# Quantco/tabmat

Measured on AMD Instinct MI355X. Metric: SplitMatrix.sandwich GFLOP/s + effective HBM GB/s, 10M×1k mixed, higher is better.
Workload: dtype f64; 1 GPU; SplitMatrix.sandwich: dense128 + csr512@5% + cats(256,96,32), 10000000 rows/GPU, p=1024, float64 (BASELINE configs[3]); rows_per_gpu=10000000, p=1024, launch=eager, collective=none

## Files before the change

include/tabmat_hip.h:

```cpp
#ifndef TABMAT_HIP_H
#define TABMAT_HIP_H

#include <stddef.h>
#include <stdint.h>

#ifdef __cplusplus
extern "C" {
#endif

#define TM_OK 0
#define TM_EINVAL (-1)
#define TM_ENOMEM (-2)
#define TM_EUNSUPPORTED (-3)

int tm_version(void);
const char *tm_last_error(void);
int tm_device_count(int *count);
int tm_set_device(int device);
int tm_device_info(char *name, int name_len, int *compute_units, int64_t *hbm_bytes);
int tm_malloc(void **ptr, size_t bytes);
int tm_free(void *ptr);
int tm_memcpy_h2d(void *dst, const void *h_src, size_t bytes, void *stream);
int tm_memcpy_d2h(void *h_dst, const void *src, size_t bytes, void *stream);
int tm_memset(void *dst, int value, size_t bytes, void *stream);
// ... 400 lines not shown
                                          int64_t n_sel, int64_t m, const double *d_sel, double *out,
                                          void *stream);
int tm_multi_cat_sparse_sandwich_rows_u8_f32(const void *const *h_codes, const int64_t *h_ncols,
                                             const int32_t *h_drop_first, int n_cats,
                                             const float *cm_data, const uint8_t *cm_col8,
                                             const int32_t *row_ranges, const int32_t *rows,
                                             int64_t n_sel, int64_t m, const float *d_sel, float *out,
                                             void *stream);
int tm_multi_cat_sparse_sandwich_rows_u8_f64(const void *const *h_codes, const int64_t *h_ncols,
                                             const int32_t *h_drop_first, int n_cats,
                                             const double *cm_data, const uint8_t *cm_col8,
                                             const int32_t *row_ranges, const int32_t *rows,
                                             int64_t n_sel, int64_t m, const double *d_sel, double *out,
                                             void *stream);
int tm_multi_cat_sparse_sandwich_ent_f32(const void *const *h_codes, const int64_t *h_ncols,
                                         const int32_t *h_drop_first, int n_cats, int64_t n, const float *d,
                                         const float *vals, const uint16_t *meta, const uint32_t *bstart,
                                         int64_t n_slots, int64_t mk, float *out, void *stream);
int tm_multi_cat_sparse_sandwich_ent_f64(const void *const *h_codes, const int64_t *h_ncols,
                                         const int32_t *h_drop_first, int n_cats, int64_t n, const double *d,
                                         const double *vals, const uint16_t *meta, const uint32_t *bstart,
                                         int64_t n_slots, int64_t mk, double *out, void *stream);
int tm_multi_cat_pack_codes(const void *const *h_codes, const int64_t *h_ncols, const int32_t *h_drop_first, int n_cats,
                            int64_t n, uint32_t *packed, void *stream);
int tm_multi_cat_sparse_sandwich_entp_f32(const void *const *h_codes, const int64_t *h_ncols,
                                          const int32_t *h_drop_first, int n_cats, int64_t n, const float *d,
                                          const float *vals, const uint16_t *meta, const uint32_t *bstart,
                                          int64_t n_slots, int64_t mk, const uint32_t *packed, float *out, void *stream);
int tm_multi_cat_sparse_sandwich_entp_f64(const void *const *h_codes, const int64_t *h_ncols,
                                          const int32_t *h_drop_first, int n_cats, int64_t n, const double *d,
                                          const double *vals, const uint16_t *meta, const uint32_t *bstart,
                                          int64_t n_slots, int64_t mk, const uint32_t *packed, double *out, void *stream);

int tm_multi_cat_sparse_sandwich_slab_f32(const void *const *h_codes, const int64_t *h_ncols,
                                          const int32_t *h_drop_first, int n_cats, int64_t n,
                                          const float *d, const float *vals, const uint32_t *koff,
                                          const uint8_t *ecol, const int64_t *gptr, int64_t m,
                                          float *out, void *stream);
int tm_multi_cat_sparse_sandwich_slab_f64(const void *const *h_codes, const int64_t *h_ncols,
                                          const int32_t *h_drop_first, int n_cats, int64_t n,
                                          const double *d, const double *vals, const uint32_t *koff,
                                          const uint8_t *ecol, const int64_t *gptr, int64_t m,
                                          double *out, void *stream);

int tm_multi_cat_pairs_max_bins(void);
int tm_multi_cat_pairs_max_slots(void);
int tm_multi_cat_pairs_row_words(void);
int tm_multi_cat_pairs_f32(const int64_t *cat_tab, int64_t n, const float *d, const int32_t *rows,
                           int64_t n_rows, const int32_t *bundles, int n_bundles,
                           const int32_t *wg_map, int n_wg, int slots, int64_t bins,
                           const int64_t *desc, int64_t n_pairs, const int64_t *pos, double *tables,
                           double *out, int64_t p, void *stream);
int tm_multi_cat_pairs_f64(const int64_t *cat_tab, int64_t n, const double *d, const int32_t *rows,
                           int64_t n_rows, const int32_t *bundles, int n_bundles,
                           const int32_t *wg_map, int n_wg, int slots, int64_t bins,
                           const int64_t *desc, int64_t n_pairs, const int64_t *pos, double *tables,
                           double *out, int64_t p, void *stream);

int tm_multi_cat_matvec_f32(const int64_t *cat_tab, int n_cats, const int64_t *pos, const float *v,
                            int64_t n, float *out, void *stream);
int tm_multi_cat_matvec_f64(const int64_t *cat_tab, int n_cats, const int64_t *pos, const double *v,
                            int64_t n, double *out, void *stream);

int tm_csr_densify_cols_f32(const float *data, const int32_t *indices, const int64_t *indptr, int64_t n,
                            const int32_t *colmap, float *T, int64_t ld, void *stream);
int tm_csr_densify_cols_f64(const double *data, const int32_t *indices, const int64_t *indptr, int64_t n,
                            const int32_t *colmap, double *T, int64_t ld, void *stream);
int tm_csc_densify_cols_f32(const int32_t *rows, const float *vals, const int64_t *seg, const int32_t *tcol,
                            int64_t n_sel, int64_t max_len, float *T, int64_t ld, void *stream);
int tm_csc_densify_cols_f64(const int32_t *rows, const double *vals, const int64_t *seg, const int32_t *tcol,
                            int64_t n_sel, int64_t max_len, double *T, int64_t ld, void *stream);
int tm_dense_gather_cols_f32(const float *X, int64_t n, int64_t m, int order_f, const int32_t *cols,
                             int64_t n_sel, float *T, int64_t ld, int64_t t0, void *stream);
int tm_dense_gather_cols_f64(const double *X, int64_t n, int64_t m, int order_f, const int32_t *cols,
                             int64_t n_sel, double *T, int64_t ld, int64_t t0, void *stream);

int tm_scatter_block_f32(const float *src, int64_t nr, int64_t nc, const int64_t *ri,
                         const int64_t *ci, double *out, int64_t p, int mirror, int diag,
                         void *stream);
int tm_scatter_block_f64(const double *src, int64_t nr, int64_t nc, const int64_t *ri,
                         const int64_t *ci, double *out, int64_t p, int mirror, int diag,
                         void *stream);

int tm_sparse_sandwich_chunked_rows_f32(const float *cm_data, const int32_t *cm_indices,
                                        const int32_t *row_ranges, int64_t n_sel, int64_t m,
                                        int64_t nnz, const float *d_sel, float *out, void *stream);
int tm_sparse_sandwich_chunked_rows_f64(const double *cm_data, const int32_t *cm_indices,
                                        const int32_t *row_ranges, int64_t n_sel, int64_t m,
                                        int64_t nnz, const double *d_sel, double *out, void *stream);

int tm_sparse_sandwich_chunked_u8_f32(const float *cm_data, const uint8_t *cm_col8, const int32_t *cptr, int64_t n,
                                      int64_t m, int64_t nnz, const float *d, float *out, void *stream);
int tm_sparse_sandwich_chunked_u8_f64(const double *cm_data, const uint8_t *cm_col8, const int32_t *cptr, int64_t n,
                                      int64_t m, int64_t nnz, const double *d, double *out, void *stream);
int tm_sparse_sandwich_chunked_rows_u8_f32(const float *cm_data, const uint8_t *cm_col8, const int32_t *row_ranges,
                                           int64_t n_sel, int64_t m, int64_t nnz, const float *d_sel, float *out,
                                           void *stream);
int tm_sparse_sandwich_chunked_rows_u8_f64(const double *cm_data, const uint8_t *cm_col8, const int32_t *row_ranges,
                                           int64_t n_sel, int64_t m, int64_t nnz, const double *d_sel, double *out,
                                           void *stream);
int tm_sparse_sandwich_direct_f32(const float *csr_data, const int32_t *csr_indices,
                                  const int64_t *csr_indptr, int64_t n, int64_t m, const float *d,
                                  float *out, void *stream);
int tm_sparse_sandwich_direct_f64(const double *csr_data, const int32_t *csr_indices,
                                  const int64_t *csr_indptr, int64_t n, int64_t m, const double *d,
                                  double *out, void *stream);
int tm_csr_dense_sandwich_rows_f32(const float *cm_data, const int32_t *cm_indices,
                                   const int32_t *row_ranges, int64_t n_sel, const int32_t *rows,
                                   const float *d_sel, int64_t n, int64_t m, const float *B, int64_t r,
                                   int order_f, float *out, void *stream);
int tm_csr_dense_sandwich_rows_f64(const double *cm_data, const int32_t *cm_indices,
                                   const int32_t *row_ranges, int64_t n_sel, const int32_t *rows,
                                   const double *d_sel, int64_t n, int64_t m, const double *B, int64_t r,
                                   int order_f, double *out, void *stream);
int tm_csr_dense_sandwich_rows_u8_f32(const float *cm_data, const uint8_t *cm_col8,
                                      const int32_t *row_ranges, int64_t n_sel, const int32_t *rows,
                                      const float *d_sel, int64_t n, int64_t m, const float *B, int64_t r,
                                      int order_f, float *out, void *stream);
int tm_csr_dense_sandwich_rows_u8_f64(const double *cm_data, const uint8_t *cm_col8,
                                      const int32_t *row_ranges, int64_t n_sel, const int32_t *rows,
                                      const double *d_sel, int64_t n, int64_t m, const double *B, int64_t r,
                                      int order_f, double *out, void *stream);

int tm_cat_det_block_rows(void);
int tm_cat_transpose_matvec_det_f32(const int32_t *perm, const int64_t *bstart, int64_t n_blocks,
                                    const int64_t *cat_bptr, int64_t n_cols, const float *v,
                                    float *out, int accumulate, void *stream);
int tm_cat_transpose_matvec_det_f64(const int32_t *perm, const int64_t *bstart, int64_t n_blocks,
                                    const int64_t *cat_bptr, int64_t n_cols, const double *v,
                                    double *out, int accumulate, void *stream);

int tm_cat_dense_sandwich_sorted_f32(const int32_t *perm, const int64_t *bstart, int64_t n_blocks,
                                     const int64_t *cat_bptr, int64_t n_cols, const float *d,
                                     const float *Y, int64_t m, float *out, void *stream);
int tm_cat_dense_sandwich_sorted_f64(const int32_t *perm, const int64_t *bstart, int64_t n_blocks,
                                     const int64_t *cat_bptr, int64_t n_cols, const double *d,
                                     const double *Y, int64_t m, double *out, void *stream);
int tm_csc_dense_sandwich_sorted_f32(const int32_t *rows, const float *vals, const int64_t *bstart,
                                     int64_t n_blocks, const int64_t *col_bptr, int64_t n_cols,
                                     const float *d, const float *Y, int64_t m, float *out,
                                     void *stream);
int tm_csc_dense_sandwich_sorted_f64(const int32_t *rows, const double *vals, const int64_t *bstart,
                                     int64_t n_blocks, const int64_t *col_bptr, int64_t n_cols,
                                     const double *d, const double *Y, int64_t m, double *out,
                                     void *stream);
int tm_cat_sparse_sandwich_sorted_f32(const int32_t *perm, const int64_t *bstart, int64_t n_blocks,
                                      const int64_t *cat_bptr, int64_t n_cols, const float *d,
                                      const float *csr_data, const int32_t *csr_indices,
                                      const int64_t *csr_indptr, int64_t m, float *out, void *stream);
int tm_cat_sparse_sandwich_sorted_f64(const int32_t *perm, const int64_t *bstart, int64_t n_blocks,
                                      const int64_t *cat_bptr, int64_t n_cols, const double *d,
                                      const double *csr_data, const int32_t *csr_indices,
                                      const int64_t *csr_indptr, int64_t m, double *out, void *stream);

int tm_csr_matvec_multi_f32(const float *csr_data, const int32_t *csr_indices,
                            const int64_t *csr_indptr, int64_t n, int64_t m, const float *V,
                            int64_t K, const int32_t *rows, int64_t n_rows, const int32_t *cols,
                            int64_t n_cols, float *out, void *stream);
int tm_csr_rmatvec_multi_f32(const float *csr_data, const int32_t *csr_indices,
                             const int64_t *csr_indptr, int64_t n, int64_t m, const float *V,
                             int64_t K, const int32_t *rows, int64_t n_rows, const int32_t *cols,
                             int64_t n_cols, float *out, void *stream);
int tm_dense_matvec_multi_f32(const float *X, int64_t n, int64_t m, int order_f, const float *V,
                              int64_t K, const int32_t *rows, int64_t n_rows, const int32_t *cols,
                              int64_t n_cols, float *out, void *stream);
int tm_dense_rmatvec_multi_f32(const float *X, int64_t n, int64_t m, int order_f, const float *V,
// ... 31 lines not shown
```

tabmat_amd/csrc/cat.hip:

```cpp
#include <algorithm>

#include "common.hpp"
#include "reduce.hpp"

namespace tmh {

__global__ void fill_i32_kernel(int32_t *p, int64_t n, int32_t v) {
    int64_t i = (int64_t)blockIdx.x * blockDim.x + threadIdx.x;
    if (i < n) p[i] = v;
}

__global__ void scatter_iota_i32_kernel(int32_t *map, const int32_t *cols, int64_t n_cols) {
    int64_t i = (int64_t)blockIdx.x * blockDim.x + threadIdx.x;
    if (i < n_cols) map[cols[i]] = (int32_t)i;
}

int build_col_map(int32_t *map, int64_t m, const int32_t *cols, int64_t n_cols, hipStream_t st) {
    if (m > 0) {
        hipLaunchKernelGGL(fill_i32_kernel, dim3((unsigned)ceil_div(m, 256)), dim3(256), 0, st, map,
                           m, -1);
        TM_LAUNCH_CHECK();
    }
    if (n_cols > 0) {
        hipLaunchKernelGGL(scatter_iota_i32_kernel, dim3((unsigned)ceil_div(n_cols, 256)),
                           dim3(256), 0, st, map, cols, n_cols);
        TM_LAUNCH_CHECK();
    }
    return TM_OK;
}

template <typename F, bool TWO>
__global__ __launch_bounds__(1024) void hist_lds_kernel(
    const int32_t *__restrict__ ci, const int32_t *__restrict__ cj, const F *__restrict__ w,
    const int32_t *__restrict__ rows, int64_t n_iter, int64_t rows_per_block, int drop_i,
    int drop_j, int i_ncol, int j_ncol, int ti, const int32_t *__restrict__ col_map,
    F *__restrict__ ws, int64_t stride) {
    extern __shared__ __attribute__((aligned(16))) unsigned char smem_raw[];
    lds_acc_t *bins = reinterpret_cast<lds_acc_t *>(smem_raw);
    const int part = blockIdx.y;
    const int i0 = part * ti;
    const int i1 = min(i0 + ti, i_ncol);
    const int nbins = TWO ? (i1 - i0) * j_ncol : (i1 - i0);
    for (int b = threadIdx.x; b < nbins; b += blockDim.x) bins[b] = 0.0;
    __syncthreads();

    const int64_t t0 = (int64_t)blockIdx.x * rows_per_block;
    const int64_t t1 = min(t0 + rows_per_block, n_iter);
    int64_t tbeg = t0;
    if (!TWO && rows == nullptr && (t0 & 3) == 0 &&
        ((reinterpret_cast<uintptr_t>(ci) | reinterpret_cast<uintptr_t>(w)) & 15) == 0) {
        typedef int i4 __attribute__((ext_vector_type(4)));
        const int64_t nvec = (t1 - t0) / 4;
        for (int64_t q = threadIdx.x; q < nvec; q += blockDim.x) {
            const int64_t k = t0 + q * 4;
            const i4 cc = *reinterpret_cast<const i4 *>(ci + k);
            F ww[4];
#pragma unroll
            for (int e = 0; e < 4; ++e) ww[e] = w[k + e];
#pragma unroll
            for (int e = 0; e < 4; ++e) {
                const int c = cc[e] - drop_i;
                if (c >= i0 && c < i1 && !(col_map && col_map[c] < 0)) atomic_add(&bins[c - i0], (lds_acc_t)ww[e]);
            }
        }
        tbeg = t0 + nvec * 4;
    }
    for (int64_t t = tbeg + threadIdx.x; t < t1; t += blockDim.x) {
        const int64_t k = rows ? (int64_t)rows[t] : t;
        const int c = ci[k] - drop_i;
        if (c < i0 || c >= i1) continue;
        if (TWO) {
            const int c2 = cj[k] - drop_j;
            if (c2 < 0) continue;
            atomic_add(&bins[(c - i0) * j_ncol + c2], (lds_acc_t)w[k]);
        } else {
            if (col_map && col_map[c] < 0) continue;
            atomic_add(&bins[c - i0], (lds_acc_t)w[k]);
        }
    }
    __syncthreads();
    F *dst = ws + ((int64_t)part * gridDim.x + blockIdx.x) * stride;
    for (int b = threadIdx.x; b < nbins; b += blockDim.x) dst[b] = (F)bins[b];
}

template <typename F, bool TWO>
// ... 1138 lines not shown
        }
    }
    __syncthreads();
    F *dst = ws + ((int64_t)blockIdx.y * gridDim.x + blockIdx.x) * stride;
    for (int b = threadIdx.x; b < cs.total * GC; b += blockDim.x)
        dst[b] = (F)tile[(b / GC) * TSTR + (b % GC)];
}

template <typename F, typename IX>
__global__ __launch_bounds__(1024) void multi_cat_sparse_rows_kernel(
    CatSet cs, const F *__restrict__ cm_data, const IX *__restrict__ cm_ind,
    const int32_t *__restrict__ ranges, const int32_t *__restrict__ rows, const F *__restrict__ d_sel,
    int64_t n_sel, int64_t rows_per_block, F *__restrict__ ws, int64_t stride) {
    constexpr int GC = 32;
    extern __shared__ __attribute__((aligned(16))) unsigned char smem_raw[];
    lds_acc_t *tile = reinterpret_cast<lds_acc_t *>(smem_raw);
    constexpr int tstr = GC + 1;
    const int nel = cs.total * tstr;
    for (int b = threadIdx.x; b < nel; b += blockDim.x) tile[b] = 0.0;
    __syncthreads();
    static_assert(SPARSE_CHUNK_COLS == 4 * GC, "the chunk of the chunk-major twin must hold four 32-column groups");
    const int g = blockIdx.y;
    const int ch = g >> 2;
    const int lane = threadIdx.x & 63, wave = threadIdx.x >> 6, nwave = blockDim.x >> 6;
    const int lr = lane >> 3, lt = lane & 7;
    const int64_t t0 = (int64_t)blockIdx.x * rows_per_block;
    const int64_t t1 = min(t0 + rows_per_block, n_sel);
    const int32_t *rg = ranges + (int64_t)ch * n_sel * 2;
    for (int64_t k0 = t0 + wave * 8; k0 < t1; k0 += (int64_t)nwave * 8) {
        const int64_t k = k0 + lr;
        if (k >= t1) continue;
        const F dk = d_sel[k];
        if (dk == F(0)) continue;
        const int e0 = rg[2 * k], e1 = rg[2 * k + 1];
        if (e0 >= e1) continue;
        const int64_t row = rows[k];
        int off[MAX_CATS];
#pragma unroll
        for (int c = 0; c < MAX_CATS; ++c) {
            off[c] = -1;
            if (c < cs.n_cats) {
                const int col = cs.codes[c][row] - cs.drop[c];
                off[c] = col >= 0 ? (cs.off[c] + col) * tstr : -1;
            }
        }
        for (int e = e0 + lt; e < e1; e += 8) {
            const int col = (int)cm_ind[e] - (sizeof(IX) == 1 ? (g & 3) : g) * GC;
            if (col < 0 || col >= GC) continue;
            const lds_acc_t x = (lds_acc_t)(dk * cm_data[e]);
#pragma unroll
            for (int c = 0; c < MAX_CATS; ++c)
                if (off[c] >= 0) atomic_add(&tile[off[c] + col], x);
        }
    }
    __syncthreads();
    F *dst = ws + ((int64_t)blockIdx.y * gridDim.x + blockIdx.x) * stride;
    for (int b = threadIdx.x; b < cs.total * GC; b += blockDim.x)
        dst[b] = (F)tile[(b / GC) * tstr + (b % GC)];
}

static int make_catset(const void *const *h_codes, const int64_t *h_ncols, const int32_t *h_drop,
                       int n_cats, CatSet *cs) {
    if (n_cats < 1 || n_cats > MAX_CATS) {
        set_error("multi-cat call supports 1..%d categoricals, got %d", MAX_CATS, n_cats);
        return TM_EINVAL;
    }
    int off = 0;
    for (int c = 0; c < MAX_CATS; ++c) {
        cs->codes[c] = c < n_cats ? reinterpret_cast<const int32_t *>(h_codes[c]) : nullptr;
        cs->ncol[c] = c < n_cats ? (int)h_ncols[c] : 0;
        cs->drop[c] = c < n_cats ? h_drop[c] : 0;
        cs->off[c] = off;
        off += cs->ncol[c];
    }
    cs->n_cats = n_cats;
    cs->total = off;
    return TM_OK;
}

template <typename F>
static int run_multi_cat_dense(const void *const *h_codes, const int64_t *h_ncols,
                               const int32_t *h_drop, int n_cats, int64_t n, const F *d, const F *M,
                               int64_t m, int order_f, F *out, hipStream_t st,
                               const int32_t *rows = nullptr, int64_t n_rows = 0) {
    CatSet cs;
    int rc = make_catset(h_codes, h_ncols, h_drop, n_cats, &cs);
    if (rc) return rc;
    const int64_t total = (int64_t)cs.total * m;
    if (total == 0) return TM_OK;
    if (rows != nullptr) n = n_rows;
    if (n == 0) {
        TM_HIP(hipMemsetAsync(out, 0, sizeof(F) * (size_t)total, st));
        return TM_OK;
    }
    {
        constexpr int VEC = MCW_VEC;
        constexpr int TJW = 16 * VEC;
        const size_t tile_b = ((sizeof(lds_acc_t) * (size_t)cs.total * TJW + 15) / 16) * 16;
        const size_t lds_w = tile_b + (size_t)16 * MCW_RS * (sizeof(F) + (size_t)n_cats * sizeof(int));
        if (!order_f && n_cats <= 8 && m >= VEC && m % VEC == 0 &&
            (reinterpret_cast<uintptr_t>(M) & 15) == 0 && lds_w <= 150 * 1024 &&
            (int64_t)cs.total * TJW * (int64_t)sizeof(lds_acc_t) < (1ll << 30)) {
            const int64_t n_parts = ceil_div(m, TJW);
            const int64_t stride = (int64_t)cs.total * TJW;
            int64_t nblk = std::max<int64_t>(1, tune("catdense_rounds", 1) * NUM_CU / n_parts);
            nblk = std::min<int64_t>(nblk, std::max<int64_t>(1, ceil_div(n, 4096)));
            const int64_t rpb = ceil_div(ceil_div(n, nblk), MCW_RS) * MCW_RS;
            nblk = ceil_div(n, rpb);
            const size_t tmp_bytes = ((sizeof(F) * (size_t)(n_parts * stride) + 255) / 256) * 256;
            void *wsv = nullptr;
            rc = get_workspace(tmp_bytes + sizeof(F) * (size_t)(n_parts * nblk * stride) + 256, &wsv, st);
            if (rc) return rc;
            F *tmp = reinterpret_cast<F *>(wsv);
            F *ws = reinterpret_cast<F *>(reinterpret_cast<char *>(wsv) + tmp_bytes);
            auto gow = [&](auto kern) -> int {
                TM_HIP(hipFuncSetAttribute(reinterpret_cast<const void *>(kern),
                                           hipFuncAttributeMaxDynamicSharedMemorySize, (int)lds_w));
                prof_begin(st);
                const int nw_dflt = (sizeof(F) == 8 && tile_b > 64 * 1024) ? 8 : 16;
                const int nw = (int)std::min<int64_t>(16, std::max<int64_t>(4, tune("catdense_waves", nw_dflt)));
                hipLaunchKernelGGL(kern, dim3((unsigned)nblk, (unsigned)n_parts), dim3(nw * 64), lds_w, st,
                                   cs, d, M, n, m, rpb, ws, stride, rows, wg_log_ptr());
                prof_end(st);
                TM_LAUNCH_CHECK();
                return TM_OK;
            };
            if (n_cats == 1) rc = gow(&multi_cat_dense_wide_kernel<F, 1>);
            else if (n_cats == 2) rc = gow(&multi_cat_dense_wide_kernel<F, 2>);
            else if (n_cats == 3) rc = gow(&multi_cat_dense_wide_kernel<F, 3>);
            else if (n_cats == 4) rc = gow(&multi_cat_dense_wide_kernel<F, 4>);
            else if (n_cats == 5) rc = gow(&multi_cat_dense_wide_kernel<F, 5>);
            else if (n_cats == 6) rc = gow(&multi_cat_dense_wide_kernel<F, 6>);
            else if (n_cats == 7) rc = gow(&multi_cat_dense_wide_kernel<F, 7>);
            else rc = gow(&multi_cat_dense_wide_kernel<F, 8>);
            if (rc) return rc;
            rc = launch_reduce_partials<F>(ws, stride, (int)nblk, (int)n_parts, tmp, n_parts * stride,
                                           false, st);
            if (rc) return rc;
            hipLaunchKernelGGL((multi_cat_untile_kernel<F>), dim3((unsigned)ceil_div(total, 256)),
                               dim3(256), 0, st, tmp, (int64_t)cs.total, m, TJW, out);
            TM_LAUNCH_CHECK();
            return TM_OK;
        }
    }
    if (rows != nullptr) {
        set_error("multi_cat_dense: the row-list form needs the wide-load path");
        return TM_EUNSUPPORTED;
    }
    int TJ = 64;
    while (TJ > 1 && sizeof(lds_acc_t) * (size_t)cs.total * TJ > HIST_LDS_MAX) TJ >>= 1;
    while (TJ > 1 && TJ / 2 >= m) TJ >>= 1;
    if (sizeof(lds_acc_t) * (size_t)cs.total * TJ > HIST_LDS_MAX) {
        set_error("multi_cat_dense: %d stacked categories exceed the LDS tile", cs.total);
        return TM_EUNSUPPORTED;
    }
    const int64_t n_parts = ceil_div(m, TJ);
    const int64_t stride = (int64_t)cs.total * TJ;
    const size_t lds = sizeof(lds_acc_t) * (size_t)stride;
    int64_t nblk = std::max<int64_t>(1, NUM_CU / n_parts);
    nblk = std::min<int64_t>(nblk, std::max<int64_t>(1, ceil_div(n, 4096)));
    const int64_t rpb = ceil_div(n, nblk);
    nblk = ceil_div(n, rpb);
    const size_t tmp_bytes = ((sizeof(F) * (size_t)(n_parts * stride) + 255) / 256) * 256;
    void *wsv = nullptr;
    rc = get_workspace(tmp_bytes + sizeof(F) * (size_t)(n_parts * nblk * stride) + 256, &wsv, st);
    if (rc) return rc;
    F *tmp = reinterpret_cast<F *>(wsv);
    F *ws = reinterpret_cast<F *>(reinterpret_cast<char *>(wsv) + tmp_bytes);
    auto go = [&](auto kern) -> int {
        if (lds > 48 * 1024)
            TM_HIP(hipFuncSetAttribute(reinterpret_cast<const void *>(kern),
                                       hipFuncAttributeMaxDynamicSharedMemorySize, (int)lds));
        prof_begin(st);
        hipLaunchKernelGGL(kern, dim3((unsigned)nblk, (unsigned)n_parts), dim3(1024), lds, st, cs, d,
                           M, n, m, rpb, ws, stride);
        prof_end(st);
        TM_LAUNCH_CHECK();
        return TM_OK;
    };
#define TM_MCD_CASE(V)                                                                       \
    case V:                                                                                  \
        if (order_f) rc = go(&multi_cat_dense_f_kernel<F, V>);                               \
        else if (n_cats == 1) rc = go(&multi_cat_dense_c_kernel<F, V, 1>);                   \
        else if (n_cats == 2) rc = go(&multi_cat_dense_c_kernel<F, V, 2>);                   \
        else if (n_cats == 3) rc = go(&multi_cat_dense_c_kernel<F, V, 3>);                   \
        else if (n_cats == 4) rc = go(&multi_cat_dense_c_kernel<F, V, 4>);                   \
        else rc = go(&multi_cat_dense_c_kernel<F, V, 0>);                                    \
        break;
    switch (TJ) {
        TM_MCD_CASE(64)
        TM_MCD_CASE(32)
        TM_MCD_CASE(16)
        TM_MCD_CASE(8)
        TM_MCD_CASE(4)
        TM_MCD_CASE(2)
        TM_MCD_CASE(1)
        default:
            rc = TM_EINVAL;
    }
#undef TM_MCD_CASE
    if (rc) return rc;
    rc = launch_reduce_partials<F>(ws, stride, (int)nblk, (int)n_parts, tmp, n_parts * stride, false,
                                   st);
    if (rc) return rc;
    hipLaunchKernelGGL((multi_cat_untile_kernel<F>), dim3((unsigned)ceil_div(total, 256)),
                       dim3(256), 0, st, tmp, (int64_t)cs.total, m, TJ, out);
    TM_LAUNCH_CHECK();
    return TM_OK;
}

template <typename F, typename IX>
static int run_multi_cat_sparse_rows(const void *const *h_codes, const int64_t *h_ncols,
                                     const int32_t *h_drop, int n_cats, const F *cm_data,
                                     const IX *cm_ind, const int32_t *ranges, const int32_t *rows,
                                     int64_t n_sel, int64_t m, const F *d_sel, F *out, hipStream_t st);

template <typename F>
static int run_multi_cat_sparse(const void *const *h_codes, const int64_t *h_ncols,
                                const int32_t *h_drop, int n_cats, int64_t n, const F *d,
                                const F *vals, const unsigned *koff, const unsigned char *ecol,
                                const int64_t *gptr, int64_t m, int slab_rows, int group_cols,
                                F *out, hipStream_t st) {
    CatSet cs;
    int rc = make_catset(h_codes, h_ncols, h_drop, n_cats, &cs);
    if (rc) return rc;
    const int64_t total = (int64_t)cs.total * m;
    if (total == 0) return TM_OK;
    if (n == 0) {
        TM_HIP(hipMemsetAsync(out, 0, sizeof(F) * (size_t)total, st));
// ... 1 lines not shown
    }
    const int64_t stride = (int64_t)cs.total * group_cols;
    const size_t tile_bytes = ((sizeof(lds_acc_t) * (size_t)cs.total * (group_cols + 1) + 15) / 16) * 16;
    if (tile_bytes > HIST_LDS_MAX) {
        set_error("multi_cat_sparse: %d stacked categories exceed the LDS tile", cs.total);
        return TM_EUNSUPPORTED;
    }
    const int nw = (int)std::min<int64_t>(16, std::max<int64_t>(4, tune("catsparse_waves", 16)));
    const size_t stage_bytes = (size_t)nw * slab_rows * (sizeof(F) + sizeof(int32_t) * (size_t)n_cats);
    const bool stage = tile_bytes + stage_bytes <= 150 * 1024;
    const size_t lds = tile_bytes + (stage ? stage_bytes : 0);
    const int n_groups = (int)ceil_div(m, group_cols);
    const int64_t n_slabs = ceil_div(n, slab_rows);
    int64_t nblk = std::max<int64_t>(1, tune("catsparse_rounds", 1) * NUM_CU / n_groups);
    nblk = std::min<int64_t>(nblk, n_slabs);
    const int64_t spb = ceil_div(n_slabs, nblk);
    nblk = ceil_div(n_slabs, spb);
    const size_t tmp_bytes = ((sizeof(F) * (size_t)(n_groups * stride) + 255) / 256) * 256;
    void *wsv = nullptr;
    rc = get_workspace(tmp_bytes + sizeof(F) * (size_t)((int64_t)n_groups * nblk * stride) + 256,
                       &wsv, st);
    if (rc) return rc;
    F *tmp = reinterpret_cast<F *>(wsv);
    F *ws = reinterpret_cast<F *>(reinterpret_cast<char *>(wsv) + tmp_bytes);
    if (stage && n_cats <= 8 && slab_rows == 128) {
        auto kpf = n_cats == 1   ? &multi_cat_sparse_pf_kernel<F, 1>
                   : n_cats == 2 ? &multi_cat_sparse_pf_kernel<F, 2>
                   : n_cats == 3 ? &multi_cat_sparse_pf_kernel<F, 3>
                   : n_cats == 4 ? &multi_cat_sparse_pf_kernel<F, 4>
                   : n_cats == 5 ? &multi_cat_sparse_pf_kernel<F, 5>
                   : n_cats == 6 ? &multi_cat_sparse_pf_kernel<F, 6>
                   : n_cats == 7 ? &multi_cat_sparse_pf_kernel<F, 7>
                                 : &multi_cat_sparse_pf_kernel<F, 8>;
        if (lds > 48 * 1024)
            TM_HIP(hipFuncSetAttribute(reinterpret_cast<const void *>(kpf),
                                       hipFuncAttributeMaxDynamicSharedMemorySize, (int)lds));
        prof_begin(st);
        hipLaunchKernelGGL(kpf, dim3((unsigned)nblk, (unsigned)n_groups), dim3(nw * 64), lds, st, cs, d,
                           vals, koff, ecol, gptr, n_groups, n_slabs, spb, group_cols, n, ws, stride,
                           wg_log_ptr());
        prof_end(st);
        TM_LAUNCH_CHECK();
    } else {
        auto kern = stage ? &multi_cat_sparse_kernel<F, true> : &multi_cat_sparse_kernel<F, false>;
        if (lds > 48 * 1024)
            TM_HIP(hipFuncSetAttribute(reinterpret_cast<const void *>(kern),
                                       hipFuncAttributeMaxDynamicSharedMemorySize, (int)lds));
        prof_begin(st);
        hipLaunchKernelGGL(kern, dim3((unsigned)nblk, (unsigned)n_groups), dim3(nw * 64), lds, st, cs,
                           d, vals, koff, ecol, gptr, n_groups, n_slabs, spb, slab_rows, group_cols,
                           n, ws, stride);
        prof_end(st);
        TM_LAUNCH_CHECK();
    }
    rc = launch_reduce_partials<F>(ws, stride, (int)nblk, n_groups, tmp,
                                   (int64_t)n_groups * stride, false, st);
    if (rc) return rc;
    hipLaunchKernelGGL((multi_cat_untile_kernel<F>), dim3((unsigned)ceil_div(total, 256)),
                       dim3(256), 0, st, tmp, (int64_t)cs.total, m, group_cols, out);
    TM_LAUNCH_CHECK();
    return TM_OK;
}

__global__ __launch_bounds__(256) void multi_cat_pack_codes_kernel(CatSet cs, int64_t n, unsigned *__restrict__ out) {
    for (int64_t r = (int64_t)blockIdx.x * blockDim.x + threadIdx.x; r < n; r += (int64_t)gridDim.x * blockDim.x) {
        unsigned pk = 0u;
#pragma unroll
        for (int c = 0; c < 3; ++c) {
            unsigned f = 1023u;
            if (c < cs.n_cats) {
                const int col = cs.codes[c][r] - cs.drop[c];
                if (col >= 0 && col < cs.ncol[c]) f = (unsigned)(cs.off[c] + col);
            }
            pk |= f << (10 * c);
        }
        out[r] = pk;
    }
}

template <typename F>
static int run_multi_cat_sparse_ent(const void *const *h_codes, const int64_t *h_ncols, const int32_t *h_drop,
                                    int n_cats, int64_t n, const F *d, const F *vals, const unsigned short *meta,
                                    const unsigned *bstart, int64_t mk, F *out, hipStream_t st,
                                    const unsigned *packed = nullptr, int64_t n_slots = 0) {
    CatSet cs;
    int rc = make_catset(h_codes, h_ncols, h_drop, n_cats, &cs);
    if (rc) return rc;
    const int64_t total = (int64_t)cs.total * mk;
    if (total == 0) return TM_OK;
    if (n == 0) {
        TM_HIP(hipMemsetAsync(out, 0, sizeof(F) * (size_t)total, st));
        return TM_OK;
    }
    TM_REQUIRE(mk % 16 == 0 && n_cats >= 1 && n_cats <= 8, "kernel columns in groups of 16, 1 .. 8 categoricals");
    TM_REQUIRE(n < (1ll << 28), "at most 2^28 - 1 rows per block");
    constexpr int GC = 32;
    const int64_t stride = (int64_t)cs.total * GC;
    const size_t lds = ((sizeof(lds_acc_t) * (size_t)cs.total * (GC + 1) + 15) / 16) * 16;
    if (lds > HIST_LDS_MAX) {
        set_error("multi_cat_sparse_ent: %d stacked categories exceed the LDS tile", cs.total);
        return TM_EUNSUPPORTED;
    }
    const int nw = (int)std::min<int64_t>(16, std::max<int64_t>(4, tune("catsparse_waves", 16)));
    const int n_groups = (int)(mk / 16);
    const int n_pairs = (n_groups + 1) / 2;
    const int64_t n_slabs = ceil_div(n, 64);
    int64_t nblk = std::max<int64_t>(1, tune("catsparse_rounds", 1) * NUM_CU / n_pairs);
    nblk = std::min<int64_t>(nblk, n_slabs);
    const int64_t spb = ceil_div(n_slabs, nblk);
    nblk = ceil_div(n_slabs, spb);
    const size_t tmp_bytes = ((sizeof(F) * (size_t)(n_pairs * stride) + 255) / 256) * 256;
    void *wsv = nullptr;
    rc = get_workspace(tmp_bytes + sizeof(F) * (size_t)((int64_t)n_pairs * nblk * stride) + 256, &wsv, st);
    if (rc) return rc;
    F *tmp = reinterpret_cast<F *>(wsv);
    F *ws = reinterpret_cast<F *>(reinterpret_cast<char *>(wsv) + tmp_bytes);
    auto kern = n_cats == 1   ? &multi_cat_sparse_ent_kernel<F, 1>
                : n_cats == 2 ? &multi_cat_sparse_ent_kernel<F, 2>
                : n_cats == 3 ? &multi_cat_sparse_ent_kernel<F, 3>
                : n_cats == 4 ? &multi_cat_sparse_ent_kernel<F, 4>
                : n_cats == 5 ? &multi_cat_sparse_ent_kernel<F, 5>
                : n_cats == 6 ? &multi_cat_sparse_ent_kernel<F, 6>
                : n_cats == 7 ? &multi_cat_sparse_ent_kernel<F, 7>
                              : &multi_cat_sparse_ent_kernel<F, 8>;
    TM_REQUIRE(packed == nullptr || (n_cats <= 3 && cs.total < 1023), "packed codes: at most 3 categoricals, 1022 levels");
    const int ncw = packed != nullptr ? 1 : n_cats;
    const size_t lds_staged = lds + (size_t)nw * 64 * (sizeof(F) + 4 * (size_t)ncw);
    const double fill = (double)n_slots / ((double)std::max(n_groups, 1) * (double)n_slabs);
    if (tune("catsparse_staged", 1) != 0 && lds_staged <= 156 * 1024 &&
        fill >= (double)tune("catsparse_staged_fill", 44)) {
        using KS = void (*)(CatSet, const F *, const F *, const unsigned short *, const unsigned *, int, int64_t, int64_t,
                            int64_t, F *, int64_t, const unsigned *, int);
        KS ks = nullptr;
        if (packed != nullptr) {
            ks = n_cats == 1 ? &multi_cat_sparse_ent_staged_kernel<F, 1, true>
                 : n_cats == 2 ? &multi_cat_sparse_ent_staged_kernel<F, 2, true>
                               : &multi_cat_sparse_ent_staged_kernel<F, 3, true>;
        } else {
            ks = n_cats == 1   ? &multi_cat_sparse_ent_staged_kernel<F, 1, false>
                 : n_cats == 2 ? &multi_cat_sparse_ent_staged_kernel<F, 2, false>
                 : n_cats == 3 ? &multi_cat_sparse_ent_staged_kernel<F, 3, false>
                 : n_cats == 4 ? &multi_cat_sparse_ent_staged_kernel<F, 4, false>
                 : n_cats == 5 ? &multi_cat_sparse_ent_staged_kernel<F, 5, false>
                 : n_cats == 6 ? &multi_cat_sparse_ent_staged_kernel<F, 6, false>
                 : n_cats == 7 ? &multi_cat_sparse_ent_staged_kernel<F, 7, false>
                               : &multi_cat_sparse_ent_staged_kernel<F, 8, false>;
        }
        if (lds_staged > 48 * 1024)
            TM_HIP(hipFuncSetAttribute(reinterpret_cast<const void *>(ks),
                                       hipFuncAttributeMaxDynamicSharedMemorySize, (int)lds_staged));
        prof_begin(st);
        hipLaunchKernelGGL(ks, dim3((unsigned)nblk, (unsigned)n_pairs), dim3(nw * 64), lds_staged, st, cs, d, vals,
                           meta, bstart, n_groups, n, n_slabs, spb, ws, stride, packed, (int)lds);
        prof_end(st);
        TM_LAUNCH_CHECK();
    } else {
        if (lds > 48 * 1024)
            TM_HIP(hipFuncSetAttribute(reinterpret_cast<const void *>(kern),
                                       hipFuncAttributeMaxDynamicSharedMemorySize, (int)lds));
        prof_begin(st);
        hipLaunchKernelGGL(kern, dim3((unsigned)nblk, (unsigned)n_pairs), dim3(nw * 64), lds, st, cs, d, vals, meta,
                           bstart, n_groups, n, n_slabs, spb, ws, stride, packed);
        prof_end(st);
        TM_LAUNCH_CHECK();
    }
    rc = launch_reduce_partials<F>(ws, stride, (int)nblk, n_pairs, tmp, (int64_t)n_pairs * stride, false, st);
    if (rc) return rc;
    hipLaunchKernelGGL((multi_cat_untile_kernel<F>), dim3((unsigned)ceil_div(total, 256)), dim3(256), 0, st, tmp,
                       (int64_t)cs.total, mk, GC, out);
    TM_LAUNCH_CHECK();
    return TM_OK;
}

}

using namespace tmh;

#define TM_CHECK_COMMON(nn) \
    TM_REQUIRE((nn) >= 0, "negative size")

extern "C" {

int tm_cat_transpose_matvec_f32(const int32_t *codes, int64_t n, int64_t n_cols, int drop_first,
                                const float *v, const int32_t *rows, int64_t n_rows,
                                const int32_t *cols, int64_t n_cols_sel, float *out, void *stream) {
    TM_CHECK_COMMON(n);
    return run_cat_tmv<float>(codes, n, n_cols, drop_first, v, rows, n_rows, cols, n_cols_sel, out,
                              as_stream(stream));
}
int tm_cat_transpose_matvec_f64(const int32_t *codes, int64_t n, int64_t n_cols, int drop_first,
                                const double *v, const int32_t *rows, int64_t n_rows,
                                const int32_t *cols, int64_t n_cols_sel, double *out,
                                void *stream) {
    TM_CHECK_COMMON(n);
    return run_cat_tmv<double>(codes, n, n_cols, drop_first, v, rows, n_rows, cols, n_cols_sel,
                               out, as_stream(stream));
}

int tm_cat_matvec_f32(const int32_t *codes, int64_t n, int64_t n_cols, int drop_first,
                      const float *v, const int32_t *cols, int64_t n_cols_sel, float *out,
                      void *stream) {
    TM_CHECK_COMMON(n);
    return run_cat_matvec<float>(codes, n, n_cols, drop_first, v, cols, n_cols_sel, out,
                                 as_stream(stream));
}
int tm_cat_matvec_f64(const int32_t *codes, int64_t n, int64_t n_cols, int drop_first,
                      const double *v, const int32_t *cols, int64_t n_cols_sel, double *out,
                      void *stream) {
    TM_CHECK_COMMON(n);
    return run_cat_matvec<double>(codes, n, n_cols, drop_first, v, cols, n_cols_sel, out,
                                  as_stream(stream));
}

int tm_cat_matvec_assign_f32(const int32_t *codes, int64_t n, int64_t n_cols, int drop_first,
                             const float *v, const int32_t *cols, int64_t n_cols_sel, float *out,
                             void *stream) {
    TM_CHECK_COMMON(n);
    return run_cat_matvec<float>(codes, n, n_cols, drop_first, v, cols, n_cols_sel, out,
                                 as_stream(stream), true);
}
int tm_cat_matvec_assign_f64(const int32_t *codes, int64_t n, int64_t n_cols, int drop_first,
                             const double *v, const int32_t *cols, int64_t n_cols_sel, double *out,
                             void *stream) {
    TM_CHECK_COMMON(n);
    return run_cat_matvec<double>(codes, n, n_cols, drop_first, v, cols, n_cols_sel, out,
                                  as_stream(stream), true);
}

int tm_cat_cat_sandwich_f32(const int32_t *i_codes, const int32_t *j_codes, int64_t n,
                            const float *d, const int32_t *rows, int64_t n_rows, int64_t i_ncol,
                            int64_t j_ncol, int i_drop_first, int j_drop_first, float *out,
                            void *stream) {
    TM_CHECK_COMMON(n);
    return run_hist<float, true>(i_codes, j_codes, d, rows, rows ? n_rows : n, i_drop_first,
                                 j_drop_first, i_ncol, j_ncol, nullptr, out, false,
                                 as_stream(stream));
}
int tm_cat_cat_sandwich_f64(const int32_t *i_codes, const int32_t *j_codes, int64_t n,
                            const double *d, const int32_t *rows, int64_t n_rows, int64_t i_ncol,
                            int64_t j_ncol, int i_drop_first, int j_drop_first, double *out,
                            void *stream) {
    TM_CHECK_COMMON(n);
    return run_hist<double, true>(i_codes, j_codes, d, rows, rows ? n_rows : n, i_drop_first,
                                  j_drop_first, i_ncol, j_ncol, nullptr, out, false,
                                  as_stream(stream));
}

int tm_cat_cat_sandwich_atomic_f32(const int32_t *i_codes, const int32_t *j_codes, int64_t n,
// ... 55 lines not shown
    TM_CHECK_COMMON(n);
    return run_cat_sparse<float>(codes, n, i_ncol, drop_first, csr_data, csr_indices, csr_indptr,
                                 s_ncol, d, rows, n_rows, cols, n_cols, out, as_stream(stream));
}
int tm_cat_sparse_sandwich_f64(const int32_t *codes, int64_t n, int64_t i_ncol, int drop_first,
                               const double *csr_data, const int32_t *csr_indices,
                               const int64_t *csr_indptr, int64_t s_ncol, const double *d,
                               const int32_t *rows, int64_t n_rows, const int32_t *cols,
                               int64_t n_cols, double *out, void *stream) {
    TM_CHECK_COMMON(n);
    return run_cat_sparse<double>(codes, n, i_ncol, drop_first, csr_data, csr_indices, csr_indptr,
                                  s_ncol, d, rows, n_rows, cols, n_cols, out, as_stream(stream));
}

int tm_multi_cat_dense_sandwich_f32(const void *const *h_codes, const int64_t *h_ncols,
                                    const int32_t *h_drop_first, int n_cats, int64_t n,
                                    const float *d, const float *M, int64_t M_ncol, int order_f,
                                    float *out, void *stream) {
    return run_multi_cat_dense<float>(h_codes, h_ncols, h_drop_first, n_cats, n, d, M, M_ncol,
                                      order_f, out, as_stream(stream));
}
int tm_multi_cat_dense_sandwich_f64(const void *const *h_codes, const int64_t *h_ncols,
                                    const int32_t *h_drop_first, int n_cats, int64_t n,
                                    const double *d, const double *M, int64_t M_ncol, int order_f,
                                    double *out, void *stream) {
    return run_multi_cat_dense<double>(h_codes, h_ncols, h_drop_first, n_cats, n, d, M, M_ncol,
                                       order_f, out, as_stream(stream));
}
int tm_multi_cat_dense_sandwich_rows_f32(const void *const *h_codes, const int64_t *h_ncols,
                                         const int32_t *h_drop_first, int n_cats, int64_t n,
                                         const float *d, const float *M, int64_t M_ncol,
                                         const int32_t *rows, int64_t n_rows, float *out,
                                         void *stream) {
    return run_multi_cat_dense<float>(h_codes, h_ncols, h_drop_first, n_cats, n, d, M, M_ncol, 0, out,
                                      as_stream(stream), rows, n_rows);
}
int tm_multi_cat_dense_sandwich_rows_f64(const void *const *h_codes, const int64_t *h_ncols,
                                         const int32_t *h_drop_first, int n_cats, int64_t n,
                                         const double *d, const double *M, int64_t M_ncol,
                                         const int32_t *rows, int64_t n_rows, double *out,
                                         void *stream) {
    return run_multi_cat_dense<double>(h_codes, h_ncols, h_drop_first, n_cats, n, d, M, M_ncol, 0, out,
                                       as_stream(stream), rows, n_rows);
}
int tm_multi_cat_sparse_sandwich_ent_f32(const void *const *h_codes, const int64_t *h_ncols,
                                         const int32_t *h_drop_first, int n_cats, int64_t n, const float *d,
                                         const float *vals, const uint16_t *meta, const uint32_t *bstart,
                                         int64_t n_slots, int64_t mk, float *out, void *stream) {
    return run_multi_cat_sparse_ent<float>(h_codes, h_ncols, h_drop_first, n_cats, n, d, vals, meta, bstart, mk,
                                           out, as_stream(stream), nullptr, n_slots);
}
int tm_multi_cat_sparse_sandwich_ent_f64(const void *const *h_codes, const int64_t *h_ncols,
                                         const int32_t *h_drop_first, int n_cats, int64_t n, const double *d,
                                         const double *vals, const uint16_t *meta, const uint32_t *bstart,
                                         int64_t n_slots, int64_t mk, double *out, void *stream) {
    return run_multi_cat_sparse_ent<double>(h_codes, h_ncols, h_drop_first, n_cats, n, d, vals, meta, bstart, mk,
                                            out, as_stream(stream), nullptr, n_slots);
}
int tm_multi_cat_pack_codes(const void *const *h_codes, const int64_t *h_ncols, const int32_t *h_drop_first, int n_cats,
                            int64_t n, uint32_t *packed, void *stream) {
    CatSet cs;
    int rc = make_catset(h_codes, h_ncols, h_drop_first, n_cats, &cs);
    if (rc) return rc;
    TM_REQUIRE(n_cats <= 3 && cs.total < 1023, "packed codes: at most 3 categoricals, 1022 stacked levels");
    if (n == 0) return TM_OK;
    hipLaunchKernelGGL(multi_cat_pack_codes_kernel, dim3((unsigned)std::min<int64_t>(4 * NUM_CU, ceil_div(n, 256))),
                       dim3(256), 0, as_stream(stream), cs, n, packed);
    TM_LAUNCH_CHECK();
    return TM_OK;
}
int tm_multi_cat_sparse_sandwich_entp_f32(const void *const *h_codes, const int64_t *h_ncols,
                                          const int32_t *h_drop_first, int n_cats, int64_t n, const float *d,
                                          const float *vals, const uint16_t *meta, const uint32_t *bstart,
                                          int64_t n_slots, int64_t mk, const uint32_t *packed, float *out, void *stream) {
    return run_multi_cat_sparse_ent<float>(h_codes, h_ncols, h_drop_first, n_cats, n, d, vals, meta, bstart, mk, out,
                                           as_stream(stream), packed, n_slots);
}
int tm_multi_cat_sparse_sandwich_entp_f64(const void *const *h_codes, const int64_t *h_ncols,
                                          const int32_t *h_drop_first, int n_cats, int64_t n, const double *d,
                                          const double *vals, const uint16_t *meta, const uint32_t *bstart,
                                          int64_t n_slots, int64_t mk, const uint32_t *packed, double *out, void *stream) {
    return run_multi_cat_sparse_ent<double>(h_codes, h_ncols, h_drop_first, n_cats, n, d, vals, meta, bstart, mk,
                                            out, as_stream(stream), packed, n_slots);
}
int tm_multi_cat_sparse_sandwich_slab_f32(const void *const *h_codes, const int64_t *h_ncols,
                                          const int32_t *h_drop_first, int n_cats, int64_t n,
                                          const float *d, const float *vals, const uint32_t *koff,
                                          const uint8_t *ecol, const int64_t *gptr, int64_t m,
                                          float *out, void *stream) {
    return run_multi_cat_sparse<float>(h_codes, h_ncols, h_drop_first, n_cats, n, d, vals, koff,
                                       ecol, gptr, m, tm_slab_rows(), tm_slab_group_cols(), out,
                                       as_stream(stream));
}
int tm_multi_cat_sparse_sandwich_slab_f64(const void *const *h_codes, const int64_t *h_ncols,
                                          const int32_t *h_drop_first, int n_cats, int64_t n,
                                          const double *d, const double *vals, const uint32_t *koff,
                                          const uint8_t *ecol, const int64_t *gptr, int64_t m,
                                          double *out, void *stream) {
    return run_multi_cat_sparse<double>(h_codes, h_ncols, h_drop_first, n_cats, n, d, vals, koff,
                                        ecol, gptr, m, tm_slab_rows(), tm_slab_group_cols(), out,
                                        as_stream(stream));
}

}

namespace tmh {
template <typename F, typename IX>
static int run_multi_cat_sparse_rows(const void *const *h_codes, const int64_t *h_ncols,
                                     const int32_t *h_drop, int n_cats, const F *cm_data,
                                     const IX *cm_ind, const int32_t *ranges, const int32_t *rows,
                                     int64_t n_sel, int64_t m, const F *d_sel, F *out, hipStream_t st) {
    CatSet cs;
    int rc = make_catset(h_codes, h_ncols, h_drop, n_cats, &cs);
    if (rc) return rc;
    const int64_t total = (int64_t)cs.total * m;
    if (total == 0) return TM_OK;
    if (n_sel == 0) {
        TM_HIP(hipMemsetAsync(out, 0, sizeof(F) * (size_t)total, st));
        return TM_OK;
    }
    constexpr int GC = 32;
    const size_t lds = ((sizeof(lds_acc_t) * (size_t)cs.total * (GC + 1) + 15) / 16) * 16;
    if (lds > HIST_LDS_MAX) {
        set_error("multi_cat_sparse_rows: %d stacked categories exceed the LDS tile", cs.total);
        return TM_EUNSUPPORTED;
    }
    const int n_groups = (int)ceil_div(m, GC);
    const int64_t stride = (int64_t)cs.total * GC;
    int64_t nblk = std::max<int64_t>(1, tune("catsparse_rounds", 1) * NUM_CU / n_groups);
    nblk = std::min<int64_t>(nblk, std::max<int64_t>(1, ceil_div(n_sel, 2048)));
    const int64_t rpb = ceil_div(n_sel, nblk);
    nblk = ceil_div(n_sel, rpb);
    const size_t tmp_bytes = ((sizeof(F) * (size_t)(n_groups * stride) + 255) / 256) * 256;
    void *wsv = nullptr;
    rc = get_workspace(tmp_bytes + sizeof(F) * (size_t)((int64_t)n_groups * nblk * stride) + 256, &wsv, st);
    if (rc) return rc;
    F *tmp = reinterpret_cast<F *>(wsv);
    F *ws = reinterpret_cast<F *>(reinterpret_cast<char *>(wsv) + tmp_bytes);
    auto kern = &multi_cat_sparse_rows_kernel<F, IX>;
    if (lds > 48 * 1024)
        TM_HIP(hipFuncSetAttribute(reinterpret_cast<const void *>(kern),
                                   hipFuncAttributeMaxDynamicSharedMemorySize, (int)lds));
    prof_begin(st);
    hipLaunchKernelGGL(kern, dim3((unsigned)nblk, (unsigned)n_groups), dim3(1024), lds, st, cs, cm_data,
                       cm_ind, ranges, rows, d_sel, n_sel, rpb, ws, stride);
    prof_end(st);
    TM_LAUNCH_CHECK();
    rc = launch_reduce_partials<F>(ws, stride, (int)nblk, n_groups, tmp, (int64_t)n_groups * stride, false, st);
    if (rc) return rc;
    hipLaunchKernelGGL((multi_cat_untile_kernel<F>), dim3((unsigned)ceil_div(total, 256)), dim3(256), 0,
                       st, tmp, (int64_t)cs.total, m, GC, out);
    TM_LAUNCH_CHECK();
    return TM_OK;
}
}

extern "C" {
int tm_multi_cat_sparse_sandwich_rows_f32(const void *const *h_codes, const int64_t *h_ncols,
                                          const int32_t *h_drop_first, int n_cats,
                                          const float *cm_data, const int32_t *cm_indices,
                                          const int32_t *row_ranges, const int32_t *rows,
                                          int64_t n_sel, int64_t m, const float *d_sel, float *out,
                                          void *stream) {
    return tmh::run_multi_cat_sparse_rows<float, int32_t>(h_codes, h_ncols, h_drop_first, n_cats, cm_data,
                                                 cm_indices, row_ranges, rows, n_sel, m, d_sel, out,
                                                 tmh::as_stream(stream));
// ... 33 lines not shown
```

tabmat_amd/csrc/common.hpp:

```cpp
#pragma once

#include <hip/hip_runtime.h>
#include <type_traits>
#include <stdint.h>
#include <stdio.h>

#include "../../include/tabmat_hip.h"

namespace tmh {

constexpr int WAVE = 64;
constexpr int NUM_CU = 256;
constexpr int NUM_XCD = 8;
constexpr int SPARSE_CHUNK_COLS = 128;
constexpr size_t LDS_BYTES = 160 * 1024;

void set_error(const char *fmt, ...);
int hip_fail(hipError_t e, const char *what, const char *file, int line);

#define TM_HIP(expr)                                                  \
    do {                                                              \
        hipError_t _e = (expr);                                       \
        if (_e != hipSuccess) return tmh::hip_fail(_e, #expr, __FILE__, __LINE__); \
    } while (0)

#define TM_LAUNCH_CHECK() TM_HIP(hipGetLastError())

#define TM_REQUIRE(cond, msg)                 \
    do {                                      \
        if (!(cond)) {                        \
            tmh::set_error("%s: %s", __func__, msg); \
            return TM_EINVAL;                 \
        }                                     \
    } while (0)

int get_workspace(size_t bytes, void **ptr, hipStream_t st);

void prof_begin(hipStream_t st);
void prof_end(hipStream_t st);
void prof_hold(bool on);

int64_t tune(const char *key, int64_t dflt);

int run_syrk_co(const double *X, int64_t n, int64_t m, const double *d, double *out,
                double *colsum, hipStream_t st, const double *center = nullptr, const double *v = nullptr,
                double *xtv = nullptr);
inline bool syrk_co_ok(const void *X, int64_t m) {
    return m > 0 && m <= 128 && (reinterpret_cast<uintptr_t>(X) & 15) == 0;
}
inline bool syrk_co_pays(int64_t m) { return m > 64; }

int run_syrk_i8_panel(const double *X, int64_t ldx, int64_t n, int64_t m, const double *d, const double *colmax,
                      double *out, int64_t ldo, double *colsum, int *history, hipStream_t st,
                      const double *center = nullptr, const double *v = nullptr, double *xtv = nullptr);

int run_syrk_bf16x3(const float *X, int64_t n, int64_t m, const float *d, float *out, hipStream_t st);
inline bool syrk_bf16x3_ok(const void *X, int64_t m) {
    return m > 0 && m <= 256 && m % 4 == 0 && (reinterpret_cast<uintptr_t>(X) & 15) == 0;
}

bool syrk_narrow_ok(int64_t m);
template <typename F>
int run_syrk_narrow(const F *X, int64_t n, int64_t m, int order_f, const F *d, F *out, hipStream_t st);

inline hipStream_t as_stream(void *s) { return reinterpret_cast<hipStream_t>(s); }

inline int64_t ceil_div(int64_t a, int64_t b) { return (a + b - 1) / b; }

typedef double lds_acc_t;

template <typename F>
__device__ __forceinline__ void atomic_add(F *p, F v) {
    atomicAdd(p, v);
}

template <typename F>
__device__ __forceinline__ F wave_sum(F v) {
#pragma unroll
    for (int off = 32; off > 0; off >>= 1) v += __shfl_down(v, off, 64);
    return v;
}

template <int S>
__device__ __forceinline__ int dpp_xor_i32(int v) {
    if constexpr (S == 1) return __builtin_amdgcn_mov_dpp(v, 0xB1, 0xF, 0xF, true);
    else if constexpr (S == 2) return __builtin_amdgcn_mov_dpp(v, 0x4E, 0xF, 0xF, true);
    else if constexpr (S == 3) return __builtin_amdgcn_mov_dpp(v, 0x1B, 0xF, 0xF, true);
    else if constexpr (S == 4) {
        const int m = __builtin_amdgcn_mov_dpp(v, 0x141, 0xF, 0xF, true);
        return __builtin_amdgcn_mov_dpp(m, 0x1B, 0xF, 0xF, true);
    } else return __builtin_amdgcn_mov_dpp(v, 0x128, 0xF, 0xF, true);
}
template <int S>
__device__ __forceinline__ double dpp_xor(double v) {
    return __hiloint2double(dpp_xor_i32<S>(__double2hiint(v)), dpp_xor_i32<S>(__double2loint(v)));
}
template <int S>
__device__ __forceinline__ float dpp_xor(float v) {
    return __int_as_float(dpp_xor_i32<S>(__float_as_int(v)));
}


__device__ __forceinline__ int64_t readfirstlane_i64(int64_t v) {
    const unsigned lo = (unsigned)__builtin_amdgcn_readfirstlane((int)(v & 0xffffffffll));
    const unsigned hi = (unsigned)__builtin_amdgcn_readfirstlane((int)(v >> 32));
    return (int64_t)(((unsigned long long)hi << 32) | lo);
}

template <int N, int K0 = 0, typename Fn>
__device__ __forceinline__ void static_for(Fn &&f) {
    if constexpr (K0 < N) {
        f(std::integral_constant<int, K0>{});
        static_for<N, K0 + 1>(f);
    }
}

template <int K>
__device__ __forceinline__ int dpp_bcast8_i32(int v, int x4) {
    constexpr int QP = (K & 3) * 0x55;
    const int t = __builtin_amdgcn_mov_dpp(x4, QP, 0xF, 0xF, true);
    return __builtin_amdgcn_update_dpp(t, v, QP, 0xF, K < 4 ? 0x5 : 0xA, false);
}
template <int K>
__device__ __forceinline__ double dpp_bcast8(double v, double x4) {
    return __hiloint2double(dpp_bcast8_i32<K>(__double2hiint(v), __double2hiint(x4)),
                            dpp_bcast8_i32<K>(__double2loint(v), __double2loint(x4)));
}
template <int K>
__device__ __forceinline__ float dpp_bcast8(float v, float x4) {
    return __int_as_float(dpp_bcast8_i32<K>(__float_as_int(v), __float_as_int(x4)));
}

struct WgLog {
    unsigned long long hw, t0, t1, tag;
};
struct WgLogBuf {
    unsigned long long count, cap, pad0, pad1;
    WgLog e[1];
};
enum WgTag { WG_SYRK_CO = 1, WG_K2 = 2, WG_CAT_DENSE = 3, WG_CAT_SPARSE = 4, WG_K3 = 5 };
inline WgLogBuf *wg_log_ptr() { return reinterpret_cast<WgLogBuf *>((uintptr_t)tune("wg_log", 0)); }
__device__ __forceinline__ unsigned long long wg_log_begin(const WgLogBuf *b) {
    return b ? wall_clock64() : 0ull;
}
__device__ __forceinline__ void wg_log_end(WgLogBuf *b, unsigned long long t_begin, int tag) {
    if (!b) return;
    const unsigned long long i = atomicAdd(&b->count, 1ull);
    if (i >= b->cap) return;
    const unsigned hw = __builtin_amdgcn_s_getreg((31 << 11) | 4);
    const unsigned xcc = __builtin_amdgcn_s_getreg((31 << 11) | 20);
// ... 12 lines not shown
```

tabmat_amd/csrc/reduce.hpp:

```cpp
#pragma once
#include "common.hpp"

namespace tmh {

template <typename F, bool ACCUMULATE, int NW>
__global__ __launch_bounds__(NW * 64) void reduce_partials_kernel(const F *__restrict__ ws,
                                                                  int64_t stride, int nb,
                                                                  F *__restrict__ out,
                                                                  int64_t out_elems) {
    __shared__ double red[NW][64];
    const int lane = threadIdx.x & 63;
    const int wave = threadIdx.x >> 6;
    const int64_t e = (int64_t)blockIdx.x * 64 + lane;
    const int part = blockIdx.y;
    double acc = 0.0;
    if (e < stride) {
        const F *p = ws + ((int64_t)part * nb) * stride + e;
        for (int b = wave; b < nb; b += NW) acc += (double)p[(int64_t)b * stride];
    }
    red[wave][lane] = acc;
    __syncthreads();
    if (wave == 0 && e < stride) {
        const int64_t o = (int64_t)part * stride + e;
        if (o < out_elems) {
            double s = 0.0;
#pragma unroll
            for (int w = 0; w < NW; w += 4)
                s += (red[w][lane] + red[w + 1][lane]) + (red[w + 2][lane] + red[w + 3][lane]);
            if (ACCUMULATE)
                out[o] += (F)s;
            else
                out[o] = (F)s;
        }
    }
}

template <typename F>
inline int launch_reduce_partials(const F *ws, int64_t stride, int nb, int n_parts, F *out,
                                  int64_t out_elems, bool accumulate, hipStream_t st) {
    dim3 grid((unsigned)ceil_div(stride, 64), (unsigned)n_parts);
    const bool small = (int64_t)grid.x * grid.y < 1024 && nb > 16;
    if (small) {
        if (accumulate)
            hipLaunchKernelGGL((reduce_partials_kernel<F, true, 16>), grid, dim3(1024), 0, st, ws,
                               stride, nb, out, out_elems);
        else
            hipLaunchKernelGGL((reduce_partials_kernel<F, false, 16>), grid, dim3(1024), 0, st, ws,
                               stride, nb, out, out_elems);
    } else if (accumulate) {
        hipLaunchKernelGGL((reduce_partials_kernel<F, true, 4>), grid, dim3(256), 0, st, ws, stride,
                           nb, out, out_elems);
    } else {
        hipLaunchKernelGGL((reduce_partials_kernel<F, false, 4>), grid, dim3(256), 0, st, ws, stride,
                           nb, out, out_elems);
    }
    TM_LAUNCH_CHECK();
    return TM_OK;
}

__global__ void fill_i32_kernel(int32_t *p, int64_t n, int32_t v);
__global__ void scatter_iota_i32_kernel(int32_t *map, const int32_t *cols, int64_t n_cols);

int build_col_map(int32_t *map, int64_t m, const int32_t *cols, int64_t n_cols, hipStream_t st);

}
```

tabmat_amd/csrc/sparse_blocks.hip:

```cpp
#include <algorithm>

#include "common.hpp"
#include "reduce.hpp"

namespace tmh {

constexpr int KB_WAVES = 16;
constexpr int KB_TS = 128;

template <typename F>
__global__ void blocks_assemble_kernel(const F *__restrict__ tiles, int n_out, F *__restrict__ out) {
    const int j = blockIdx.x * blockDim.x + threadIdx.x;
    const int i = blockIdx.y;
    if (i >= n_out || j >= n_out) return;
    const int hi = max(i, j), lo = min(i, j);
    const int I = hi / KB_TS, J = lo / KB_TS;
    const int part = I * (I + 1) / 2 + J;
    out[(int64_t)i * n_out + j] = tiles[(int64_t)part * KB_TS * KB_TS + (hi % KB_TS) * KB_TS + (lo % KB_TS)];
}

constexpr int KB_FLAG_REP_A = 1 << 16;
constexpr int KB_FLAG_REP_B = 1 << 17;

template <typename F, bool U8, bool D12 = false>
__global__ __launch_bounds__(KB_WAVES * 64) void sparse_sandwich_blocks_kernel(
    const F *__restrict__ data, const int32_t *__restrict__ ind, const int32_t *__restrict__ cptr,
    int64_t n, int64_t nnz1, const int32_t *__restrict__ blocks, const int4 *__restrict__ wg_tab,
    const F *__restrict__ d, int max_nb, F *__restrict__ ws, WgLogBuf *__restrict__ wglog) {
    constexpr int TS = KB_TS;
    const unsigned long long t_begin = wg_log_begin(wglog);
    extern __shared__ __attribute__((aligned(16))) unsigned char smem_raw[];
    lds_acc_t *tile = reinterpret_cast<lds_acc_t *>(smem_raw);
    const int4 w = wg_tab[2 * blockIdx.x], x = wg_tab[2 * blockIdx.x + 1];
    const int part = __builtin_amdgcn_readfirstlane(w.x), slot = __builtin_amdgcn_readfirstlane(w.y);
    const int b0 = __builtin_amdgcn_readfirstlane(w.z), b1 = __builtin_amdgcn_readfirstlane(w.w);
    const int bfull = __builtin_amdgcn_readfirstlane(x.x);
    int wfull = __builtin_amdgcn_readfirstlane(x.y);
    {
        const int nwv = (int)(blockDim.x >> 6);
        if (nwv != KB_WAVES) {
            wfull = (wfull * nwv + KB_WAVES / 2) / KB_WAVES;
            if (bfull > b0) wfull = max(wfull, 1);
            if (b1 > bfull) wfull = min(wfull, nwv - 1);
            if (bfull == b0) wfull = 0;
            if (b1 == bfull) wfull = nwv;
        }
    }
    int I = (int)((sqrtf(8.0f * (float)part + 1.0f) - 1.0f) * 0.5f);
    while ((I + 1) * (I + 2) / 2 <= part) ++I;
    while (I * (I + 1) / 2 > part) --I;
    const int J = part - I * (I + 1) / 2;
    const int i0 = I * TS, j0 = J * TS;
    for (int b = threadIdx.x; b < TS * TS; b += blockDim.x) tile[b] = 0.0;
    __syncthreads();

    const int lane = threadIdx.x & 63;
    const int wave = __builtin_amdgcn_readfirstlane(threadIdx.x >> 6);
    const int lr = lane >> 3, lt = lane & 7;
    if (b1 > b0) {
        const int row_first = __builtin_amdgcn_readfirstlane(x.z), row_last = __builtin_amdgcn_readfirstlane(x.w);
        const int32_t *cpA = cptr + (int64_t)I * (n + 1), *cpB = cptr + (int64_t)J * (n + 1);
        const int baseA = __builtin_amdgcn_readfirstlane(cpA[row_first]);
        const int baseB = __builtin_amdgcn_readfirstlane(cpB[row_first]);
        const unsigned spanA1 = (unsigned)max(__builtin_amdgcn_readfirstlane(cpA[row_last + 1]) - baseA - 1, 0);
        const unsigned spanB1 = (unsigned)max(__builtin_amdgcn_readfirstlane(cpB[row_last + 1]) - baseB - 1, 0);
        const F *dataA = data + min((int64_t)baseA, nnz1), *dataB = data + min((int64_t)baseB, nnz1);
        const int32_t *indA = ind + min((int64_t)baseA, nnz1), *indB = ind + min((int64_t)baseB, nnz1);
        const unsigned char *ind8 = reinterpret_cast<const unsigned char *>(ind);
        const unsigned char *ind8A = ind8 + min((int64_t)baseA, nnz1), *ind8B = ind8 + min((int64_t)baseB, nnz1);
        const int i0c = U8 ? 0 : i0, j0c = U8 ? 0 : j0;
        const unsigned nrow1 = (unsigned)max(n - 1, (int64_t)0);
        auto ldi = [](const int32_t *base, unsigned i) {
            return *reinterpret_cast<const int32_t *>(reinterpret_cast<const char *>(base) + (i << 2));
        };
        auto ldf = [](const F *base, unsigned i) {
            return *reinterpret_cast<const F *>(reinterpret_cast<const char *>(base) + (i * (unsigned)sizeof(F)));
        };
        constexpr int SH = 3;
        constexpr int BIGKEY = 0x7ffffff0;
        char *const tile_bytes = reinterpret_cast<char *>(tile);
        auto add_pair = [&](int kb, int la, int ba, F prod) {
            if (kb <= la)
                atomic_add(reinterpret_cast<lds_acc_t *>(tile_bytes + (unsigned)(kb ^ ba)), (lds_acc_t)prod);
        };

// ... 35 lines not shown
                const unsigned iA = min((unsigned)(sd.q.x - baseA) + min((unsigned)e.ta, (unsigned)max(e.nA - 1, 0)), spanA1);
                const unsigned iB = min((unsigned)(sd.q.y - baseB) + min((unsigned)e.tb, (unsigned)max(e.nB - 1, 0)), spanB1);
#ifdef KB_ABL_WRAP
                const unsigned iAw = iA & (unsigned)(KB_ABL_WRAP), iBw = iB & (unsigned)(KB_ABL_WRAP);
                e.ca = ldi(indA, min(iAw, spanA1));
                e.va = ldf(dataA, min(iAw, spanA1));
                e.cb = ldi(indB, min(iBw, spanB1));
                e.vb = ldf(dataB, min(iBw, spanB1));
                return e;
#endif
                e.ca = U8 ? (int)ind8A[iA] : ldi(indA, iA);
                e.va = ldf(dataA, iA);
                e.cb = U8 ? (int)ind8B[iB] : ldi(indB, iB);
                e.vb = ldf(dataB, iB);
                return e;
            };
            auto process = [&](const Grp &cur) {
                __builtin_amdgcn_s_setprio(1);
                const int colA = cur.ta < cur.nA ? cur.ca - i0c : -1;
                const int colB = cur.tb < cur.nB ? cur.cb - j0c : -1;
                const int la = (colA < 0 ? -8 : colA << SH) | offmask;
                const int ba = (int)(((unsigned)colA << (7 + SH)) | ((colA & 15) << (3 + SH)));
                const int kb = colB < 0 ? BIGKEY : colB << SH;
                const F av = cur.va * cur.d, vb = cur.vb;
                add_pair(kb, la, ba, av * vb);
                add_pair(dpp_xor_i32<1>(kb), la, ba, av * dpp_xor<1>(vb));
                add_pair(dpp_xor_i32<2>(kb), la, ba, av * dpp_xor<2>(vb));
                add_pair(dpp_xor_i32<3>(kb), la, ba, av * dpp_xor<3>(vb));
#ifndef KB_ABL_HALFSTEPS
                if constexpr (FULL) {
                    const int kb4 = dpp_xor_i32<4>(kb);
                    const F vb4 = dpp_xor<4>(vb);
                    add_pair(kb4, la, ba, av * vb4);
                    add_pair(dpp_xor_i32<1>(kb4), la, ba, av * dpp_xor<1>(vb4));
                    add_pair(dpp_xor_i32<2>(kb4), la, ba, av * dpp_xor<2>(vb4));
                    add_pair(dpp_xor_i32<3>(kb4), la, ba, av * dpp_xor<3>(vb4));
                }
#endif
                __builtin_amdgcn_s_setprio(0);
            };
            const int gstep = nw * 8;
            const int gw = (wave - w0) * 8;
            Grp ea[2], eb[2];
            Dsc ps[2];
            ea[0] = load_entries(load_desc(gw));
            ea[1] = load_entries(load_desc(gw + gstep));
            ps[0] = load_desc(gw + 2 * gstep);
            ps[1] = load_desc(gw + 3 * gstep);
            for (int g = gw; g < nseg; g += 4 * gstep) {
                eb[0] = load_entries(ps[0]);
                eb[1] = load_entries(ps[1]);
                ps[0] = load_desc(g + 4 * gstep);
                ps[1] = load_desc(g + 5 * gstep);
                process(ea[0]);
                if (g + gstep < nseg) process(ea[1]);
                if (g + 2 * gstep >= nseg) break;
                ea[0] = load_entries(ps[0]);
                ea[1] = load_entries(ps[1]);
                ps[0] = load_desc(g + 6 * gstep);
                ps[1] = load_desc(g + 7 * gstep);
                process(eb[0]);
                if (g + 3 * gstep < nseg) process(eb[1]);
            }
        };
        auto run_tile = [&](auto diag_c) {
            if (wave < wfull) run_list(diag_c, std::true_type{}, b0, bfull, 0, wfull);
            else run_list(diag_c, std::false_type{}, bfull, b1, wfull, (int)(blockDim.x >> 6) - wfull);
        };
        if (I == J) run_tile(std::true_type{});
        else run_tile(std::false_type{});
    }
    __syncthreads();
    if (threadIdx.x == 0) wg_log_end(wglog, t_begin, WG_K2);
    F *dst = ws + ((int64_t)part * max_nb + slot) * (TS * TS);
    for (int b = threadIdx.x; b < TS * TS; b += blockDim.x) {
        const int r = b / TS, c = b % TS;
        dst[b] = (F)tile[r * TS + (c ^ ((r & 15) << 3))];
    }
}

template <typename F, bool U8 = false, bool D12 = false>
static int run_sparse_sandwich_blocks(const F *data, const int32_t *ind, const int32_t *cptr, int64_t n,
                                      int64_t m, int64_t nnz, const int32_t *blocks, const int32_t *wg_tab,
                                      int n_wg, int max_nb, const F *d, F *out, hipStream_t st) {
    if (m == 0) return TM_OK;
    if (n == 0 || nnz == 0 || n_wg == 0) {
        TM_HIP(hipMemsetAsync(out, 0, sizeof(F) * (size_t)(m * m), st));
        return TM_OK;
    }
    constexpr int TS = KB_TS;
    const int nchunk = (int)ceil_div(m, TS);
    const int n_parts = nchunk * (nchunk + 1) / 2;
    TM_REQUIRE(nnz < (1ll << 31) && n < (1ll << 29), "sparse block too large for the block-list sandwich");
    TM_REQUIRE(!D12 || n < (1ll << 24), "12-byte block descriptors hold 24 bits of row");
    TM_REQUIRE(max_nb >= 1 && n_wg >= 1, "empty workgroup table");
    const size_t lds = sizeof(lds_acc_t) * (size_t)(TS * TS);
    const size_t tmp_bytes = (sizeof(F) * (size_t)n_parts * TS * TS + 255) / 256 * 256;
    const size_t ws_bytes = sizeof(F) * (size_t)n_parts * (size_t)max_nb * TS * TS;
    void *wsv = nullptr;
    int rc = get_workspace(tmp_bytes + ws_bytes + 256, &wsv, st);
    if (rc) return rc;
    F *tmp = reinterpret_cast<F *>(wsv);
    F *ws = reinterpret_cast<F *>(reinterpret_cast<char *>(wsv) + tmp_bytes);
    TM_HIP(hipMemsetAsync(ws, 0, ws_bytes, st));
    auto kern = &sparse_sandwich_blocks_kernel<F, U8, D12>;
    TM_HIP(hipFuncSetAttribute(reinterpret_cast<const void *>(kern),
                               hipFuncAttributeMaxDynamicSharedMemorySize, (int)lds));
    prof_begin(st);
    const int kb_waves = (int)std::min<int64_t>(KB_WAVES, std::max<int64_t>(2, tune("k2b_waves", KB_WAVES)));
    hipLaunchKernelGGL(kern, dim3((unsigned)n_wg), dim3(kb_waves * 64), lds, st, data, ind, cptr, n, nnz - 1,
                       blocks, reinterpret_cast<const int4 *>(wg_tab), d,
                       max_nb, ws, wg_log_ptr());
    prof_end(st);
    TM_LAUNCH_CHECK();
    rc = launch_reduce_partials<F>(ws, (int64_t)TS * TS, max_nb, n_parts, tmp, (int64_t)n_parts * TS * TS,
                                   false, st);
    if (rc) return rc;
    hipLaunchKernelGGL((blocks_assemble_kernel<F>), dim3((unsigned)ceil_div(m, 64), (unsigned)m), dim3(64),
                       0, st, tmp, (int)m, out);
    TM_LAUNCH_CHECK();
    return TM_OK;
}

}

extern "C" {

int tm_sparse_sandwich_blocks_f32(const float *cm_data, const int32_t *cm_indices, const int32_t *cptr,
                                  int64_t n, int64_t m, int64_t nnz, const int32_t *blocks,
                                  const int32_t *wg_tab, int n_wg, int max_nb, const float *d, float *out,
                                  void *stream) {
    return tmh::run_sparse_sandwich_blocks<float>(cm_data, cm_indices, cptr, n, m, nnz, blocks, wg_tab, n_wg,
                                                  max_nb, d, out, tmh::as_stream(stream));
}
int tm_sparse_sandwich_blocks_f64(const double *cm_data, const int32_t *cm_indices, const int32_t *cptr,
                                  int64_t n, int64_t m, int64_t nnz, const int32_t *blocks,
                                  const int32_t *wg_tab, int n_wg, int max_nb, const double *d, double *out,
                                  void *stream) {
    return tmh::run_sparse_sandwich_blocks<double>(cm_data, cm_indices, cptr, n, m, nnz, blocks, wg_tab, n_wg,
                                                   max_nb, d, out, tmh::as_stream(stream));
}

int tm_sparse_sandwich_blocks_u8_f32(const float *cm_data, const uint8_t *cm_col8, const int32_t *cptr,
                                     int64_t n, int64_t m, int64_t nnz, const int32_t *blocks,
                                     const int32_t *wg_tab, int n_wg, int max_nb, const float *d, float *out,
                                     void *stream) {
    return tmh::run_sparse_sandwich_blocks<float, true>(cm_data, reinterpret_cast<const int32_t *>(cm_col8), cptr, n, m,
                                                        nnz, blocks, wg_tab, n_wg, max_nb, d, out,
                                                        tmh::as_stream(stream));
}
int tm_sparse_sandwich_blocks_u8_f64(const double *cm_data, const uint8_t *cm_col8, const int32_t *cptr,
                                     int64_t n, int64_t m, int64_t nnz, const int32_t *blocks,
                                     const int32_t *wg_tab, int n_wg, int max_nb, const double *d, double *out,
                                     void *stream) {
    return tmh::run_sparse_sandwich_blocks<double, true>(cm_data, reinterpret_cast<const int32_t *>(cm_col8), cptr, n, m,
                                                         nnz, blocks, wg_tab, n_wg, max_nb, d, out,
                                                         tmh::as_stream(stream));
}

int tm_sparse_sandwich_blocks_p12_f32(const float *cm_data, const uint8_t *cm_col8, const int32_t *cptr,
                                      int64_t n, int64_t m, int64_t nnz, const int32_t *blocks12,
                                      const int32_t *wg_tab, int n_wg, int max_nb, const float *d, float *out,
                                      void *stream) {
    return tmh::run_sparse_sandwich_blocks<float, true, true>(cm_data, reinterpret_cast<const int32_t *>(cm_col8), cptr,
                                                              n, m, nnz, blocks12, wg_tab, n_wg, max_nb, d, out,
                                                              tmh::as_stream(stream));
}
int tm_sparse_sandwich_blocks_p12_f64(const double *cm_data, const uint8_t *cm_col8, const int32_t *cptr,
                                      int64_t n, int64_t m, int64_t nnz, const int32_t *blocks12,
                                      const int32_t *wg_tab, int n_wg, int max_nb, const double *d, double *out,
                                      void *stream) {
    return tmh::run_sparse_sandwich_blocks<double, true, true>(cm_data, reinterpret_cast<const int32_t *>(cm_col8), cptr,
                                                               n, m, nnz, blocks12, wg_tab, n_wg, max_nb, d, out,
                                                               tmh::as_stream(stream));
}

}
```

tabmat_amd/csrc/sparse_ent.hip:

```cpp
#include "common.hpp"
#include "reduce.hpp"

namespace tmh {

constexpr int EN_R = 64;
constexpr int EN_C = 16;
constexpr int EN_NW = 16;
constexpr int EN_THREADS = EN_NW * 64;
constexpr int EN_W = 128;
constexpr int EN_B = 16;
constexpr int EN_SB = 64;

template <typename F>
struct EnLds {
    static constexpr int ROWB = EN_W * (int)sizeof(F);
    static constexpr int SLABB = EN_R * ROWB;
    static constexpr int SCR_OFF = ROWB + 2 * SLABB;
    static constexpr int CS_OFF = SCR_OFF + EN_NW * EN_SB * 16;
    static constexpr int TOTAL = CS_OFF + EN_NW * EN_C * (int)sizeof(double);
};

constexpr int EN_CVGPR = 24;
#define EN_LD "40"

#if defined(__HIP_DEVICE_COMPILE__)
typedef __amdgpu_buffer_rsrc_t en_rsrc_t;
__device__ __forceinline__ en_rsrc_t en_rsrc(const void *base, int64_t bytes) {
    const unsigned nb = bytes <= 0 ? 0u : (bytes > 0xFFFFFFFFll ? 0xFFFFFFFFu : (unsigned)bytes);
    return __builtin_amdgcn_make_buffer_rsrc(const_cast<void *>(base), 0, (int)nb, 0x00020000);
}
__device__ __forceinline__ void en_buf_to_lds16(en_rsrc_t rs, void *lds, int voff, int soff) {
    __builtin_amdgcn_raw_ptr_buffer_load_lds(rs, (__attribute__((address_space(3))) void *)lds, 16, voff,
                                             soff, 0, 0);
}
template <typename F>
__device__ __forceinline__ void en_zero_acc() {
    if constexpr (sizeof(F) == 8) {
        static_for<16>([&](auto jc) {
            asm volatile("v_mov_b32 v[64+4*%0], 0\n\tv_mov_b32 v[64+4*%0+1], 0\n\t"
                         "v_mov_b32 v[64+4*%0+2], 0\n\tv_mov_b32 v[64+4*%0+3], 0"
                         :: "n"(decltype(jc)::value) : "v127");
        });
    } else {
        static_for<16>([&](auto jc) {
            asm volatile("v_mov_b32 v[64+2*%0], 0\n\tv_mov_b32 v[64+2*%0+1], 0" :: "n"(decltype(jc)::value) : "v95");
        });
    }
}
template <int K>
__device__ __forceinline__ unsigned en_read_acc() {
    unsigned x;
    asm volatile("v_mov_b32 %0, v[64+%1]" : "=v"(x) : "n"(K));
    return x;
}
template <typename F>
__device__ __forceinline__ void en_load_stream(unsigned voff_v, const F *vp, unsigned voff_m, const unsigned short *mp) {
    if constexpr (sizeof(F) == 8)
        asm volatile("global_load_dwordx2 v[" EN_LD ":" EN_LD "+1], %0, %1\n\t"
                     "global_load_ushort v[" EN_LD "+2], %2, %3" :: "v"(voff_v), "s"(vp), "v"(voff_m), "s"(mp) : "memory");
    else
        asm volatile("global_load_dword v[" EN_LD "], %0, %1\n\t"
                     "global_load_ushort v[" EN_LD "+2], %2, %3" :: "v"(voff_v), "s"(vp), "v"(voff_m), "s"(mp) : "memory");
}
template <typename F>
__device__ __forceinline__ void en_load_d(unsigned voff, const F *dp) {
    if constexpr (sizeof(F) == 8)
        asm volatile("global_load_dwordx2 v[" EN_LD "+4:" EN_LD "+5], %0, %1" :: "v"(voff), "s"(dp) : "memory");
    else
        asm volatile("global_load_dword v[" EN_LD "+4], %0, %1" :: "v"(voff), "s"(dp) : "memory");
}
template <int N>
__device__ __forceinline__ void en_take(double &v, unsigned &m, double &dd) {
    unsigned vl, vh, dl, dh;
    asm volatile("s_waitcnt vmcnt(%5)\n\t"
                 "v_mov_b32 %0, v[" EN_LD "]\n\tv_mov_b32 %1, v[" EN_LD "+1]\n\tv_mov_b32 %2, v[" EN_LD "+2]\n\t"
                 "v_mov_b32 %3, v[" EN_LD "+4]\n\tv_mov_b32 %4, v[" EN_LD "+5]"
                 : "=v"(vl), "=v"(vh), "=v"(m), "=v"(dl), "=v"(dh) : "n"(N) : "memory");
    v = __hiloint2double((int)vh, (int)vl);
    dd = __hiloint2double((int)dh, (int)dl);
}
template <int N>
__device__ __forceinline__ void en_take(float &v, unsigned &m, float &dd) {
    unsigned vl, dl;
// ... 195 lines not shown
        if (q != 3) enext = scratch[(q + 1) * EN_B + l16];
        EN_TICK(pt_a)
        const int slab = __builtin_amdgcn_readlane((int)e[3], 1);
        while (w < slab) end_slab();
        if (ncopied == 0 && w + 1 < ns) {
            issue_pieces((w & 1) ^ 1, 0, NV);

            ncopied = NV;
            psince += NV;
            lsince = 0;
        }
        EN_TICK(pt_p)
        F a;
        if constexpr (sizeof(F) == 8) a = __hiloint2double((int)e[1], (int)e[0]);
        else a = __uint_as_float(e[0]);
#if defined(EN_ABL_NOBATCH)
        asm volatile("" ::"v"(a), "v"(e[2]), "v"(e[3]));
#else
        const unsigned live = (unsigned)__builtin_amdgcn_ballot_w64(a != F(0)) & 0xffffu;
        const int nq = live ? ((31 - __builtin_clz(live)) >> 2) + 1 : 0;
        unsigned p0 = (unsigned)__builtin_amdgcn_readlane((int)e[3], 0);
        unsigned p1 = (unsigned)__builtin_amdgcn_readlane((int)e[3], 4);
        unsigned p2 = (unsigned)__builtin_amdgcn_readlane((int)e[3], 8);
        unsigned p3 = (unsigned)__builtin_amdgcn_readlane((int)e[3], 12);
        if (nq == 4) en_batch_asm<16, F>(p0, p1, p2, p3, a, e[2], lane_off);
        else if (nq == 3) en_batch_asm<12, F>(p0, p1, p2, p3, a, e[2], lane_off);
        else if (nq == 2) en_batch_asm<8, F>(p0, p1, p2, p3, a, e[2], lane_off);
        else if (nq == 1) en_batch_asm<4, F>(p0, p1, p2, p3, a, e[2], lane_off);
#endif
        EN_TICK(pt_x)
#if defined(EN_PROF)
        ++pt_n;
#endif
    }
    while (w < ns) end_slab();
    wait_loads(std::integral_constant<int, 0>{});
#if defined(EN_PROF)
    if (prof != nullptr && lane == 0) {
        long long *o = prof + (((int64_t)blockIdx.z * gridDim.y + blockIdx.y) * gridDim.x + blockIdx.x) * (EN_NW * 8) + wave * 8;
        o[0] = pt_a; o[1] = pt_p; o[2] = pt_x; o[3] = pt_b; o[4] = pt_bar; o[5] = pt_n; o[6] = clock64() - pt_start; o[7] = ns;
    }
#endif

    if (active) {
        F *dst = ws + (((int64_t)blockIdx.y * gridDim.x + blockIdx.x) * n_groups + group) * (EN_C * EN_W);
        static_for<EN_C>([&](auto jc) {
            constexpr int j = decltype(jc)::value;
            if constexpr (sizeof(F) == 8) {
                const u4 o = u4{en_read_acc<4 * j>(), en_read_acc<4 * j + 1>(), en_read_acc<4 * j + 2>(),
                                en_read_acc<4 * j + 3>()};
                *reinterpret_cast<u4 *>(dst + j * EN_W + 2 * lane) = o;
            } else {
                typedef unsigned u2 __attribute__((ext_vector_type(2)));
                const u2 o = u2{en_read_acc<2 * j>(), en_read_acc<2 * j + 1>()};
                *reinterpret_cast<u2 *>(dst + j * EN_W + 2 * lane) = o;
            }
        });
        if constexpr (CSUM) {
            if (blockIdx.y == 0 && lane < EN_C)
                ws_csum[(int64_t)blockIdx.x * (n_groups * EN_C) + group * EN_C + lane] = (F)cs_lds[lane];
        }
    }
}

template <typename F>
__global__ void en_untile_kernel(const F *__restrict__ tmp, int64_t m, int64_t nB, F *__restrict__ out) {
    const int64_t e = (int64_t)blockIdx.x * blockDim.x + threadIdx.x;
    if (e >= m * nB) return;
    const int64_t i = e / nB, j = e % nB;
    out[e] = tmp[((j / EN_W) * m + i) * EN_W + (j % EN_W)];
}

template <typename F>
__global__ void en_csum_kernel(const F *__restrict__ part, int nblk, int64_t m, F *__restrict__ csum) {
    const int64_t c = (int64_t)blockIdx.x * blockDim.x + threadIdx.x;
    if (c >= m) return;
    double a = 0.0;
    for (int b = 0; b < nblk; ++b) a += (double)part[(int64_t)b * m + c];
    csum[c] = (F)a;
}

template <typename F>
static int run_csr_dense_ent(const F *vals, const uint16_t *meta, const uint32_t *bstart, int64_t n, int64_t m,
                             const F *B, int64_t r, const F *d, F *out, F *colsum, hipStream_t st) {
    const int64_t nB = r;
    const int64_t total = m * nB;
    if (total == 0) return TM_OK;
    constexpr int VEC = 16 / (int)sizeof(F);
    if ((reinterpret_cast<uintptr_t>(B) & 15) != 0 || r % VEC != 0 || nB < VEC) {
        set_error("tm_csr_dense_sandwich_ent: B must be C-ordered with 16-byte aligned rows");
        return TM_EUNSUPPORTED;
    }
    if (m % EN_C != 0) {
        set_error("tm_csr_dense_sandwich_ent: m must be a multiple of tm_ent_group_cols()");
        return TM_EINVAL;
    }
    if (n >= (1ll << 28)) {
        set_error("tm_csr_dense_sandwich_ent: at most 2^28 - 1 rows per block (work in row parts)");
        return TM_EUNSUPPORTED;
    }
    const int64_t n_slabs = ceil_div(n, EN_R);
    const int n_groups = (int)(m / EN_C);
    const int n_parts = (int)ceil_div(nB, EN_W);
    const int nz = (int)ceil_div(n_groups, EN_NW);
    const bool want_csum = colsum != nullptr;
    if (n_slabs == 0) {
        TM_HIP(hipMemsetAsync(out, 0, sizeof(F) * (size_t)total, st));
        if (want_csum) TM_HIP(hipMemsetAsync(colsum, 0, sizeof(F) * (size_t)m, st));
        return TM_OK;
    }
    int64_t nblk = std::max<int64_t>(1, tune("ent_rounds", 1) * NUM_CU / ((int64_t)n_parts * nz));
    nblk = std::min<int64_t>(nblk, n_slabs);
    const int64_t spb = ceil_div(n_slabs, nblk);
    nblk = ceil_div(n_slabs, spb);
    const int64_t stride = m * EN_W;
    const size_t tmp_bytes = (sizeof(F) * (size_t)(n_parts * stride) + 255) / 256 * 256;
    const size_t part_bytes = (sizeof(F) * (size_t)((int64_t)n_parts * nblk * stride) + 255) / 256 * 256;
    const size_t csum_bytes = ((want_csum ? sizeof(F) * (size_t)(nblk * m) : 0) + 255) / 256 * 256 + 256;
    void *wsv = nullptr;
    int rc = get_workspace(tmp_bytes + part_bytes + csum_bytes + 256, &wsv, st);
    if (rc) return rc;
    F *tmp = reinterpret_cast<F *>(wsv);
    F *ws = reinterpret_cast<F *>(reinterpret_cast<char *>(wsv) + tmp_bytes);
    F *ws_csum = reinterpret_cast<F *>(reinterpret_cast<char *>(wsv) + tmp_bytes + part_bytes);
    const size_t lds = (size_t)EnLds<F>::TOTAL;
    auto kern = want_csum ? &csr_dense_ent_kernel<F, true> : &csr_dense_ent_kernel<F, false>;
    TM_HIP(hipFuncSetAttribute(reinterpret_cast<const void *>(kern),
                               hipFuncAttributeMaxDynamicSharedMemorySize, (int)lds));
    prof_begin(st);
    hipLaunchKernelGGL(kern, dim3((unsigned)nblk, (unsigned)n_parts, (unsigned)nz), dim3(EN_THREADS), lds, st,
                       vals, meta, bstart, n_groups, n_slabs, spb, B, n, r, (int)nB, d, ws, ws_csum,
                       reinterpret_cast<long long *>((uintptr_t)tune("ent_prof", 0)));
    prof_end(st);
    TM_LAUNCH_CHECK();
    rc = launch_reduce_partials<F>(ws, stride, (int)nblk, n_parts, tmp, n_parts * stride, false, st);
    if (rc) return rc;
    hipLaunchKernelGGL((en_untile_kernel<F>), dim3((unsigned)ceil_div(total, 256)), dim3(256), 0, st, tmp, m,
                       nB, out);
    TM_LAUNCH_CHECK();
    if (want_csum) {
        hipLaunchKernelGGL((en_csum_kernel<F>), dim3((unsigned)ceil_div(m, 256)), dim3(256), 0, st, ws_csum,
                           (int)nblk, m, colsum);
        TM_LAUNCH_CHECK();
    }
    return TM_OK;
}

}

extern "C" {
int tm_ent_rows(void) { return tmh::EN_R; }
int tm_ent_group_cols(void) { return tmh::EN_C; }
int tm_ent_batch_slots(void) { return tmh::EN_B; }

int tm_csr_dense_sandwich_ent_f32(const float *vals, const uint16_t *meta, const uint32_t *bstart, int64_t n,
                                  int64_t m, const float *B, int64_t r, const float *d, float *out,
                                  float *colsum, void *stream) {
    return tmh::run_csr_dense_ent<float>(vals, meta, bstart, n, m, B, r, d, out, colsum, tmh::as_stream(stream));
}
int tm_csr_dense_sandwich_ent_f64(const double *vals, const uint16_t *meta, const uint32_t *bstart, int64_t n,
                                  int64_t m, const double *B, int64_t r, const double *d, double *out,
                                  double *colsum, void *stream) {
    return tmh::run_csr_dense_ent<double>(vals, meta, bstart, n, m, B, r, d, out, colsum, tmh::as_stream(stream));
}
}
```

tabmat_amd/sparse_matrix.py:

```python
from __future__ import annotations

import os

import numpy as np
import torch
from scipy import sparse as sps

from . import _device as D
from .ext import sparse as xs
from .ext._types import CsrDev, SlabCsc, SlabEll, SlabEnt, SlabLg
from .matrix_base import MatrixBase
from .util import (
    check_indexer,
    check_matvec_dimensions,
    check_matvec_out_shape,
    check_sandwich_compatible,
    check_transpose_matvec_out_shape,
    normalize_index,
    device_row_index,
    selects_all_columns,
)


ELL_MAX_PAD = 8.0
# ... 141 lines not shown
    @property
    def indices(self):
        return self._host().indices

    @property
    def indptr(self):
        return self._host().indptr

    @property
    def data(self):
        return self._host().data

    __array_ufunc__ = None

    def tocsc(self, copy=False):
        return self._host().tocsc(copy=copy)

    def unpack(self):
        return self._host()

    def toarray(self):
        return self._host().toarray()

    def dot(self, other):
        return self._host().dot(other)

    def transpose(self):
        return type(self)(self._host().T)

    T = property(transpose)

    def getcol(self, i):
        return type(self)(self._host()[:, [i]], column_names=[self._colnames[i]],
                          term_names=[self._terms[i]])

    def astype(self, dtype, order="K", casting="unsafe", copy=True):
        return type(self)(self._host().astype(dtype, casting, copy))

    def __getitem__(self, key):
        row, col = check_indexer(key)
        if self._devblk is not None and selects_all_columns(col, self.shape[1]):
            sub = type(self).from_device(self._devblk.take_rows(*device_row_index(row, self.shape[0])))
            sub._colnames, sub._terms = list(self._colnames), list(self._terms)
            return sub
        names = np.array(self._colnames, dtype=object)[col].ravel().tolist()
        terms = np.array(self._terms, dtype=object)[col].ravel().tolist()
        return type(self)(self._host()[row, col], column_names=names, term_names=terms)

    def __matmul__(self, other):
        return self.matvec(other)

    def multiply(self, other):
        if other.ndim == 1:
            return type(self)(self._host().multiply(other[:, np.newaxis]))
        return type(self)(self._host().multiply(other))

    def _row_parts(self):
        parts = self.__dict__.get("_parts_cache", False)
        if parts is False:
            parts = None
            ptr = self._dev().indptr
            nnz = int(self._dev().data.numel())
            if nnz >= PART_NNZ:
                n = self.shape[0]
                k = -(-nnz // max(1, int(0.8 * PART_NNZ)))
                targets = torch.arange(1, k, device=ptr.device, dtype=torch.int64) * nnz // k
                cuts = sorted(set([0] + torch.searchsorted(ptr, targets).clamp_(0, n).tolist() + [n]))
                parts = [(a, b, self[a:b]) for a, b in zip(cuts[:-1], cuts[1:]) if b > a]
            self.__dict__["_parts_cache"] = parts
        return parts

    def _narrow_pays(self, w: int) -> bool:
        n, mcols = self.shape
        nnz = float(self._dev().data.numel())
        per_row = nnz / max(n, 1)
        pairs = n * per_row * (per_row + 1) / 2
        nch = -(-mcols // 128)
        t_full = max(31e-12 * (nch * (nch + 1) / 2) * n, 1.6e-12 * pairs)
        if getattr(self, "_direct_pays", None):
            t_full = pairs / 22e9
        t_narrow = 0.2e-3 + n * w * 4.5e-12 + nnz * w / max(mcols, 1) * 40e-12
        return t_narrow < 0.8 * t_full

    def _sandwich_dev(self, d, rows, cols):
        parts = self._row_parts()
        if parts is not None:
            out = None
            for a, b, part in parts:
                r = None
                if rows is not None:
                    r64 = rows.to(torch.int64)
                    sel = r64[(r64 >= a) & (r64 < b)]
                    if sel.numel() == 0:
                        continue
                    r = (sel - a).to(torch.int32)
                res = part._sandwich_dev(d[a:b], r, cols)
                out = res if out is None else out + res
            if out is None:
                k = self.shape[1] if cols is None else D.nlen(cols)
                out = D.zeros((k, k), d.dtype)
            return out
        A = self._dev()
        from . import categorical_matrix as _cm

        if _cm.DETERMINISTIC and A.data.numel() > 0 and self.shape[0] > 0:
            res = self._sandwich_deterministic(d, rows, cols)
            if res is not None:
                return res
            import warnings

            warnings.warn("TABMAT_AMD_DETERMINISTIC=1: this sparse block has no entry twin, its self sandwich "
                          "falls back to the LDS-atomic kernels and is NOT bit-reproducible from run to run",
                          RuntimeWarning, stacklevel=3)
        if getattr(self, "_direct_pays", None) is None:
            self._direct_pays = xs.direct_sandwich_pays(A)
        w = D.nlen(cols) if cols is not None else 0
        if (0 < w <= NARROW_COLS and 2 * w < self.shape[1] and self.shape[0] > 0 and A.data.numel() > 0
                and self._narrow_pays(w)
                and self.shape[0] * w * A.data.element_size() * 4 < torch.cuda.mem_get_info()[0]):
            from .ext import dense as xd
            from .ext._types import DenseDev

            rws, vls, bstart, _, col_bptr = A.csc_blocks()
            mx = getattr(self, "_max_col_len", None)
            if mx is None:
                ends = bstart[col_bptr]
                mx = self._max_col_len = int((ends[1:] - ends[:-1]).max().item())
            cd = cols.to(torch.int64)
            seg = torch.stack([bstart[col_bptr[cd]], bstart[col_bptr[cd + 1]]], dim=1).contiguous()
            T = torch.zeros((self.shape[0], w), dtype=A.data.dtype, device=A.data.device)
            xs.csc_densify_cols(rws, vls, seg, torch.arange(w, dtype=torch.int32, device=A.data.device),
                                mx, T)
            return xd.dense_sandwich(DenseDev(T, self.shape[0], w, 0), d, rows, None)
        pp = getattr(self, "_pairs_pay", None)
        if pp is None:
            pp = self._pairs_pay = xs.pairs_sandwich_pays(A)
        if pp and (rows is None or D.nlen(rows) > 0.3 * self.shape[0]):
            d = D.masked_d(d, rows, as_set=True)
            res = xs.sparse_sandwich_pairs(A, d)
            if cols is not None:
                c64 = cols.to(torch.int64)
                res = res[c64][:, c64].contiguous()
            return res
        pays = getattr(self, "_direct_pays", None)
        if pays is None:
            pays = self._direct_pays = xs.direct_sandwich_pays(A)
        if pays:
            d = D.masked_d(d, rows, as_set=True)
            res = xs.sparse_sandwich_direct(A, d)
            if cols is not None:
                c64 = cols.to(torch.int64)
                res = res[c64][:, c64].contiguous()
            return res
        if A.data.numel() > 0 and A.data.numel() < 2**31 and self.shape[1] <= 128 * 32:
            if rows is not None and 0 < D.nlen(rows) <= ROW_LIST_FRACTION * self.shape[0]:
                res = xs.sparse_sandwich_rows(A, d, rows)
                if cols is not None:
                    c64 = cols.to(torch.int64)
                    res = res[c64][:, c64].contiguous()
                return res
            d = D.masked_d(d, rows, as_set=True)
            bl = getattr(self, "_blocks_pay", None)
            if bl is None:
                bl = self._blocks_pay = xs.blocks_sandwich_pays(A)
            res = xs.sparse_sandwich_blocks(A, d) if bl else xs.sparse_sandwich_chunked(A, d)
            if cols is not None:
                c64 = cols.to(torch.int64)
                res = res[c64][:, c64].contiguous()
            return res
        return xs.sparse_sandwich(A, d, rows, cols)

    def _ent_det(self):
        ent = self._ent()
        if ent is None:
            hit = getattr(self, "_entblk_det", None)
            if hit is None:
                twin = SlabEnt.from_csr(self._dev(), max_pad=None)
                hit = self._entblk_det = twin if twin is not None else False
            ent = hit or None
        return ent

    def _sandwich_deterministic(self, d, rows, cols=None):
        from .ext._types import DenseDev

        ent = self._ent_det()
        if ent is None:
            return None
        n, m = self.shape
        A = self._dev()
        d = D.masked_d(d, rows, as_set=True)
        inv = None
        if cols is None:
            sel = torch.arange(m, dtype=torch.int64, device=d.device)
        else:
            sel, inv = torch.unique(cols.to(torch.int64), return_inverse=True)
            if int(sel.numel()) == int(inv.numel()) and bool((sel == cols.to(torch.int64)).all()):
                inv = None
        k = int(sel.numel())
        out = torch.empty((m, k), dtype=d.dtype, device=d.device)
        W = 128
        for c0 in range(0, k, W):
            w = min(W, k - c0)
            w_pad = (w + 3) // 4 * 4
            colmap = torch.full((m,), -1, dtype=torch.int32, device=d.device)
            colmap[sel[c0:c0 + w]] = torch.arange(w, dtype=torch.int32, device=d.device)
            T = torch.zeros((n, w_pad), dtype=A.data.dtype, device=d.device)
            xs.csr_densify_cols(A, colmap, T)
            res = xs.csr_dense_sandwich_ent(ent, DenseDev(T, n, w_pad, 0), d)
            out[:, c0:c0 + w] = res[:, :w]
            del T
        out = out if cols is None else out[sel]
        low = torch.tril(out)
        full = low + torch.tril(out, -1).T
        if inv is not None:
            full = full.index_select(0, inv).index_select(1, inv)
        return full

    def _sdiag_dev(self, d, rows, want_s1=False):
        parts = self._row_parts()
        if parts is not None:
            s1 = D.zeros((self.shape[1],), d.dtype) if want_s1 else None
            s2 = D.zeros((self.shape[1],), d.dtype)
            for a, b, part in parts:
                r = None
                if rows is not None:
                    r64 = rows.to(torch.int64)
                    sel = r64[(r64 >= a) & (r64 < b)]
                    if sel.numel() == 0:
                        continue
                    r = (sel - a).to(torch.int32)
                p1, p2 = part._sdiag_dev(d[a:b], r, want_s1)
                s2 += p2
                if want_s1:
                    s1 += p1
            return s1, s2
        A = self._dev()
        if rows is not None and A.data.numel() > 0 and not self._values_finite():
            r64 = rows.to(torch.int64)
            return xs.csr_sandwich_diag(A.take_rows("index", r64), d[r64].contiguous(), want_s1)
        return xs.csr_sandwich_diag(A, D.masked_d(d, rows).contiguous(), want_s1)

    def sandwich_diag(self, d, rows=None, cols=None):
        from .matrix_base import _sd_args

        a = _sd_args(self, d, rows, cols)
        if a.trivial is not None:
            return a.finish(a.trivial)
        tdt = D.torch_dtype(self.dtype)
        _, g = self._sdiag_dev(D.to_dev(a.d, tdt), D.idx_dev(a.rows))
        if a.cols is not None:
            g = g[D.idx_dev(a.cols, torch.int64)]
        return a.finish(g)

    def sandwich(self, d, rows=None, cols=None):
        on_dev = D.is_dev(d)
        if not on_dev:
            d = np.asarray(d)
        check_sandwich_compatible(self, d)
        res = self._sandwich_dev(D.to_dev(d), D.idx_dev(normalize_index(rows, self.shape[0])),
                                 D.idx_dev(normalize_index(cols, self.shape[1])))
        return res if on_dev else D.to_host(res)

    def _cross_sandwich_dev(self, other, d, rows, L_cols, R_cols, colsum_box=None):
        from .categorical_matrix import CategoricalMatrix
        from .dense_matrix import DenseMatrix

        if isinstance(other, DenseMatrix):
            if other.dtype != self.dtype:
                raise TypeError(
                    "self, B and d all need to be of same dtype, either np.float64 or "
                    f"np.float32. This matrix is of type {self.dtype}, B is of type "
                    f"{other.dtype}.")
            Bd = other._dev_c()
            A = self._dev()
            if (rows is not None and 0 < D.nlen(rows) <= ROW_LIST_FRACTION_K3 * self.shape[0]
                    and 0 < A.data.numel() < 2**31 and self.shape[1] <= 128 * 32):
                res = xs.csr_dense_sandwich_rows(A, Bd, d, rows)
                if L_cols is not None:
                    res = res[L_cols.to(torch.int64)]
                if R_cols is not None:
                    res = res[:, R_cols.to(torch.int64)]
                return res
            if self.shape[0] > 0 and self._dev().data.numel() > 0 and (
                    rows is None or self._values_finite()):
                d = D.masked_d(d, rows)
                if (A.data.numel() <= SORTED_K3_NNZ_PER_ROW * self.shape[0] and self.shape[1] >= 1024
                        and xs.ell_supported(Bd)):
                    res = xs.csc_dense_sandwich_sorted(A, Bd, d)
                    if L_cols is not None:
                        res = res[L_cols.to(torch.int64)]
                    if R_cols is not None:
                        res = res[:, R_cols.to(torch.int64)]
                    return res
                wide = Bd.m > 64 and xs.ell_supported(Bd)
                ent = self._ent() if wide else None
                lg = self._lg() if (wide and ent is None) else None
                ell = None
                if ent is None and lg is None and xs.ell_supported(Bd):
                    ell = self._ell(wide=Bd.m > 64)
                if ent is not None and colsum_box is not None:
                    res, cs = xs.csr_dense_sandwich_ent(ent, Bd, d, want_colsum=True)
                    colsum_box.append(cs if L_cols is None else cs[L_cols.to(torch.int64)])
                elif ent is not None:
                    res = xs.csr_dense_sandwich_ent(ent, Bd, d)
                elif lg is not None and colsum_box is not None:
                    res, cs = xs.csr_dense_sandwich_lg(lg, Bd, d, want_colsum=True)
                    colsum_box.append(cs if L_cols is None else cs[L_cols.to(torch.int64)])
                elif lg is not None:
                    res = xs.csr_dense_sandwich_lg(lg, Bd, d)
                elif ell is not None:
                    res = xs.csr_dense_sandwich_ell(ell, Bd, d)
                else:
                    res = xs.csr_dense_sandwich_slab(self._slab(), Bd, d)
                if L_cols is not None:
                    res = res[L_cols.to(torch.int64)]
                if R_cols is not None:
                    res = res[:, R_cols.to(torch.int64)]
                return res
            return xs.csr_dense_sandwich(self._dev(), Bd, d, rows, L_cols, R_cols)
        if isinstance(other, CategoricalMatrix):
            return other._cross_sandwich_dev(self, d, rows, R_cols, L_cols).T
        raise TypeError

    def _cross_sandwich(self, other, d, rows, L_cols=None, R_cols=None):
        on_dev = D.is_dev(d)
        if not on_dev:
            d = np.asarray(d)
        check_sandwich_compatible(self, d)
        res = self._cross_sandwich_dev(
            other, D.to_dev(d), D.idx_dev(normalize_index(rows, self.shape[0])),
            D.idx_dev(normalize_index(L_cols, self.shape[1])),
            D.idx_dev(normalize_index(R_cols, other.shape[1])))
        return res if on_dev else D.to_host(res)

    def sandwich_dense(self, B, d, rows, L_cols, R_cols):
        from .dense_matrix import DenseMatrix

        Bm = B if isinstance(B, DenseMatrix) else DenseMatrix(B)
        return self._cross_sandwich(Bm, d, rows, L_cols, R_cols)

    def _matvec_dev(self, vec, rows, cols, out, transpose):
        fn = xs.csc_rmatvec if transpose else xs.csr_matvec
        return fn(self._dev(), vec, rows, cols, out)

    def _matvec_helper(self, vec, rows, cols, out, transpose):
        on_dev = D.is_dev(vec)
        if not on_dev:
            vec = np.asarray(vec)
        check_matvec_dimensions(self, vec, transpose)
        n, m = self.shape
        rows_n = normalize_index(rows, n)
        cols_n = normalize_index(cols, m)
        if rows_n is not None and len(rows_n) == n:
            rows_n = None
        if cols_n is not None and len(cols_n) == m:
            cols_n = None
        tdt = D.torch_dtype(self.dtype)
        v_dev = D.to_dev(vec, tdt)
        rd, cd = D.idx_dev(rows_n), D.idx_dev(cols_n)
        if v_dev.ndim == 1:
            res = self._matvec_dev(v_dev, rd, cd, None, transpose)
        else:
            res = xs.csr_matvec_multi(self._dev(), v_dev, rd, cd, transpose)
        if not on_dev:
            res = D.to_host(res)
        if out is None:
            return res
        if transpose and cols_n is not None:
            out[cols_n if not D.is_dev(out) else D.idx_dev(cols_n, torch.int64)] += res
        else:
            out += res
        return out

    def matvec(self, vec, cols=None, out=None):
        check_matvec_out_shape(self, out)
        return self._matvec_helper(vec, None, cols, out, False)

    def transpose_matvec(self, vec, rows=None, cols=None, out=None):
        check_transpose_matvec_out_shape(self, out)
        return self._matvec_helper(vec, rows, cols, out, True)

    def _get_col_stds(self, weights, col_means):
        tdt = D.torch_dtype(self.dtype)
        ex2 = D.to_host(xs.transpose_square_dot_weights(self._dev(),
                                                        D.to_dev(np.asarray(weights), tdt)))
# ... 4 lines not shown
```

tabmat_amd/split_matrix.py:

```python
from __future__ import annotations

import os
import warnings
from collections.abc import Sequence
from typing import Optional, Union

import numpy as np
import torch
from scipy import sparse as sps

from . import _device as D
from .categorical_matrix import CategoricalMatrix
from .dense_matrix import DenseMatrix
from .ext import split as xsplit
from .ext.dense import dense_sandwich_matvec as xd_smv
from .matrix_base import MatrixBase
from .sparse_matrix import SparseMatrix
from .standardized_mat import StandardizedMatrix
from .util import (
    check_matvec_dimensions,
    check_matvec_out_shape,
    check_sandwich_compatible,
    check_transpose_matvec_out_shape,
    collapse_identity,
    normalize_index,
    set_up_rows_or_cols,
)


ROW_LIST_FRACTION_CATSPARSE = 0.04
DIAG_FROM_PAIRS = True
CAT_PAIRS_FUSED = os.environ.get("TABMAT_AMD_CAT_PAIRS", "1") != "0"
FULL_THEN_SELECT = float(os.environ.get("TABMAT_AMD_FULL_THEN_SELECT", "0.5"))
FULL_RESULT_MAX_BYTES = 256 << 20
FULL_UNSELECTED_SHARE = 0.2
FULL_THEN_SELECT_MV = 0.0
NARROW_COLS = int(os.environ.get("TABMAT_AMD_NARROW_COLS", "128"))
from . import categorical_matrix as _cm
from . import sparse_matrix as _spm


class _Centering:
    NARROW_GROUP = 1 << 20

    def __init__(self, vec):
        self.vec = dict(vec)
        self.cs_centered = set()
        self.groups = None

    def get(self, b):
        return self.vec.get(b)


class _Xtv:

    def __init__(self, v):
        self.v = v
        self.out = {}


def as_tabmat(a):
    if isinstance(a, (MatrixBase, StandardizedMatrix)):
        return a
    if sps.issparse(a):
        return SparseMatrix(a.tocsc(copy=False))
    if isinstance(a, np.ndarray):
        return DenseMatrix(a)
    raise ValueError(f"Cannot convert type {type(a)} to Matrix.")


def hstack(tup: Sequence) -> MatrixBase:
    mats = [as_tabmat(a) for a in tup]
    if not mats:
        raise ValueError("Need at least one array to concatenate.")
    if all(isinstance(m, SparseMatrix) for m in mats):
        return SparseMatrix(sps.hstack([m.array_csc for m in mats]))
    if all(isinstance(m, DenseMatrix) for m in mats):
        return DenseMatrix(np.hstack([m.toarray() for m in mats]))
    return SplitMatrix(mats)


def _merge_same_kind(matrices, indices):
    for kind in (DenseMatrix, SparseMatrix):
        which = [i for i, m in enumerate(matrices) if isinstance(m, kind)]
        if len(which) <= 1:
            continue
        gidx = np.concatenate([indices[i] for i in which])
        order = np.argsort(gidx)
        names = np.concatenate([np.array(matrices[i]._colnames, dtype=object) for i in which])
        terms = np.concatenate([np.array(matrices[i]._terms, dtype=object) for i in which])
        if kind is DenseMatrix:
            merged = DenseMatrix(np.hstack([matrices[i].toarray() for i in which])[:, order])
        else:
            merged = SparseMatrix(sps.hstack([matrices[i].array_csc for i in which]).tocsc()[:, order])
        merged._colnames = names[order].tolist()
        merged._terms = terms[order].tolist()
# ... 222 lines not shown

    def _pairs_pos_sel(self, plan, cols_host, split=None):
        key = np.asarray(cols_host).tobytes()
        hit = self.__dict__.get("_pos_sel")
        if hit is not None and hit[0] == key:
            return hit[1]
        pos_h, sub_h = split if split is not None else self._split_col_subsets(cols_host)[:2]
        pf = np.full(int(plan.pstart[-1]), -1, dtype=np.int64)
        for a, i in enumerate(plan.cat_ids):
            if len(sub_h[i]):
                pf[int(plan.pstart[a]) + np.asarray(sub_h[i], dtype=np.int64)] = pos_h[i]
        t = D.to_dev(pf)
        self.__dict__["_pos_sel"] = (key, t)
        return t

    def _sandwich_xtd_dev(self, d, rows, cols_host, center=None):
        colsum = [None] * len(self.matrices)
        out = self._sandwich_dev(d, rows, cols_host, colsum=colsum, center=center)
        pos_d, sub_d, n_cols = self._sandwich_plan(cols_host)
        xtd = D.zeros((n_cols,), torch.float64)
        cmask = None if center is None else torch.zeros((n_cols,), dtype=torch.bool, device=xtd.device)
        for i, (mi, pd, sd) in enumerate(zip(self.matrices, pos_d, sub_d)):
            if sd is not None and D.nlen(sd) == 0:
                continue
            cs = colsum[i]
            if cs is None:
                if isinstance(mi, CategoricalMatrix):
                    full = D.zeros((mi.shape[1],), d.dtype)
                    mi._transpose_matvec_dev(d, rows, sd, full)
                    cs = full if sd is None else full[sd.to(torch.int64)]
                else:
                    cs = mi._matvec_dev(d, rows, sd, None, True)
            elif center is not None and i in center.cs_centered:
                cmask[pd] = True
            xtd[pd] = cs.to(torch.float64)
        if center is not None:
            return out, xtd, cmask, center.groups
        return out, xtd

    FUSED_LEVELS = 496
    FUSED_CATS = 8

    def _cat_groups(self, cat_ids):
        groups, cur, tot = [], [], 0
        for i in cat_ids:
            k = self.matrices[i].shape[1]
            if k > self.FUSED_LEVELS:
                continue
            if cur and (len(cur) == self.FUSED_CATS or tot + k > self.FUSED_LEVELS):
                groups.append(cur)
                cur, tot = [], 0
            cur.append(i)
            tot += k
        if cur:
            groups.append(cur)
        return groups

    def _cat_pairs_plan(self):
        plan = self.__dict__.get("_cp_plan", False)
        if plan is False:
            plan = None
            ids = [i for i, m in enumerate(self.matrices)
                   if isinstance(m, CategoricalMatrix) and m.shape[1] > 0]
            if len(ids) >= 1:
                pos = self._full_dev_indices()
                plan = xsplit.CatPairsPlan([(i, self.matrices[i].shape[1]) for i in ids],
                                           [pos[i] for i in ids])
            self.__dict__["_cp_plan"] = plan
        return plan

    def _cat_hist_plan(self):
        plan = self.__dict__.get("_ch_plan", False)
        if plan is False:
            plan = None
            ids = [i for i, m in enumerate(self.matrices)
                   if isinstance(m, CategoricalMatrix) and m.shape[1] > 0 and m.shape[0] > 0]
            if len(ids) >= 2:
                pos = self._full_dev_indices()
                plan = xsplit.CatPairsPlan([(i, self.matrices[i].shape[1]) for i in ids],
                                           [pos[i] for i in ids], diag_only=True)
            self.__dict__["_ch_plan"] = plan
        return plan

    def _fused_cats(self, mw, cats, cat_ids, d_eff, rows, total, budget, d_rows=None):
        if isinstance(mw, DenseMatrix) and xsplit.multi_cat_dense_wide_ok(cats, mw._dev_c()):
            if rows is not None and D.nlen(rows) <= 0.5 * self.shape[0]:
                return xsplit.multi_cat_dense_sandwich(cats, d_rows, mw._dev_c(), rows)
            return xsplit.multi_cat_dense_sandwich(cats, d_eff, mw._dev_c())
        if isinstance(mw, DenseMatrix) and xsplit.multi_cat_dense_tile_ok(cats, mw._dev_c()):
            return xsplit.multi_cat_dense_sandwich(cats, d_eff, mw._dev_c())
        if isinstance(mw, DenseMatrix):
            if xsplit.cat_dense_sorted_ok(mw._dev_c()):
                return None
            from .ext import sparse as xs

            oh, inv = self._onehot_slab(cat_ids)
            return xs.csr_dense_sandwich_slab(oh, mw._dev_c(), d_eff)[inv]
        if (isinstance(mw, SparseMatrix) and total * 33 <= budget and rows is not None
                and 0 < D.nlen(rows) <= ROW_LIST_FRACTION_CATSPARSE * self.shape[0]
                and 0 < mw._dev().data.numel() < 2**31):
            return xsplit.multi_cat_sparse_sandwich_rows(cats, d_rows, mw._dev(), rows)
        if (isinstance(mw, SparseMatrix) and total * 33 <= budget
                and mw._dev().data.numel() > 0 and (rows is None or mw._values_finite())):
            ent = None
            if len(cats) <= 8 and (getattr(mw, "_entblk", None) or any(
                    isinstance(mo, DenseMatrix) and mo.shape[1] > 64 and mo.dtype == mw.dtype
                    for mo in self.matrices)):
                ent = mw._ent()
            if ent is not None:
                pk_cache = self.__dict__.setdefault("_packed_codes", {})
                key = tuple(cat_ids)
                if key not in pk_cache:
                    pk_cache[key] = xsplit.pack_codes(cats)
                return xsplit.multi_cat_sparse_sandwich_ent(cats, d_eff, ent, pk_cache[key])
            return xsplit.multi_cat_sparse_sandwich(cats, d_eff, mw._slab())
        return None

    def _parts(self):
        parts = self.__dict__.get("_row_parts", False)
        if parts is False:
            parts = None
            big = [m for m in self.matrices
                   if isinstance(m, SparseMatrix) and m._dev().data.numel() >= _spm.PART_NNZ]
            if big:
                n = self.shape[0]
                lead = max(big, key=lambda m: m._dev().data.numel())
                ptr = lead._dev().indptr
                nnz = int(ptr[-1].item())
                k = -(-nnz // max(1, int(0.8 * _spm.PART_NNZ)))
                while True:
                    targets = torch.arange(1, k, device=ptr.device, dtype=torch.int64) * nnz // k
                    cuts = [0] + torch.searchsorted(ptr, targets).clamp_(0, n).tolist() + [n]
                    cuts = sorted(set(int(c) for c in cuts))
                    ok = all(int((m._dev().indptr[cuts[1:]] - m._dev().indptr[cuts[:-1]]).max().item())
                             < _spm.PART_NNZ for m in big)
                    if ok or k >= n:
                        break
                    k += 1
                parts = [(a, b, self[a:b]) for a, b in zip(cuts[:-1], cuts[1:]) if b > a]
            self.__dict__["_row_parts"] = parts
        return parts

    def _sandwich_parts(self, parts, d, rows, cols_host, colsum, center=None):
        out = None
        for a, b, part in parts:
            r = None
            if rows is not None:
                r64 = rows.to(torch.int64)
                sel = r64[(r64 >= a) & (r64 < b)]
                if sel.numel() == 0:
                    continue
                r = (sel - a).to(torch.int32)
            cs = [None] * len(self.matrices) if colsum is not None else None
            sub_cen = None if center is None else _Centering(center.vec)
            res = part._sandwich_dev(d[a:b], r, cols_host, None, cs, center=sub_cen)
            if sub_cen is not None:
                center.groups = sub_cen.groups
            if sub_cen is not None and colsum is not None:
                dsum = (d[a:b] if r is None else d[a:b][r.to(torch.int64)]).sum(dtype=torch.float64)
                _, sub_p, _ = self._sandwich_plan(cols_host)
                for i in sub_cen.cs_centered:
                    if cs[i] is not None and sub_cen.get(i) is not None:
                        cv = sub_cen.get(i).to(torch.float64)
                        if sub_p[i] is not None:
                            cv = cv[sub_p[i].to(torch.int64)]
                        cs[i] = cs[i].to(torch.float64) + cv * dsum
            out = res if out is None else out + res
            if colsum is not None:
                for i, c in enumerate(cs):
                    if c is None:
                        colsum[i] = False
                    elif colsum[i] is not False:
                        colsum[i] = c if colsum[i] is None else colsum[i] + c
        if colsum is not None:
            for i, c in enumerate(colsum):
                if c is False:
                    colsum[i] = None
        if out is None:
            _, _, n_cols = self._sandwich_plan(cols_host)
            out = D.zeros((n_cols, n_cols), torch.float64)
        return out

    def _full_product_pays(self, sub_h) -> bool:
        p = self.shape[1]
        if p * p * 8 > FULL_RESULT_MAX_BYTES:
            return False
        n = max(self.shape[0], 1)
        tot = unsel = 0.0
        for b, mb in enumerate(self.matrices):
            if isinstance(mb, DenseMatrix):
                wb = float(mb.shape[1])
            elif isinstance(mb, SparseMatrix):
                nnz = mb._devblk.data.numel() if mb._devblk is not None else mb._host().nnz
                wb = max(1.0, float(nnz) / n)
            else:
                wb = 1.0 + mb.shape[1] / 256.0
            tot += wb
            if len(sub_h[b]) == 0:
                unsel += wb
        return unsel <= FULL_UNSELECTED_SHARE * tot

    def _full_product_pays_cols(self, cols_host) -> bool:
        key = np.asarray(cols_host).tobytes()
        hit = self.__dict__.get("_fpp_cache")
        if hit is None or hit[0] != key:
            hit = self.__dict__["_fpp_cache"] = (key, self._full_product_pays(self._split_col_subsets(cols_host)[1]))
        return hit[1]

    def _narrow_plan(self, cols_host):
        key = np.asarray(cols_host).tobytes()
        hit = self.__dict__.get("_narrow_cache")
        if hit is not None and hit[0] == key:
            return hit[1]
        nar = None
        pos_h, sub_h, n_cols = self._split_col_subsets(cols_host)
        mats = self.matrices
        noncat = [b for b, mb in enumerate(mats) if not isinstance(mb, CategoricalMatrix)]
        cat = [b for b, mb in enumerate(mats) if isinstance(mb, CategoricalMatrix) and len(sub_h[b]) > 0]
        w = sum(len(sub_h[b]) for b in noncat)
        itemsize = np.dtype(self.dtype).itemsize
        if (noncat and 0 < w <= NARROW_COLS and self.shape[0] > 0
                and all(isinstance(mats[b], (DenseMatrix, SparseMatrix)) and mats[b].dtype == self.dtype
                        for b in noncat)
                and any(len(sub_h[b]) < mats[b].shape[1] for b in noncat)
                and self.shape[0] * (w + 1) * itemsize * 4 < torch.cuda.mem_get_info()[0]):
            w_pad = w + (w & 1)
            t0, parts = 0, []
            sel = np.zeros(n_cols, dtype=np.int64)
            for b in noncat:
                s = len(sub_h[b])
                if s == 0:
                    continue
                sc = np.asarray(sub_h[b], dtype=np.int32)
                if isinstance(mats[b], SparseMatrix):
                    rws, vls, bstart, _, col_bptr = mats[b]._dev().csc_blocks()
                    cd = D.idx_dev(sc, torch.int64)
                    seg = torch.stack([bstart[col_bptr[cd]], bstart[col_bptr[cd + 1]]], dim=1).contiguous()
                    mx = int((seg[:, 1] - seg[:, 0]).max().item()) if s else 0
                    tcol = D.to_dev(t0 + np.arange(s, dtype=np.int32))
                    parts.append((b, t0, s, (rws, vls, seg, tcol, mx)))
                else:
                    parts.append((b, t0, s, D.to_dev(sc)))
                sel[np.asarray(pos_h[b], dtype=np.int64)] = t0 + np.arange(s)
                t0 += s
            off, cat_off, cat_sub = w_pad, {}, {}
            for i in cat:
                cat_off[i] = off
                if len(sub_h[i]):
                    sel[np.asarray(pos_h[i], dtype=np.int64)] = off + np.asarray(sub_h[i], dtype=np.int64)
                    cat_sub[i] = D.idx_dev(sub_h[i], torch.int64)
                off += mats[i].shape[1]
            indices = [np.arange(w_pad)] + [cat_off[i] + np.arange(mats[i].shape[1]) for i in cat]
            nar = dict(w=w, w_pad=w_pad, parts=parts, cat=cat, cat_sub=cat_sub, indices=indices,
                       sel=D.to_dev(sel), tmp=None, n_cols=n_cols)
        elif noncat and w > NARROW_COLS and FULL_THEN_SELECT <= 1.0 and self._full_product_pays(sub_h):
            nar = "wide"
        self.__dict__["_narrow_cache"] = (key, nar)
        return nar

    def _sandwich_narrow(self, nar, d, rows, colsum, center=None):
        from .ext import dense as xd
        from .ext import sparse as xs
        from .ext._types import DenseDev

        n = self.shape[0]
        T = torch.zeros((n, nar["w_pad"]), dtype=d.dtype, device=d.device)
        for b, t0, s, idx in nar["parts"]:
            mb = self.matrices[b]
            if isinstance(mb, SparseMatrix):
                xs.csc_densify_cols(*idx, T)
            else:
                xd.dense_gather_cols(mb._dev(), idx, T, t0)
        tmp = nar["tmp"]
        if tmp is None:
            tmp = nar["tmp"] = SplitMatrix([DenseMatrix(T)] + [self.matrices[i] for i in nar["cat"]],
                                           nar["indices"])
        dm = tmp.matrices[0]
        dm._devblk = DenseDev(T, n, nar["w_pad"], 0)
        sub_cen = None
        if center is not None:
            tc = torch.zeros((nar["w_pad"],), dtype=d.dtype, device=d.device)
            for b, t0, s, idx in nar["parts"]:
                if center.get(b) is not None:
                    tc[t0:t0 + s] = center.get(b)[idx.to(torch.int64)]
            sub_cen = _Centering({0: tc})
        try:
            cs_tmp = [None] * len(tmp.matrices) if colsum is not None else None
            full = tmp._sandwich_dev(d, rows, None, None, cs_tmp, center=sub_cen)
        finally:
            dm._devblk = None
        if colsum is not None:
            if cs_tmp[0] is not None:
                for b, t0, s, _ in nar["parts"]:
                    colsum[b] = cs_tmp[0][t0:t0 + s]
                    if sub_cen is not None and 0 in sub_cen.cs_centered:
                        center.cs_centered.add(b)
            for k, i in enumerate(nar["cat"]):
                if cs_tmp[1 + k] is not None and i in nar["cat_sub"]:
                    colsum[i] = cs_tmp[1 + k][nar["cat_sub"][i]]
        if center is not None:
            g = torch.full_like(nar["sel"], -1, dtype=torch.int32)
            g[nar["sel"] < nar["w_pad"]] = _Centering.NARROW_GROUP
            center.groups = g
        sel = nar["sel"]
        return full.index_select(0, sel).index_select(1, sel)

    def _sandwich_dev(self, d, rows, cols_host, plan=None, colsum=None, center=None, xtv=None):
        if cols_host is not None and len(cols_host) >= FULL_THEN_SELECT * self.shape[1] \
                and len(cols_host) > 0 and self._full_product_pays_cols(cols_host):
            pos_d, sub_d, n_cols = plan if plan is not None else self._sandwich_plan(cols_host)
            cs_full = [None] * len(self.matrices) if colsum is not None else None
            full = self._sandwich_dev(d, rows, None, None, cs_full, center=center, xtv=xtv)
            if colsum is not None:
                for i, c in enumerate(cs_full):
                    if c is not None:
                        colsum[i] = c if sub_d[i] is None else c[sub_d[i].to(torch.int64)]
            cd = self._cols_dev64(cols_host)
            return full.index_select(0, cd).index_select(1, cd)
        parts = self._parts()
        if parts is not None:
            return self._sandwich_parts(parts, d, rows, cols_host, colsum, center)
        if cols_host is not None and plan is None and NARROW_COLS > 0:
            nar = self._narrow_plan(cols_host)
            if nar == "wide":
                cs_full = [None] * len(self.matrices) if colsum is not None else None
                full = self._sandwich_dev(d, rows, None, None, cs_full, center=center, xtv=xtv)
                if colsum is not None:
                    _, sub_sel, _ = self._sandwich_plan(cols_host)
                    for i, c in enumerate(cs_full):
                        if c is not None:
                            colsum[i] = c if sub_sel[i] is None else c[sub_sel[i].to(torch.int64)]
                cd = self._cols_dev64(cols_host)
                return full.index_select(0, cd).index_select(1, cd)
            if nar is not None and d.dtype == D.torch_dtype(self.dtype):
                return self._sandwich_narrow(nar, d, rows, colsum, center)
        pos_d, sub_d, n_cols = plan if plan is not None else self._sandwich_plan(cols_host)
        out = D.zeros((n_cols, n_cols), torch.float64)
        mats = self.matrices
        empty = [sd is not None and D.nlen(sd) == 0 for sd in sub_d]
        done = set()
        return self._sandwich_terms(d, rows, cols_host, colsum, out, pos_d, sub_d, empty, done, center,
                                    xtv if cols_host is None else None)

    def _sandwich_terms(self, d, rows, cols_host, colsum, out, pos_d, sub_d, empty, done, center=None, xtv=None):
        from .ext import dense as xd

        mats = self.matrices
        cat_ids = [i for i, m in enumerate(mats) if isinstance(m, CategoricalMatrix) and not empty[i]
                   and m.shape[1] > 0]
        budget = (128 * 1024) // 8
        groups = self._cat_groups(cat_ids)
        if groups:
            d_eff = D.masked_d(d, rows)
        for grp in groups:
            cats = [(mats[i]._dev(), mats[i].shape[1], mats[i].drop_first) for i in grp]
            total = sum(c[1] for c in cats)
            offs = np.concatenate([[0], np.cumsum([c[1] for c in cats])])
            for w, mw in enumerate(mats):
                if empty[w] or mw.dtype != self.dtype or d.dtype != D.torch_dtype(self.dtype):
                    continue
                stacked = self._fused_cats(mw, cats, grp, d_eff, rows, total, budget, d)
                if stacked is None:
                    continue
                whole = cols_host is None and len(grp) > 1
                if whole:
                    cache = self.__dict__.setdefault("_group_pos", {})
                    gpos = cache.get(tuple(grp))
                    if gpos is None:
                        gpos = cache[tuple(grp)] = torch.cat([pos_d[i] for i in grp])
                    xsplit.scatter_block(stacked.contiguous(), gpos, pos_d[w], out, mirror=True)
                for ci, i in enumerate(grp):
                    res = stacked[int(offs[ci]):int(offs[ci + 1])]
                    if (colsum is not None and colsum[w] is None and not mats[i].drop_first
                            and not mats[i]._has_missings):
                        cs = res.sum(dim=0)
                        colsum[w] = cs if sub_d[w] is None else cs[sub_d[w].to(torch.int64)]
                    if not whole:
                        res = CategoricalMatrix._restrict(res, sub_d[i], sub_d[w])
                        xsplit.scatter_block(res.contiguous(), pos_d[i], pos_d[w], out, mirror=True)
                    done.add((min(i, w), max(i, w)))
        big = [i for i in cat_ids if mats[i].shape[1] > self.FUSED_LEVELS]
        if len(big) >= 2 and len(big) <= 16 and d.dtype == D.torch_dtype(self.dtype):
            cats = [(mats[i]._dev(), mats[i].shape[1], mats[i].drop_first) for i in big]
            offs = np.concatenate([[0], np.cumsum([c[1] for c in cats])])
            d_big = None
            for w, mw in enumerate(mats):
                if (empty[w] or not isinstance(mw, DenseMatrix) or mw.dtype != self.dtype
                        or not xsplit.multi_cat_dense_tile_ok(cats, mw._dev_c())):
                    continue
                if d_big is None:
                    d_big = D.masked_d(d, rows)
                stacked = xsplit.multi_cat_dense_sandwich(cats, d_big, mw._dev_c())
                for ci, i in enumerate(big):
                    res = stacked[int(offs[ci]):int(offs[ci + 1])]
                    if (colsum is not None and colsum[w] is None and not mats[i].drop_first
                            and not mats[i]._has_missings):
                        cs = res.sum(dim=0)
                        colsum[w] = cs if sub_d[w] is None else cs[sub_d[w].to(torch.int64)]
                    res = CategoricalMatrix._restrict(res, sub_d[i], sub_d[w])
                    xsplit.scatter_block(res.contiguous(), pos_d[i], pos_d[w], out, mirror=True)
                    done.add((min(i, w), max(i, w)))
        cat_diag = {}
        diag_scattered = set()
        det = _cm.DETERMINISTIC
        plan = self._cat_pairs_plan() if CAT_PAIRS_FUSED and not det else None
        if (plan is not None and plan.n_pairs > 0
                and d.dtype in (torch.float32, torch.float64)
                and d.dtype == D.torch_dtype(self.dtype)):
            cl = [(mats[i]._dev(), mats[i].shape[1], mats[i].drop_first) for i in plan.cat_ids]
            pos_sel = None if cols_host is None else self._pairs_pos_sel(plan, cols_host)
            tables = xsplit.multi_cat_pairs(plan, cl, d, rows, out, pos=pos_sel)
            for i, j, toff, li, lj, stride in plan.pairs:
                if i == j:
                    if not empty[i]:
                        full = tables[toff:toff + (li - 1) * stride + 1:stride]
                        if sub_d[i] is not None and colsum is not None:
                            full = full[sub_d[i].to(torch.int64)]
                        cat_diag[i] = full.to(d.dtype)
                        diag_scattered.add(i)
                else:
                    done.add((i, j))
        complete = [isinstance(m, CategoricalMatrix) and not m.drop_first and not m._has_missings
                    and sub_d[k] is None and not empty[k] for k, m in enumerate(mats)]
        for i, mi in enumerate(mats):
            if empty[i] or not isinstance(mi, CategoricalMatrix):
                continue
            for j in range(i + 1, len(mats)):
                if empty[j] or not isinstance(mats[j], CategoricalMatrix) or (i, j) in done:
                    continue
                res = mi._cross_sandwich_dev(mats[j], d, rows, sub_d[i], sub_d[j])
                xsplit.scatter_block(res.contiguous(), pos_d[i], pos_d[j], out, mirror=True)
                done.add((i, j))
                if DIAG_FROM_PAIRS and not det and complete[j] and i not in cat_diag:
                    cat_diag[i] = res.sum(dim=1)
                if DIAG_FROM_PAIRS and not det and complete[i] and j not in cat_diag:
                    cat_diag[j] = res.sum(dim=0)
        for i, mi in enumerate(mats):
            if empty[i]:
                continue
            if isinstance(mi, CategoricalMatrix):
                diag = cat_diag[i] if i in cat_diag else mi._sandwich_diag_dev(d, rows, sub_d[i])
                if colsum is not None:
                    colsum[i] = diag
                if i not in diag_scattered:
                    xsplit.scatter_block(diag, pos_d[i], pos_d[i], out, diag=True)
            elif (xtv is not None and colsum is None and center is None and isinstance(mi, DenseMatrix)
                  and sub_d[i] is None and (both := mi._sandwich_xtv_dev(d, xtv.v, rows)) is not None):
                res, xtv.out[i] = both
                xsplit.scatter_block(res, pos_d[i], pos_d[i], out)
            elif (colsum is not None and colsum[i] is None and isinstance(mi, DenseMatrix)
                  and rows is None and sub_d[i] is None
                  and (both := mi._sandwich_xtd_dev(d, cen_i := (center.get(i) if center else None))) is not None):
                res, colsum[i] = both
                if cen_i is not None:
                    center.cs_centered.add(i)
                xsplit.scatter_block(res, pos_d[i], pos_d[i], out)
            elif isinstance(mi, DenseMatrix) and center is not None and center.get(i) is not None:
                res = mi._sandwich_dev(d, rows, sub_d[i], center=center.get(i))
                xsplit.scatter_block(res, pos_d[i], pos_d[i], out)
            else:
                res = mi._sandwich_dev(d, rows, sub_d[i])
                xsplit.scatter_block(res, pos_d[i], pos_d[i], out)
        for i, mi in enumerate(mats):
            if empty[i]:
                continue
            for j in range(i + 1, len(mats)):
                if empty[j] or (i, j) in done:
                    continue
                si, di = (i, j) if isinstance(mi, SparseMatrix) else (j, i)
                if (colsum is not None and colsum[si] is None and isinstance(mats[si], SparseMatrix)
                        and isinstance(mats[di], DenseMatrix)):
                    box = []
                    res = mats[si]._cross_sandwich_dev(mats[di], d, rows, sub_d[si], sub_d[di],
                                                       colsum_box=box)
                    if box:
                        colsum[si] = box[0]
                    if si != i:
                        res = res.T
                else:
                    res = mi._cross_sandwich_dev(mats[j], d, rows, sub_d[i], sub_d[j])
                xsplit.scatter_block(res.contiguous(), pos_d[i], pos_d[j], out, mirror=True)
        return out

    def sandwich_graph(self, d, rows=None, cols=None):
        from .graph import CapturedProduct

        check_sandwich_compatible(self, d)
        rows_d = D.idx_dev(normalize_index(rows, self.shape[0]))
        cols_n = collapse_identity(normalize_index(cols, self.shape[1]), self.shape[1])
        plan = self._sandwich_plan(cols_n)
        return CapturedProduct(lambda dd: self._sandwich_dev(dd, rows_d, cols_n, plan), d)

    def sandwich(self, d, rows=None, cols=None):
        on_dev = D.is_dev(d)
        if not on_dev:
            d = np.asarray(d)
        check_sandwich_compatible(self, d)
        rows_n = normalize_index(rows, self.shape[0])
        cols_n = collapse_identity(normalize_index(cols, self.shape[1]), self.shape[1])
        out = self._sandwich_dev(D.to_dev(d), D.idx_dev(rows_n), cols_n)
        return out if on_dev else D.to_host(out)

    def sandwich_and_transpose_matvec(self, d, v, rows=None, cols=None):
        from .matrix_base import _check_1d

        _check_1d(v)
        d_dev_side, v_dev_side = D.is_dev(d), D.is_dev(v)
        if not d_dev_side:
            d = np.asarray(d)
        if not v_dev_side:
            v = np.asarray(v)
        check_sandwich_compatible(self, d)
        check_matvec_dimensions(self, v, transpose=True)
        rows_n = normalize_index(rows, self.shape[0])
        cols_n = collapse_identity(normalize_index(cols, self.shape[1]), self.shape[1])
        tdt = D.torch_dtype(self.dtype)
        v_dev = D.to_dev(v, tdt)
        acc = None
        if (tdt == torch.float64 and not _cm.DETERMINISTIC
                and (rows_n is None or len(rows_n) < self.shape[0])):
            acc = _Xtv(v_dev)
        H = self._sandwich_dev(D.to_dev(d), D.idx_dev(rows_n), cols_n, xtv=acc)
        g, _ = self._transpose_matvec_dev(v_dev, rows_n, cols_n, done=None if acc is None else acc.out)
        if not v_dev_side:
            g = D.to_host(g)
            if np.issubdtype(v.dtype, np.floating):
                g = g.astype(np.result_type(self.dtype, v.dtype), copy=False)
        return (H if d_dev_side else D.to_host(H)), g

    def sandwich_matvec(self, d, u, rows=None, cols=None):
        from .matrix_base import _smv_args, _smv_compose

        a = _smv_args(self, d, u, rows, cols, h_dtype=np.float64)
        if a.trivial is not None:
            return a.finish(a.trivial)
        tdt = D.torch_dtype(self.dtype)
        res = None
        if (rows is None and cols is None) or self._blocks_finite():
            res = self._smv_dev(a.d_masked(tdt), a.u_full(tdt))
        if res is None:
            return a.finish(_smv_compose(self, a))
        g = res[0]
        if a.cols is not None:
            g = g[self._cols_dev64(a.cols)]
        return a.finish(g)

    def _sdiag_dev(self, d, rows, cols_host=None, centers=None, want_s1=False):
        p = self.shape[1]
        parts = self._parts()
        if parts is not None:
            s2 = D.zeros((p,), torch.float64)
            s1 = D.zeros((p,), torch.float64) if want_s1 else None
            for a, b, part in parts:
                r = None
                if rows is not None:
                    r64 = rows.to(torch.int64)
                    sel = r64[(r64 >= a) & (r64 < b)]
                    if sel.numel() == 0:
                        continue
                    r = (sel - a).to(torch.int32)
                p2, p1 = part._sdiag_dev(d[a:b], r, cols_host, centers, want_s1)
                s2 += p2
                if want_s1:
                    s1 += p1
# ... 214 lines not shown
```

Measured before the change: 1059 GB/s.

## Defer per-block partial reductions into a single fused sandwich finish kernel

Adds partial-only variants of the multi-cat dense, multi-cat sparse, CSR-dense cross and sparse blocked sandwich kernels. These write per-block partials into a shared arena and register a job descriptor instead of reducing, untiling and scattering each term separately. A new finish kernel then processes all jobs in one launch, reducing the partials and scattering them straight into the output matrix. The aim is to remove many small reduce, untile and scatter launches and intermediate buffers per sandwich. The cost is a new arena, extra job bookkeeping on the host, and more complex code paths.

```diff
diff --git a/include/tabmat_hip.h b/include/tabmat_hip.h
--- a/include/tabmat_hip.h
+++ b/include/tabmat_hip.h
@@ -506,6 +506,54 @@
                          const int64_t *ci, double *out, int64_t p, int mirror, int diag,
                          void *stream);
 
+int tm_sandwich_finish_job_words(void);
+int tm_sandwich_finish_f32(const int64_t *jobs, int n_jobs, int64_t n_blocks, double *out, int64_t p, void *stream);
+int tm_sandwich_finish_f64(const int64_t *jobs, int n_jobs, int64_t n_blocks, double *out, int64_t p, void *stream);
+int tm_csr_dense_sandwich_ent_partial_f32(const float *vals, const uint16_t *meta, const uint32_t *bstart, int64_t n,
+                                          int64_t m, const float *B, int64_t r, const float *d, float *partials,
+                                          int64_t cap, int64_t *job, void *stream);
+int tm_csr_dense_sandwich_ent_partial_f64(const double *vals, const uint16_t *meta, const uint32_t *bstart, int64_t n,
+                                          int64_t m, const double *B, int64_t r, const double *d, double *partials,
+                                          int64_t cap, int64_t *job, void *stream);
+int tm_sparse_sandwich_blocks_u8_partial_f32(const float *cm_data, const uint8_t *cm_col8, const int32_t *cptr,
+                                             int64_t n, int64_t m, int64_t nnz, const int32_t *blocks,
+                                             const int32_t *wg_tab, int n_wg, int max_nb,
+                                             const int32_t *slot_used, const float *d, float *partials,
+                                             int64_t cap, int64_t *job, void *stream);
+int tm_sparse_sandwich_blocks_u8_partial_f64(const double *cm_data, const uint8_t *cm_col8, const int32_t *cptr,
+                                             int64_t n, int64_t m, int64_t nnz, const int32_t *blocks,
+                                             const int32_t *wg_tab, int n_wg, int max_nb,
+                                             const int32_t *slot_used, const double *d, double *partials,
+                                             int64_t cap, int64_t *job, void *stream);
+int tm_sparse_sandwich_blocks_p12_partial_f32(const float *cm_data, const uint8_t *cm_col8, const int32_t *cptr,
+                                              int64_t n, int64_t m, int64_t nnz, const int32_t *blocks12,
+                                              const int32_t *wg_tab, int n_wg, int max_nb,
+                                              const int32_t *slot_used, const float *d, float *partials,
+                                              int64_t cap, int64_t *job, void *stream);
+int tm_sparse_sandwich_blocks_p12_partial_f64(const double *cm_data, const uint8_t *cm_col8, const int32_t *cptr,
+                                              int64_t n, int64_t m, int64_t nnz, const int32_t *blocks12,
+                                              const int32_t *wg_tab, int n_wg, int max_nb,
+                                              const int32_t *slot_used, const double *d, double *partials,
+                                              int64_t cap, int64_t *job, void *stream);
+int tm_multi_cat_dense_sandwich_partial_f32(const void *const *h_codes, const int64_t *h_ncols,
+                                            const int32_t *h_drop_first, int n_cats, int64_t n, const float *d,
+                                            const float *M, int64_t M_ncol, float *partials, int64_t cap,
+                                            int64_t *job, void *stream);
+int tm_multi_cat_dense_sandwich_partial_f64(const void *const *h_codes, const int64_t *h_ncols,
+                                            const int32_t *h_drop_first, int n_cats, int64_t n, const double *d,
+                                            const double *M, int64_t M_ncol, double *partials, int64_t cap,
+                                            int64_t *job, void *stream);
+int tm_multi_cat_sparse_sandwich_entp_partial_f32(const void *const *h_codes, const int64_t *h_ncols,
+                                                  const int32_t *h_drop_first, int n_cats, int64_t n, const float *d,
+                                                  const float *vals, const uint16_t *meta, const uint32_t *bstart,
+                                                  int64_t n_slots, int64_t mk, const uint32_t *packed,
+                                                  float *partials, int64_t cap, int64_t *job, void *stream);
+int tm_multi_cat_sparse_sandwich_entp_partial_f64(const void *const *h_codes, const int64_t *h_ncols,
+                                                  const int32_t *h_drop_first, int n_cats, int64_t n, const double *d,
+                                                  const double *vals, const uint16_t *meta, const uint32_t *bstart,
+                                                  int64_t n_slots, int64_t mk, const uint32_t *packed,
+                                                  double *partials, int64_t cap, int64_t *job, void *stream);
+
 int tm_sparse_sandwich_chunked_rows_f32(const float *cm_data, const int32_t *cm_indices,
                                         const int32_t *row_ranges, int64_t n_sel, int64_t m,
                                         int64_t nnz, const float *d_sel, float *out, void *stream);
diff --git a/tabmat_amd/csrc/cat.hip b/tabmat_amd/csrc/cat.hip
--- a/tabmat_amd/csrc/cat.hip
+++ b/tabmat_amd/csrc/cat.hip
@@ -1,6 +1,7 @@
 #include <algorithm>
 
 #include "common.hpp"
+#include "finish.hpp"
 #include "reduce.hpp"
 
 namespace tmh {
@@ -1305,14 +1306,16 @@
 static int run_multi_cat_dense(const void *const *h_codes, const int64_t *h_ncols,
                                const int32_t *h_drop, int n_cats, int64_t n, const F *d, const F *M,
                                int64_t m, int order_f, F *out, hipStream_t st,
-                               const int32_t *rows = nullptr, int64_t n_rows = 0) {
+                               const int32_t *rows = nullptr, int64_t n_rows = 0, const PartialReq *pr = nullptr) {
     CatSet cs;
     int rc = make_catset(h_codes, h_ncols, h_drop, n_cats, &cs);
     if (rc) return rc;
     const int64_t total = (int64_t)cs.total * m;
+    if (pr) finish_empty_job(*pr);
     if (total == 0) return TM_OK;
     if (rows != nullptr) n = n_rows;
     if (n == 0) {
+        if (pr) return TM_OK;
         TM_HIP(hipMemsetAsync(out, 0, sizeof(F) * (size_t)total, st));
         return TM_OK;
     }
@@ -1332,10 +1335,16 @@
             nblk = ceil_div(n, rpb);
             const size_t tmp_bytes = ((sizeof(F) * (size_t)(n_parts * stride) + 255) / 256) * 256;
             void *wsv = nullptr;
-            rc = get_workspace(tmp_bytes + sizeof(F) * (size_t)(n_parts * nblk * stride) + 256, &wsv, st);
-            if (rc) return rc;
-            F *tmp = reinterpret_cast<F *>(wsv);
-            F *ws = reinterpret_cast<F *>(reinterpret_cast<char *>(wsv) + tmp_bytes);
+            F *tmp = nullptr, *ws = nullptr;
+            if (pr) {
+                if (!finish_fill_job(*pr, n_parts, nblk, stride, FL_PANEL, TJW, cs.total, m, nullptr)) return TM_OK;
+                ws = reinterpret_cast<F *>(pr->buf);
+            } else {
+                rc = get_workspace(tmp_bytes + sizeof(F) * (size_t)(n_parts * nblk * stride) + 256, &wsv, st);
+                if (rc) return rc;
+                tmp = reinterpret_cast<F *>(wsv);
+                ws = reinterpret_cast<F *>(reinterpret_cast<char *>(wsv) + tmp_bytes);
+            }
             auto gow = [&](auto kern) -> int {
                 TM_HIP(hipFuncSetAttribute(reinterpret_cast<const void *>(kern),
                                            hipFuncAttributeMaxDynamicSharedMemorySize, (int)lds_w));
@@ -1356,7 +1365,7 @@
             else if (n_cats == 6) rc = gow(&multi_cat_dense_wide_kernel<F, 6>);
             else if (n_cats == 7) rc = gow(&multi_cat_dense_wide_kernel<F, 7>);
             else rc = gow(&multi_cat_dense_wide_kernel<F, 8>);
-            if (rc) return rc;
+            if (rc || pr) return rc;
             rc = launch_reduce_partials<F>(ws, stride, (int)nblk, (int)n_parts, tmp, n_parts * stride,
                                            false, st);
             if (rc) return rc;
@@ -1366,8 +1375,8 @@
             return TM_OK;
         }
     }
-    if (rows != nullptr) {
-        set_error("multi_cat_dense: the row-list form needs the wide-load path");
+    if (rows != nullptr || pr != nullptr) {
+        set_error("multi_cat_dense: the row-list and partial-only forms need the wide-load path");
         return TM_EUNSUPPORTED;
     }
     int TJ = 64;
@@ -1535,13 +1544,16 @@
 static int run_multi_cat_sparse_ent(const void *const *h_codes, const int64_t *h_ncols, const int32_t *h_drop,
                                     int n_cats, int64_t n, const F *d, const F *vals, const unsigned short *meta,
                                     const unsigned *bstart, int64_t mk, F *out, hipStream_t st,
-                                    const unsigned *packed = nullptr, int64_t n_slots = 0) {
+                                    const unsigned *packed = nullptr, int64_t n_slots = 0,
+                                    const PartialReq *pr = nullptr) {
     CatSet cs;
     int rc = make_catset(h_codes, h_ncols, h_drop, n_cats, &cs);
     if (rc) return rc;
     const int64_t total = (int64_t)cs.total * mk;
+    if (pr) finish_empty_job(*pr);
     if (total == 0) return TM_OK;
     if (n == 0) {
+        if (pr) return TM_OK;
         TM_HIP(hipMemsetAsync(out, 0, sizeof(F) * (size_t)total, st));
         return TM_OK;
     }
@@ -1564,10 +1576,16 @@
     nblk = ceil_div(n_slabs, spb);
     const size_t tmp_bytes = ((sizeof(F) * (size_t)(n_pairs * stride) + 255) / 256) * 256;
     void *wsv = nullptr;
-    rc = get_workspace(tmp_bytes + sizeof(F) * (size_t)((int64_t)n_pairs * nblk * stride) + 256, &wsv, st);
-    if (rc) return rc;
-    F *tmp = reinterpret_cast<F *>(wsv);
-    F *ws = reinterpret_cast<F *>(reinterpret_cast<char *>(wsv) + tmp_bytes);
+    F *tmp = nullptr, *ws = nullptr;
+    if (pr) {
+        if (!finish_fill_job(*pr, n_pairs, nblk, stride, FL_PANEL, GC, cs.total, mk, nullptr)) return TM_OK;
+        ws = reinterpret_cast<F *>(pr->buf);
+    } else {
+        rc = get_workspace(tmp_bytes + sizeof(F) * (size_t)((int64_t)n_pairs * nblk * stride) + 256, &wsv, st);
+        if (rc) return rc;
+        tmp = reinterpret_cast<F *>(wsv);
+        ws = reinterpret_cast<F *>(reinterpret_cast<char *>(wsv) + tmp_bytes);
+    }
     auto kern = n_cats == 1   ? &multi_cat_sparse_ent_kernel<F, 1>
                 : n_cats == 2 ? &multi_cat_sparse_ent_kernel<F, 2>
                 : n_cats == 3 ? &multi_cat_sparse_ent_kernel<F, 3>
@@ -1617,6 +1635,7 @@
         prof_end(st);
         TM_LAUNCH_CHECK();
     }
+    if (pr) return TM_OK;
     rc = launch_reduce_partials<F>(ws, stride, (int)nblk, n_pairs, tmp, (int64_t)n_pairs * stride, false, st);
     if (rc) return rc;
     hipLaunchKernelGGL((multi_cat_untile_kernel<F>), dim3((unsigned)ceil_div(total, 256)), dim3(256), 0, st, tmp,
@@ -1838,6 +1857,44 @@
                                           int64_t n_slots, int64_t mk, const uint32_t *packed, double *out, void *stream) {
     return run_multi_cat_sparse_ent<double>(h_codes, h_ncols, h_drop_first, n_cats, n, d, vals, meta, bstart, mk,
                                             out, as_stream(stream), packed, n_slots);
+}
+int tm_multi_cat_dense_sandwich_partial_f32(const void *const *h_codes, const int64_t *h_ncols,
+                                            const int32_t *h_drop_first, int n_cats, int64_t n, const float *d,
+                                            const float *M, int64_t M_ncol, float *partials, int64_t cap,
+                                            int64_t *job, void *stream) {
+    TM_REQUIRE(job != nullptr, "job is required");
+    const PartialReq pr{partials, cap, job};
+    return run_multi_cat_dense<float>(h_codes, h_ncols, h_drop_first, n_cats, n, d, M, M_ncol, 0, nullptr,
+                                      as_stream(stream), nullptr, 0, &pr);
+}
+int tm_multi_cat_dense_sandwich_partial_f64(const void *const *h_codes, const int64_t *h_ncols,
+                                            const int32_t *h_drop_first, int n_cats, int64_t n, const double *d,
+                                            const double *M, int64_t M_ncol, double *partials, int64_t cap,
+                                            int64_t *job, void *stream) {
+    TM_REQUIRE(job != nullptr, "job is required");
+    const PartialReq pr{partials, cap, job};
+    return run_multi_cat_dense<double>(h_codes, h_ncols, h_drop_first, n_cats, n, d, M, M_ncol, 0, nullptr,
+                                       as_stream(stream), nullptr, 0, &pr);
+}
+int tm_multi_cat_sparse_sandwich_entp_partial_f32(const void *const *h_codes, const int64_t *h_ncols,
+                                                  const int32_t *h_drop_first, int n_cats, int64_t n, const float *d,
+                                                  const float *vals, const uint16_t *meta, const uint32_t *bstart,
+                                                  int64_t n_slots, int64_t mk, const uint32_t *packed,
+                                                  float *partials, int64_t cap, int64_t *job, void *stream) {
+    TM_REQUIRE(job != nullptr, "job is required");
+    const PartialReq pr{partials, cap, job};
+    return run_multi_cat_sparse_ent<float>(h_codes, h_ncols, h_drop_first, n_cats, n, d, vals, meta, bstart, mk,
+                                           nullptr, as_stream(stream), packed, n_slots, &pr);
+}
+int tm_multi_cat_sparse_sandwich_entp_partial_f64(const void *const *h_codes, const int64_t *h_ncols,
+                                                  const int32_t *h_drop_first, int n_cats, int64_t n, const double *d,
+                                                  const double *vals, const uint16_t *meta, const uint32_t *bstart,
+                                                  int64_t n_slots, int64_t mk, const uint32_t *packed,
+                                                  double *partials, int64_t cap, int64_t *job, void *stream) {
+    TM_REQUIRE(job != nullptr, "job is required");
+    const PartialReq pr{partials, cap, job};
+    return run_multi_cat_sparse_ent<double>(h_codes, h_ncols, h_drop_first, n_cats, n, d, vals, meta, bstart, mk,
+                                            nullptr, as_stream(stream), packed, n_slots, &pr);
 }
 int tm_multi_cat_sparse_sandwich_slab_f32(const void *const *h_codes, const int64_t *h_ncols,
                                           const int32_t *h_drop_first, int n_cats, int64_t n,
diff --git a/tabmat_amd/csrc/common.hpp b/tabmat_amd/csrc/common.hpp
--- a/tabmat_amd/csrc/common.hpp
+++ b/tabmat_amd/csrc/common.hpp
@@ -66,6 +66,10 @@
 inline hipStream_t as_stream(void *s) { return reinterpret_cast<hipStream_t>(s); }
 
 inline int64_t ceil_div(int64_t a, int64_t b) { return (a + b - 1) / b; }
+
+inline int reduce_waves(int64_t stride, int64_t n_parts, int64_t nb) {
+    return (ceil_div(stride, 64) * n_parts < 1024 && nb > 16) ? 16 : 4;
+}
 
 typedef double lds_acc_t;
 
diff --git a/tabmat_amd/csrc/finish.hip b/tabmat_amd/csrc/finish.hip
--- /dev/null
+++ b/tabmat_amd/csrc/finish.hip
@@ -0,0 +1,103 @@
+#include "finish.hpp"
+
+namespace tmh {
+
+template <typename F>
+__global__ __launch_bounds__(FINISH_THREADS) void sandwich_finish_kernel(const int64_t *__restrict__ jobs,
+                                                                         int n_jobs, double *__restrict__ out,
+                                                                         int64_t p) {
+    constexpr int WAVES = FINISH_THREADS / 64;
+    __shared__ double red[WAVES][64];
+    const int lane = threadIdx.x & 63;
+    const int wave = threadIdx.x >> 6;
+    int jn = 0;
+    for (int k = 1; k < n_jobs; ++k)
+        if ((int64_t)blockIdx.x >= jobs[(int64_t)k * FJ_WORDS + FJ_FIRST]) jn = k;
+    const int64_t *job = jobs + (int64_t)jn * FJ_WORDS;
+    const int64_t lb = (int64_t)blockIdx.x - job[FJ_FIRST];
+    const int64_t stride = job[FJ_STRIDE];
+    const int nb = (int)job[FJ_NB];
+    const int nw = (int)job[FJ_NW];
+    const int n_parts = (int)job[FJ_NPARTS];
+    const int groups = WAVES / nw;
+    const int64_t gpp = (stride + 64 * groups - 1) / (64 * groups);
+    const int part = (int)(lb / gpp);
+    const int g = wave / nw, w = wave % nw;
+    const int64_t e = ((lb % gpp) * groups + g) * 64 + lane;
+    const bool live = lb < job[FJ_NBLOCKS] && part < n_parts && e < stride;
+    double acc = 0.0;
+    if (live) {
+        const int32_t *used = reinterpret_cast<const int32_t *>((uintptr_t)job[FJ_USED]);
+        if (used) used += (int64_t)part * nb;
+        const F *src = reinterpret_cast<const F *>((uintptr_t)job[FJ_PTR]) + ((int64_t)part * nb) * stride + e;
+        const int64_t step = (int64_t)nw * stride;
+        const F *q = src + (int64_t)w * stride;
+        int b = w;
+        for (; b + 7 * nw < nb; b += 8 * nw, q += 8 * step) {
+            F x[8];
+#pragma unroll
+            for (int u = 0; u < 8; ++u)
+                x[u] = (!used || used[b + u * nw]) ? __builtin_nontemporal_load(q + u * step) : F(0);
+#pragma unroll
+            for (int u = 0; u < 8; ++u) acc += (double)x[u];
+        }
+        for (; b < nb; b += nw, q += step)
+            if (!used || used[b]) acc += (double)__builtin_nontemporal_load(q);
+    }
+    red[wave][lane] = acc;
+    __syncthreads();
+    if (!live || w != 0) return;
+    double s = 0.0;
+    for (int k = 0; k < nw; k += 4) {
+        const int r = g * nw + k;
+        s += (red[r][lane] + red[r + 1][lane]) + (red[r + 2][lane] + red[r + 3][lane]);
+    }
+    const double v = (double)(F)s;
+    const int64_t nr = job[FJ_NR], nc = job[FJ_NC];
+    int64_t i, j;
+    bool mirror = (job[FJ_FLAGS] & 1) != 0;
+    if (job[FJ_LAYOUT] == FL_TRI128) {
+        int I = 0;
+        while ((I + 1) * (I + 2) / 2 <= part) ++I;
+        const int J = part - I * (I + 1) / 2;
+        i = (int64_t)I * 128 + e / 128;
+        j = (int64_t)J * 128 + e % 128;
+        if (j > i) return;
+        mirror = i != j;
+    } else {
+        const int64_t tj = job[FJ_TJ];
+        i = e / tj;
+        j = (int64_t)part * tj + e % tj;
+    }
+    if (i >= nr || j >= nc) return;
+    const int64_t r = reinterpret_cast<const int64_t *>((uintptr_t)job[FJ_POS_R])[i];
+    const int64_t c = reinterpret_cast<const int64_t *>((uintptr_t)job[FJ_POS_C])[j];
+    if ((uint64_t)r >= (uint64_t)p || (uint64_t)c >= (uint64_t)p) return;
+    out[r * p + c] = v;
+    if (mirror) out[c * p + r] = v;
+}
+
+template <typename F>
+static int run_sandwich_finish(const int64_t *jobs, int n_jobs, int64_t n_blocks, double *out, int64_t p,
+                               hipStream_t st) {
+    TM_REQUIRE(n_jobs >= 0 && n_blocks >= 0 && p >= 0, "negative size");
+    if (n_jobs == 0 || n_blocks == 0) return TM_OK;
+    TM_REQUIRE(jobs != nullptr && out != nullptr, "jobs and out are required");
+    TM_REQUIRE(n_blocks < (1ll << 31), "epilogue grid too large");
+    hipLaunchKernelGGL((sandwich_finish_kernel<F>), dim3((unsigned)n_blocks), dim3(FINISH_THREADS), 0, st, jobs,
+                       n_jobs, out, p);
+    TM_LAUNCH_CHECK();
+    return TM_OK;
+}
+
+}
+
+extern "C" {
+int tm_sandwich_finish_job_words(void) { return tmh::FJ_WORDS; }
+int tm_sandwich_finish_f32(const int64_t *jobs, int n_jobs, int64_t n_blocks, double *out, int64_t p, void *stream) {
+    return tmh::run_sandwich_finish<float>(jobs, n_jobs, n_blocks, out, p, tmh::as_stream(stream));
+}
+int tm_sandwich_finish_f64(const int64_t *jobs, int n_jobs, int64_t n_blocks, double *out, int64_t p, void *stream) {
+    return tmh::run_sandwich_finish<double>(jobs, n_jobs, n_blocks, out, p, tmh::as_stream(stream));
+}
+}
diff --git a/tabmat_amd/csrc/finish.hpp b/tabmat_amd/csrc/finish.hpp
--- /dev/null
+++ b/tabmat_amd/csrc/finish.hpp
@@ -0,0 +1,64 @@
+#pragma once
+#include "common.hpp"
+
+namespace tmh {
+
+enum FinishWord {
+    FJ_PTR = 0,
+    FJ_NPARTS,
+    FJ_NB,
+    FJ_STRIDE,
+    FJ_LAYOUT,
+    FJ_TJ,
+    FJ_NR,
+    FJ_NC,
+    FJ_USED,
+    FJ_NW,
+    FJ_POS_R,
+    FJ_POS_C,
+    FJ_FLAGS,
+    FJ_NBLOCKS,
+    FJ_FIRST,
+    FJ_NEED,
+    FJ_WORDS
+};
+
+enum FinishLayout {
+    FL_PANEL = 0,
+    FL_TRI128 = 1
+};
+
+constexpr int FINISH_THREADS = 1024;
+
+struct PartialReq {
+    void *buf;
+    int64_t cap;
+    int64_t *job;
+};
+
+inline bool finish_fill_job(const PartialReq &pr, int64_t n_parts, int64_t nb, int64_t stride, int layout,
+                            int64_t tj, int64_t nr, int64_t nc, const int32_t *used) {
+    int64_t *j = pr.job;
+    for (int w = 0; w < FJ_WORDS; ++w) j[w] = 0;
+    j[FJ_NPARTS] = n_parts;
+    j[FJ_NB] = nb;
+    j[FJ_STRIDE] = stride;
+    j[FJ_LAYOUT] = layout;
+    j[FJ_TJ] = tj;
+    j[FJ_NR] = nr;
+    j[FJ_NC] = nc;
+    j[FJ_USED] = (int64_t)reinterpret_cast<uintptr_t>(used);
+    const int nw = reduce_waves(stride, n_parts, nb);
+    j[FJ_NW] = nw;
+    j[FJ_NBLOCKS] = n_parts * ceil_div(stride, 64 * (FINISH_THREADS / 64 / nw));
+    j[FJ_NEED] = n_parts * nb * stride;
+    if (pr.buf == nullptr || pr.cap < j[FJ_NEED]) return false;
+    j[FJ_PTR] = (int64_t)reinterpret_cast<uintptr_t>(pr.buf);
+    return true;
+}
+
+inline void finish_empty_job(const PartialReq &pr) {
+    for (int w = 0; w < FJ_WORDS; ++w) pr.job[w] = 0;
+}
+
+}
diff --git a/tabmat_amd/csrc/reduce.hpp b/tabmat_amd/csrc/reduce.hpp
--- a/tabmat_amd/csrc/reduce.hpp
+++ b/tabmat_amd/csrc/reduce.hpp
@@ -39,7 +39,7 @@
 inline int launch_reduce_partials(const F *ws, int64_t stride, int nb, int n_parts, F *out,
                                   int64_t out_elems, bool accumulate, hipStream_t st) {
     dim3 grid((unsigned)ceil_div(stride, 64), (unsigned)n_parts);
-    const bool small = (int64_t)grid.x * grid.y < 1024 && nb > 16;
+    const bool small = reduce_waves(stride, n_parts, nb) == 16;
     if (small) {
         if (accumulate)
             hipLaunchKernelGGL((reduce_partials_kernel<F, true, 16>), grid, dim3(1024), 0, st, ws,
diff --git a/tabmat_amd/csrc/sparse_blocks.hip b/tabmat_amd/csrc/sparse_blocks.hip
--- a/tabmat_amd/csrc/sparse_blocks.hip
+++ b/tabmat_amd/csrc/sparse_blocks.hip
@@ -1,6 +1,7 @@
 #include <algorithm>
 
 #include "common.hpp"
+#include "finish.hpp"
 #include "reduce.hpp"
 
 namespace tmh {
@@ -202,9 +203,12 @@
 template <typename F, bool U8 = false, bool D12 = false>
 static int run_sparse_sandwich_blocks(const F *data, const int32_t *ind, const int32_t *cptr, int64_t n,
                                       int64_t m, int64_t nnz, const int32_t *blocks, const int32_t *wg_tab,
-                                      int n_wg, int max_nb, const F *d, F *out, hipStream_t st) {
+                                      int n_wg, int max_nb, const F *d, F *out, hipStream_t st,
+                                      const PartialReq *pr = nullptr, const int32_t *slot_used = nullptr) {
+    if (pr) finish_empty_job(*pr);
     if (m == 0) return TM_OK;
     if (n == 0 || nnz == 0 || n_wg == 0) {
+        if (pr) return TM_OK;
         TM_HIP(hipMemsetAsync(out, 0, sizeof(F) * (size_t)(m * m), st));
         return TM_OK;
     }
@@ -218,11 +222,19 @@
     const size_t tmp_bytes = (sizeof(F) * (size_t)n_parts * TS * TS + 255) / 256 * 256;
     const size_t ws_bytes = sizeof(F) * (size_t)n_parts * (size_t)max_nb * TS * TS;
     void *wsv = nullptr;
-    int rc = get_workspace(tmp_bytes + ws_bytes + 256, &wsv, st);
-    if (rc) return rc;
-    F *tmp = reinterpret_cast<F *>(wsv);
-    F *ws = reinterpret_cast<F *>(reinterpret_cast<char *>(wsv) + tmp_bytes);
-    TM_HIP(hipMemsetAsync(ws, 0, ws_bytes, st));
+    int rc = TM_OK;
+    F *tmp = nullptr, *ws = nullptr;
+    if (pr) {
+        TM_REQUIRE(slot_used != nullptr, "the partial-only form needs the mask of the written slots");
+        if (!finish_fill_job(*pr, n_parts, max_nb, (int64_t)TS * TS, FL_TRI128, TS, m, m, slot_used)) return TM_OK;
+        ws = reinterpret_cast<F *>(pr->buf);
+    } else {
+        rc = get_workspace(tmp_bytes + ws_bytes + 256, &wsv, st);
+        if (rc) return rc;
+        tmp = reinterpret_cast<F *>(wsv);
+        ws = reinterpret_cast<F *>(reinterpret_cast<char *>(wsv) + tmp_bytes);
+        TM_HIP(hipMemsetAsync(ws, 0, ws_bytes, st));
+    }
     auto kern = &sparse_sandwich_blocks_kernel<F, U8, D12>;
     TM_HIP(hipFuncSetAttribute(reinterpret_cast<const void *>(kern),
                                hipFuncAttributeMaxDynamicSharedMemorySize, (int)lds));
@@ -233,6 +245,7 @@
                        max_nb, ws, wg_log_ptr());
     prof_end(st);
     TM_LAUNCH_CHECK();
+    if (pr) return TM_OK;
     rc = launch_reduce_partials<F>(ws, (int64_t)TS * TS, max_nb, n_parts, tmp, (int64_t)n_parts * TS * TS,
                                    false, st);
     if (rc) return rc;
@@ -295,4 +308,20 @@
                                                                tmh::as_stream(stream));
 }
 
-}
+#define TM_K2B_PARTIAL(NAME, F, ...)                                                                              \
+    int NAME(const F *cm_data, const uint8_t *cm_col8, const int32_t *cptr, int64_t n, int64_t m, int64_t nnz,   \
+             const int32_t *blocks, const int32_t *wg_tab, int n_wg, int max_nb, const int32_t *slot_used,        \
+             const F *d, F *partials, int64_t cap, int64_t *job, void *stream) {                                  \
+        TM_REQUIRE(job != nullptr, "job is required");                                                            \
+        const tmh::PartialReq pr{partials, cap, job};                                                             \
+        return tmh::run_sparse_sandwich_blocks<F, __VA_ARGS__>(cm_data, reinterpret_cast<const int32_t *>(cm_col8), \
+                                                               cptr, n, m, nnz, blocks, wg_tab, n_wg, max_nb, d,  \
+                                                               nullptr, tmh::as_stream(stream), &pr, slot_used);   \
+    }
+TM_K2B_PARTIAL(tm_sparse_sandwich_blocks_u8_partial_f32, float, true)
+TM_K2B_PARTIAL(tm_sparse_sandwich_blocks_u8_partial_f64, double, true)
+TM_K2B_PARTIAL(tm_sparse_sandwich_blocks_p12_partial_f32, float, true, true)
+TM_K2B_PARTIAL(tm_sparse_sandwich_blocks_p12_partial_f64, double, true, true)
+#undef TM_K2B_PARTIAL
+
+}
diff --git a/tabmat_amd/csrc/sparse_ent.hip b/tabmat_amd/csrc/sparse_ent.hip
--- a/tabmat_amd/csrc/sparse_ent.hip
+++ b/tabmat_amd/csrc/sparse_ent.hip
@@ -1,4 +1,5 @@
 #include "common.hpp"
+#include "finish.hpp"
 #include "reduce.hpp"
 
 namespace tmh {
@@ -360,9 +361,11 @@
 
 template <typename F>
 static int run_csr_dense_ent(const F *vals, const uint16_t *meta, const uint32_t *bstart, int64_t n, int64_t m,
-                             const F *B, int64_t r, const F *d, F *out, F *colsum, hipStream_t st) {
+                             const F *B, int64_t r, const F *d, F *out, F *colsum, hipStream_t st,
+                             const PartialReq *pr = nullptr) {
     const int64_t nB = r;
     const int64_t total = m * nB;
+    if (pr) finish_empty_job(*pr);
     if (total == 0) return TM_OK;
     constexpr int VEC = 16 / (int)sizeof(F);
     if ((reinterpret_cast<uintptr_t>(B) & 15) != 0 || r % VEC != 0 || nB < VEC) {
@@ -383,6 +386,7 @@
     const int nz = (int)ceil_div(n_groups, EN_NW);
     const bool want_csum = colsum != nullptr;
     if (n_slabs == 0) {
+        if (pr) return TM_OK;
         TM_HIP(hipMemsetAsync(out, 0, sizeof(F) * (size_t)total, st));
         if (want_csum) TM_HIP(hipMemsetAsync(colsum, 0, sizeof(F) * (size_t)m, st));
         return TM_OK;
@@ -396,11 +400,18 @@
     const size_t part_bytes = (sizeof(F) * (size_t)((int64_t)n_parts * nblk * stride) + 255) / 256 * 256;
     const size_t csum_bytes = ((want_csum ? sizeof(F) * (size_t)(nblk * m) : 0) + 255) / 256 * 256 + 256;
     void *wsv = nullptr;
-    int rc = get_workspace(tmp_bytes + part_bytes + csum_bytes + 256, &wsv, st);
-    if (rc) return rc;
-    F *tmp = reinterpret_cast<F *>(wsv);
-    F *ws = reinterpret_cast<F *>(reinterpret_cast<char *>(wsv) + tmp_bytes);
-    F *ws_csum = reinterpret_cast<F *>(reinterpret_cast<char *>(wsv) + tmp_bytes + part_bytes);
+    int rc = TM_OK;
+    F *tmp = nullptr, *ws = nullptr, *ws_csum = nullptr;
+    if (pr) {
+        if (!finish_fill_job(*pr, n_parts, nblk, stride, FL_PANEL, EN_W, m, nB, nullptr)) return TM_OK;
+        ws = reinterpret_cast<F *>(pr->buf);
+    } else {
+        rc = get_workspace(tmp_bytes + part_bytes + csum_bytes + 256, &wsv, st);
+        if (rc) return rc;
+        tmp = reinterpret_cast<F *>(wsv);
+        ws = reinterpret_cast<F *>(reinterpret_cast<char *>(wsv) + tmp_bytes);
+        ws_csum = reinterpret_cast<F *>(reinterpret_cast<char *>(wsv) + tmp_bytes + part_bytes);
+    }
     const size_t lds = (size_t)EnLds<F>::TOTAL;
     auto kern = want_csum ? &csr_dense_ent_kernel<F, true> : &csr_dense_ent_kernel<F, false>;
     TM_HIP(hipFuncSetAttribute(reinterpret_cast<const void *>(kern),
@@ -411,6 +422,7 @@
                        reinterpret_cast<long long *>((uintptr_t)tune("ent_prof", 0)));
     prof_end(st);
     TM_LAUNCH_CHECK();
+    if (pr) return TM_OK;
     rc = launch_reduce_partials<F>(ws, stride, (int)nblk, n_parts, tmp, n_parts * stride, false, st);
     if (rc) return rc;
     hipLaunchKernelGGL((en_untile_kernel<F>), dim3((unsigned)ceil_div(total, 256)), dim3(256), 0, st, tmp, m,
@@ -441,4 +453,20 @@
                                   double *colsum, void *stream) {
     return tmh::run_csr_dense_ent<double>(vals, meta, bstart, n, m, B, r, d, out, colsum, tmh::as_stream(stream));
 }
-}
+int tm_csr_dense_sandwich_ent_partial_f32(const float *vals, const uint16_t *meta, const uint32_t *bstart, int64_t n,
+                                          int64_t m, const float *B, int64_t r, const float *d, float *partials,
+                                          int64_t cap, int64_t *job, void *stream) {
+    TM_REQUIRE(job != nullptr, "job is required");
+    const tmh::PartialReq pr{partials, cap, job};
+    return tmh::run_csr_dense_ent<float>(vals, meta, bstart, n, m, B, r, d, nullptr, nullptr, tmh::as_stream(stream),
+                                         &pr);
+}
+int tm_csr_dense_sandwich_ent_partial_f64(const double *vals, const uint16_t *meta, const uint32_t *bstart, int64_t n,
+                                          int64_t m, const double *B, int64_t r, const double *d, double *partials,
+                                          int64_t cap, int64_t *job, void *stream) {
+    TM_REQUIRE(job != nullptr, "job is required");
+    const tmh::PartialReq pr{partials, cap, job};
+    return tmh::run_csr_dense_ent<double>(vals, meta, bstart, n, m, B, r, d, nullptr, nullptr,
+                                          tmh::as_stream(stream), &pr);
+}
+}
diff --git a/tabmat_amd/ext/finish.py b/tabmat_amd/ext/finish.py
--- /dev/null
+++ b/tabmat_amd/ext/finish.py
@@ -0,0 +1,202 @@
+from __future__ import annotations
+
+import os
+
+import numpy as np
+import torch
+
+from .. import _device as D
+from .._lib import call, lib
+
+STEP_EPILOGUE = os.environ.get("TABMAT_AMD_STEP_EPILOGUE", "0") == "1"
+MAX_IDLE_ARENAS = 2
+
+J_PTR, J_NPARTS, J_POS_R, J_POS_C, J_FLAGS, J_NBLOCKS, J_FIRST, J_NEED = 0, 1, 10, 11, 12, 13, 14, 15
+_ALIGN = 64
+
+
+class PartialArena:
+
+    def __init__(self, dtype):
+        self.dtype = dtype
+        self.chunks = []
+        self._ci = self._off = 0
+        self._k = 0
+        self._plan = []
+        self.captured = False
+        self._jobs_key = None
+        self._jobs_dev = None
+
+    def nbytes(self) -> int:
+        return sum(c.numel() * c.element_size() for c in self.chunks)
+
+    def begin(self):
+        self._ci = self._off = self._k = 0
+        if torch.cuda.is_current_stream_capturing():
+            self.captured = True
+        if D.POISON:
+            for c in self.chunks:
+                c.fill_(float("nan"))
+
+    def run(self, launch):
+        job = np.zeros(_job_words(), dtype=np.int64)
+        k = self._k
+        self._k += 1
+        if k < len(self._plan):
+            self._ci, self._off = self._plan[k]
+        for attempt in range(2):
+            if self._ci < len(self.chunks):
+                c = self.chunks[self._ci]
+                launch(c.data_ptr() + self._off * c.element_size(), c.numel() - self._off, job.ctypes.data)
+            else:
+                launch(None, 0, job.ctypes.data)
+            if job[J_NPARTS] == 0:
+                return None
+            if job[J_PTR] != 0:
+                del self._plan[k:]
+                self._plan.append((self._ci, self._off))
+                self._off += -(-int(job[J_NEED]) // _ALIGN) * _ALIGN
+                return job
+            assert attempt == 0, "a partial-only entry point refused a buffer of the size it asked for"
+            need = -(-int(job[J_NEED]) // _ALIGN) * _ALIGN
+            self._ci += 1 if self._ci < len(self.chunks) else 0
+            while self._ci < len(self.chunks) and self.chunks[self._ci].numel() < need:
+                self._ci += 1
+            self._off = 0
+            if self._ci == len(self.chunks):
+                if torch.cuda.is_current_stream_capturing():
+                    raise RuntimeError("the partial arena of a sandwich step must be sized by a warm-up call "
+                                       "before the step is captured into a graph")
+                c = torch.empty((need,), dtype=self.dtype, device=D.require_gpu())
+                if D.POISON:
+                    c.fill_(float("nan"))
+                self.chunks.append(c)
+        raise AssertionError
+
+    def jobs_dev(self, jobs: np.ndarray) -> torch.Tensor:
+        key = jobs.tobytes()
+        if key != self._jobs_key:
+            self._jobs_dev = D.to_dev(jobs.reshape(-1))
+            self._jobs_key = key
+        return self._jobs_dev
+
+
+_WORDS = None
+
+
+def _job_words() -> int:
+    global _WORDS
+    if _WORDS is None:
+        _WORDS = int(lib().tm_sandwich_finish_job_words())
+    return _WORDS
+
+
+def arena_for(owner: dict, dtype) -> PartialArena:
+    arenas = owner.setdefault("_epi_arenas", {})
+    key = (D.stream_ptr(), dtype)
+    arena = arenas.pop(key, None)
+    if arena is None:
+        arena = PartialArena(dtype)
+    arenas[key] = arena
+    idle = [k for k, a in arenas.items() if not a.captured and k != key]
+    for k in idle[:max(0, len(idle) - (MAX_IDLE_ARENAS - 1))]:
+        del arenas[k]
+    return arena
+
+
+class StepEpilogue:
+
+    def __init__(self, arena: PartialArena, dtype):
+        self.arena = arena
+        self.dtype = dtype
+        self.jobs = []
+        self._keep = []
+        arena.begin()
+
+    def add(self, launch, pos_r, pos_c, mirror: bool) -> None:
+        job = self.arena.run(launch)
+        if job is None:
+            return
+        assert pos_r.dtype == torch.int64 and pos_c.dtype == torch.int64
+        assert pos_r.numel() >= job[6] and pos_c.numel() >= job[7], "one position per logical row / column"
+        job[J_POS_R], job[J_POS_C], job[J_FLAGS] = pos_r.data_ptr(), pos_c.data_ptr(), int(bool(mirror))
+        self._keep += [pos_r, pos_c]
+        self.jobs.append(job)
+
+    def launch(self, out) -> None:
+        if not self.jobs:
+            return
+        jobs = np.stack(self.jobs)
+        jobs[:, J_FIRST] = np.concatenate([[0], np.cumsum(jobs[:-1, J_NBLOCKS])])
+        n_blocks = int(jobs[:, J_NBLOCKS].sum())
+        assert out.dtype == torch.float64 and out.is_contiguous()
+        call(f"tm_sandwich_finish_{'f32' if self.dtype == torch.float32 else 'f64'}",
+             D.p(self.arena.jobs_dev(jobs)), len(self.jobs), n_blocks, D.p(out), out.shape[0], D.stream_ptr())
+        self.jobs = []
+
+
+def csr_dense_ent(epi: StepEpilogue, A, B, d, kpos, pos_b) -> None:
+    from . import sparse as xs
+
+    D.same_float("csr_dense_sandwich_ent", A.vals, B.buf, d)
+    epi.add(lambda ptr, cap, job: xs.call("tm_csr_dense_sandwich_ent_partial_" + D.fsuf(A.vals), D.p(A.vals),
+                                          D.p(A.meta), D.p(A.bstart), A.n, A.mk, D.p(B.buf), B.m, D.p(d), ptr, cap,
+                                          job, D.stream_ptr()),
+            kpos, pos_b, True)
+
+
+def k2b_slot_mask(wg_tab, n_parts: int, max_nb: int):
+    wt = wg_tab.detach().cpu().numpy().reshape(-1, 8)
+    mask = np.zeros((n_parts, max_nb), dtype=np.int32)
+    mask[wt[:, 0], wt[:, 1]] = 1
+    return mask
+
+
+def sparse_sandwich_blocks(epi: StepEpilogue, A, d, pos) -> bool:
+    from . import sparse as xs
+
+    if not xs.K2B_U8:
+        return False
+    D.same_float("sparse_sandwich_blocks", A.data, d)
+    cm_data, cm_c8, cptr = A.chunk_major()
+    blocks, wg_tab, max_nb = A.pair_blocks(d12=None)
+    form = "p12" if int(blocks.shape[1]) == 3 else "u8"
+    cache = A.__dict__.setdefault("_pb_used", {})
+    hit = cache.get(form)
+    if hit is None or hit[0] is not wg_tab:
+        nch = -(-A.m // 128)
+        hit = cache[form] = (wg_tab, D.to_dev(k2b_slot_mask(wg_tab, nch * (nch + 1) // 2, int(max_nb)).reshape(-1)))
+    used = hit[1]
+    epi.add(lambda ptr, cap, job: xs.call(f"tm_sparse_sandwich_blocks_{form}_partial_{D.fsuf(A.data)}", D.p(cm_data),
+                                          D.p(cm_c8), D.p(cptr), A.n, A.m, int(cm_data.numel()), D.p(blocks),
+                                          D.p(wg_tab), int(wg_tab.shape[0]), int(max_nb), D.p(used), D.p(d), ptr,
+                                          cap, job, D.stream_ptr()),
+            pos, pos, False)
+    return True
+
+
+def multi_cat_dense(epi: StepEpilogue, cats, d, mat_j, gpos, pos_j) -> None:
+    from . import split as xsplit
+
+    codes, ncols, drop, n = xsplit._cat_args(cats)
+    D.same_float("multi_cat_dense_sandwich", mat_j.buf, d)
+    epi.add(lambda ptr, cap, job: xsplit.call(f"tm_multi_cat_dense_sandwich_partial_{D.fsuf(mat_j.buf)}", codes, ncols, drop,
+                                       n, mat_j.n, D.p(d), D.p(mat_j.buf), mat_j.m, ptr, cap, job, D.stream_ptr()),
+            gpos, pos_j, True)
+
+
+def multi_cat_sparse_ent(epi: StepEpilogue, cats, d, E, packed, gpos, kpos) -> None:
+    from . import split as xsplit
+
+    codes, ncols, drop, n = xsplit._cat_args(cats)
+    D.same_float("multi_cat_sparse_sandwich_ent", E.vals, d)
+    epi.add(lambda ptr, cap, job: xsplit.call(f"tm_multi_cat_sparse_sandwich_entp_partial_{D.fsuf(E.vals)}", codes, ncols,
+                                       drop, n, E.n, D.p(d), D.p(E.vals), D.p(E.meta), D.p(E.bstart), E.n_slots(),
+                                       E.mk, D.p(packed), ptr, cap, job, D.stream_ptr()),
+            gpos, kpos, True)
+
+
+def kernel_col_pos(E, pos) -> torch.Tensor:
+    kpos = torch.full((E.mk,), -1, dtype=torch.int64, device=pos.device)
+    kpos[E.inv] = pos
+    return kpos
diff --git a/tabmat_amd/sparse_matrix.py b/tabmat_amd/sparse_matrix.py
--- a/tabmat_amd/sparse_matrix.py
+++ b/tabmat_amd/sparse_matrix.py
@@ -247,7 +247,7 @@
         t_narrow = 0.2e-3 + n * w * 4.5e-12 + nnz * w / max(mcols, 1) * 40e-12
         return t_narrow < 0.8 * t_full
 
-    def _sandwich_dev(self, d, rows, cols):
+    def _sandwich_dev(self, d, rows, cols, partial=None):
         parts = self._row_parts()
         if parts is not None:
             out = None
@@ -328,6 +328,8 @@
             bl = getattr(self, "_blocks_pay", None)
             if bl is None:
                 bl = self._blocks_pay = xs.blocks_sandwich_pays(A)
+            if bl and partial is not None and rows is None and cols is None and partial(A, d):
+                return None
             res = xs.sparse_sandwich_blocks(A, d) if bl else xs.sparse_sandwich_chunked(A, d)
             if cols is not None:
                 c64 = cols.to(torch.int64)
@@ -426,7 +428,7 @@
                                  D.idx_dev(normalize_index(cols, self.shape[1])))
         return res if on_dev else D.to_host(res)
 
-    def _cross_sandwich_dev(self, other, d, rows, L_cols, R_cols, colsum_box=None):
+    def _cross_sandwich_dev(self, other, d, rows, L_cols, R_cols, colsum_box=None, partial=None):
         from .categorical_matrix import CategoricalMatrix
         from .dense_matrix import DenseMatrix
 
@@ -466,6 +468,9 @@
                 if ent is not None and colsum_box is not None:
                     res, cs = xs.csr_dense_sandwich_ent(ent, Bd, d, want_colsum=True)
                     colsum_box.append(cs if L_cols is None else cs[L_cols.to(torch.int64)])
+                elif ent is not None and partial is not None and rows is None and L_cols is None and R_cols is None:
+                    partial(ent, Bd, d)
+                    return None
                 elif ent is not None:
                     res = xs.csr_dense_sandwich_ent(ent, Bd, d)
                 elif lg is not None and colsum_box is not None:
diff --git a/tabmat_amd/split_matrix.py b/tabmat_amd/split_matrix.py
--- a/tabmat_amd/split_matrix.py
+++ b/tabmat_amd/split_matrix.py
@@ -12,6 +12,7 @@
 from . import _device as D
 from .categorical_matrix import CategoricalMatrix
 from .dense_matrix import DenseMatrix
+from .ext import finish as xfinish
 from .ext import split as xsplit
 from .ext.dense import dense_sandwich_matvec as xd_smv
 from .matrix_base import MatrixBase
@@ -400,10 +401,13 @@
             self.__dict__["_ch_plan"] = plan
         return plan
 
-    def _fused_cats(self, mw, cats, cat_ids, d_eff, rows, total, budget, d_rows=None):
+    def _fused_cats(self, mw, cats, cat_ids, d_eff, rows, total, budget, d_rows=None, epi=None, w=None, pos_d=None):
         if isinstance(mw, DenseMatrix) and xsplit.multi_cat_dense_wide_ok(cats, mw._dev_c()):
             if rows is not None and D.nlen(rows) <= 0.5 * self.shape[0]:
                 return xsplit.multi_cat_dense_sandwich(cats, d_rows, mw._dev_c(), rows)
+            if epi is not None and total > 0 and mw.shape[0] > 0 and mw.shape[1] > 0:
+                xfinish.multi_cat_dense(epi, cats, d_eff, mw._dev_c(), self._group_positions(cat_ids, pos_d), pos_d[w])
+                return True
             return xsplit.multi_cat_dense_sandwich(cats, d_eff, mw._dev_c())
         if isinstance(mw, DenseMatrix) and xsplit.multi_cat_dense_tile_ok(cats, mw._dev_c()):
             return xsplit.multi_cat_dense_sandwich(cats, d_eff, mw._dev_c())
@@ -420,19 +424,51 @@
             return xsplit.multi_cat_sparse_sandwich_rows(cats, d_rows, mw._dev(), rows)
         if (isinstance(mw, SparseMatrix) and total * 33 <= budget
                 and mw._dev().data.numel() > 0 and (rows is None or mw._values_finite())):
-            ent = None
-            if len(cats) <= 8 and (getattr(mw, "_entblk", None) or any(
-                    isinstance(mo, DenseMatrix) and mo.shape[1] > 64 and mo.dtype == mw.dtype
-                    for mo in self.matrices)):
-                ent = mw._ent()
+            ent, packed = self._cat_sparse_ent(mw, cats, cat_ids)
+            if ent is not None and epi is not None and total > 0 and ent.m > 0 and ent.n > 0:
+                xfinish.multi_cat_sparse_ent(epi, cats, d_eff, ent, packed, self._group_positions(cat_ids, pos_d),
+                                             self._kernel_pos(w, ent, pos_d))
+                return True
             if ent is not None:
-                pk_cache = self.__dict__.setdefault("_packed_codes", {})
-                key = tuple(cat_ids)
-                if key not in pk_cache:
-                    pk_cache[key] = xsplit.pack_codes(cats)
-                return xsplit.multi_cat_sparse_sandwich_ent(cats, d_eff, ent, pk_cache[key])
+                return xsplit.multi_cat_sparse_sandwich_ent(cats, d_eff, ent, packed)
             return xsplit.multi_cat_sparse_sandwich(cats, d_eff, mw._slab())
         return None
+
+    def _cat_sparse_ent(self, mw, cats, cat_ids):
+        ent = None
+        if len(cats) <= 8 and (getattr(mw, "_entblk", None) or any(
+                isinstance(mo, DenseMatrix) and mo.shape[1] > 64 and mo.dtype == mw.dtype
+                for mo in self.matrices)):
+            ent = mw._ent()
+        if ent is None:
+            return None, None
+        pk_cache = self.__dict__.setdefault("_packed_codes", {})
+        key = tuple(cat_ids)
+        if key not in pk_cache:
+            pk_cache[key] = xsplit.pack_codes(cats)
+        return ent, pk_cache[key]
+
+    def _step_epilogue(self, d, rows, cols_host, colsum, center, xtv):
+        if (not xfinish.STEP_EPILOGUE or rows is not None or cols_host is not None or colsum is not None
+                or center is not None or xtv is not None or _cm.DETERMINISTIC
+                or d.dtype not in (torch.float32, torch.float64) or d.dtype != D.torch_dtype(self.dtype)):
+            return None
+        arena = xfinish.arena_for(self.__dict__, d.dtype)
+        return xfinish.StepEpilogue(arena, d.dtype)
+
+    def _group_positions(self, grp, pos_d):
+        cache = self.__dict__.setdefault("_group_pos", {})
+        gpos = cache.get(tuple(grp))
+        if gpos is None:
+            gpos = cache[tuple(grp)] = torch.cat([pos_d[i] for i in grp])
+        return gpos
+
+    def _kernel_pos(self, w, ent, pos_d):
+        cache = self.__dict__.setdefault("_epi_kpos", {})
+        hit = cache.get(w)
+        if hit is None or hit[0] is not ent:
+            hit = cache[w] = (ent, xfinish.kernel_col_pos(ent, pos_d[w]))
+        return hit[1]
 
     def _parts(self):
         parts = self.__dict__.get("_row_parts", False)
@@ -459,7 +495,7 @@
             self.__dict__["_row_parts"] = parts
         return parts
 
-    def _sandwich_parts(self, parts, d, rows, cols_host, colsum, center=None):
+    def _sandwich_parts(self, parts, d, rows, cols_host, colsum, center=None, epilogue=True):
         out = None
         for a, b, part in parts:
             r = None
@@ -471,7 +507,7 @@
                 r = (sel - a).to(torch.int32)
             cs = [None] * len(self.matrices) if colsum is not None else None
             sub_cen = None if center is None else _Centering(center.vec)
-            res = part._sandwich_dev(d[a:b], r, cols_host, None, cs, center=sub_cen)
+            res = part._sandwich_dev(d[a:b], r, cols_host, None, cs, center=sub_cen, epilogue=epilogue)
             if sub_cen is not None:
                 center.groups = sub_cen.groups
             if sub_cen is not None and colsum is not None:
@@ -604,7 +640,7 @@
             sub_cen = _Centering({0: tc})
         try:
             cs_tmp = [None] * len(tmp.matrices) if colsum is not None else None
-            full = tmp._sandwich_dev(d, rows, None, None, cs_tmp, center=sub_cen)
+            full = tmp._sandwich_dev(d, rows, None, None, cs_tmp, center=sub_cen, epilogue=False)
         finally:
             dm._devblk = None
         if colsum is not None:
@@ -623,12 +659,12 @@
         sel = nar["sel"]
         return full.index_select(0, sel).index_select(1, sel)
 
-    def _sandwich_dev(self, d, rows, cols_host, plan=None, colsum=None, center=None, xtv=None):
+    def _sandwich_dev(self, d, rows, cols_host, plan=None, colsum=None, center=None, xtv=None, epilogue=True):
         if cols_host is not None and len(cols_host) >= FULL_THEN_SELECT * self.shape[1] \
                 and len(cols_host) > 0 and self._full_product_pays_cols(cols_host):
             pos_d, sub_d, n_cols = plan if plan is not None else self._sandwich_plan(cols_host)
             cs_full = [None] * len(self.matrices) if colsum is not None else None
-            full = self._sandwich_dev(d, rows, None, None, cs_full, center=center, xtv=xtv)
+            full = self._sandwich_dev(d, rows, None, None, cs_full, center=center, xtv=xtv, epilogue=False)
             if colsum is not None:
                 for i, c in enumerate(cs_full):
                     if c is not None:
@@ -637,12 +673,13 @@
             return full.index_select(0, cd).index_select(1, cd)
         parts = self._parts()
         if parts is not None:
-            return self._sandwich_parts(parts, d, rows, cols_host, colsum, center)
+            return self._sandwich_parts(parts, d, rows, cols_host, colsum, center, epilogue)
         if cols_host is not None and plan is None and NARROW_COLS > 0:
             nar = self._narrow_plan(cols_host)
             if nar == "wide":
                 cs_full = [None] * len(self.matrices) if colsum is not None else None
-                full = self._sandwich_dev(d, rows, None, None, cs_full, center=center, xtv=xtv)
+                full = self._sandwich_dev(d, rows, None, None, cs_full, center=center, xtv=xtv,
+                                          epilogue=False)
                 if colsum is not None:
                     _, sub_sel, _ = self._sandwich_plan(cols_host)
                     for i, c in enumerate(cs_full):
@@ -658,9 +695,10 @@
         empty = [sd is not None and D.nlen(sd) == 0 for sd in sub_d]
         done = set()
         return self._sandwich_terms(d, rows, cols_host, colsum, out, pos_d, sub_d, empty, done, center,
-                                    xtv if cols_host is None else None)
-
-    def _sandwich_terms(self, d, rows, cols_host, colsum, out, pos_d, sub_d, empty, done, center=None, xtv=None):
+                                    xtv if cols_host is None else None, epilogue)
+
+    def _sandwich_terms(self, d, rows, cols_host, colsum, out, pos_d, sub_d, empty, done, center=None, xtv=None,
+                        epilogue=True):
         from .ext import dense as xd
 
         mats = self.matrices
@@ -668,6 +706,7 @@
                    and m.shape[1] > 0]
         budget = (128 * 1024) // 8
         groups = self._cat_groups(cat_ids)
+        epi = self._step_epilogue(d, rows, cols_host, colsum, center, xtv) if epilogue else None
         if groups:
             d_eff = D.masked_d(d, rows)
         for grp in groups:
@@ -677,16 +716,16 @@
             for w, mw in enumerate(mats):
                 if empty[w] or mw.dtype != self.dtype or d.dtype != D.torch_dtype(self.dtype):
                     continue
-                stacked = self._fused_cats(mw, cats, grp, d_eff, rows, total, budget, d)
+                stacked = self._fused_cats(mw, cats, grp, d_eff, rows, total, budget, d, epi, w, pos_d)
                 if stacked is None:
+                    continue
+                if stacked is True:
+                    done.update((min(i, w), max(i, w)) for i in grp)
                     continue
                 whole = cols_host is None and len(grp) > 1
                 if whole:
-                    cache = self.__dict__.setdefault("_group_pos", {})
-                    gpos = cache.get(tuple(grp))
-                    if gpos is None:
-                        gpos = cache[tuple(grp)] = torch.cat([pos_d[i] for i in grp])
-                    xsplit.scatter_block(stacked.contiguous(), gpos, pos_d[w], out, mirror=True)
+                    xsplit.scatter_block(stacked.contiguous(), self._group_positions(grp, pos_d), pos_d[w], out,
+                                         mirror=True)
                 for ci, i in enumerate(grp):
                     res = stacked[int(offs[ci]):int(offs[ci + 1])]
                     if (colsum is not None and colsum[w] is None and not mats[i].drop_first
@@ -776,6 +815,11 @@
             elif isinstance(mi, DenseMatrix) and center is not None and center.get(i) is not None:
                 res = mi._sandwich_dev(d, rows, sub_d[i], center=center.get(i))
                 xsplit.scatter_block(res, pos_d[i], pos_d[i], out)
+            elif epi is not None and isinstance(mi, SparseMatrix):
+                res = mi._sandwich_dev(d, rows, sub_d[i],
+                                       partial=lambda A, dd, i=i: xfinish.sparse_sandwich_blocks(epi, A, dd, pos_d[i]))
+                if res is not None:
+                    xsplit.scatter_block(res, pos_d[i], pos_d[i], out)
             else:
                 res = mi._sandwich_dev(d, rows, sub_d[i])
                 xsplit.scatter_block(res, pos_d[i], pos_d[i], out)
@@ -786,6 +830,15 @@
                 if empty[j] or (i, j) in done:
                     continue
                 si, di = (i, j) if isinstance(mi, SparseMatrix) else (j, i)
+                if epi is not None and isinstance(mats[si], SparseMatrix) and isinstance(mats[di], DenseMatrix):
+                    res = mats[si]._cross_sandwich_dev(
+                        mats[di], d, rows, sub_d[si], sub_d[di],
+                        partial=lambda ent, Bd, dd, si=si, di=di: xfinish.csr_dense_ent(
+                            epi, ent, Bd, dd, self._kernel_pos(si, ent, pos_d), pos_d[di]))
+                    if res is not None:
+                        res = res if si == i else res.T
+                        xsplit.scatter_block(res.contiguous(), pos_d[i], pos_d[j], out, mirror=True)
+                    continue
                 if (colsum is not None and colsum[si] is None and isinstance(mats[si], SparseMatrix)
                         and isinstance(mats[di], DenseMatrix)):
                     box = []
@@ -798,6 +851,8 @@
                 else:
                     res = mi._cross_sandwich_dev(mats[j], d, rows, sub_d[i], sub_d[j])
                 xsplit.scatter_block(res.contiguous(), pos_d[i], pos_d[j], out, mirror=True)
+        if epi is not None:
+            epi.launch(out)
         return out
 
     def sandwich_graph(self, d, rows=None, cols=None):
```

Measured after the change: 1056 GB/s (median of 2 runs). Within noise of the previous version (-0.3%).
